# WT-MM/thor-slam

Hardware: AMD Instinct MI355X
Metric: synced stereo frames/sec (detect+match+pose) @640×400, 1/2/4/8 GPU (higher is better)
Workload: dtype u8+f64

## Files before the change

thor-slam_amd/csrc/k_describe.hip:

```cpp
#include "tslam_common.h"

#include "tslam_describe.h"

#define TS_DT_G 1

__device__ __forceinline__ void glds16d(const void* src, void* wave_dst) {
    __builtin_amdgcn_global_load_lds((__attribute__((address_space(1))) void*)src,
                                     (__attribute__((address_space(3))) void*)wave_dst, 16, 0, 0);
}

template <int NCH, int NLD = NCH>
__device__ __forceinline__ void stage_tile(const uint8_t* level, int W, int H, int r0, int cs, int nrows,
                                           uint8_t* lds, bool wide16) {
    const int lane = threadIdx.x & 63, wave = threadIdx.x >> 6;
    if (wide16) {
        const int n = nrows * NCH;
        for (int i0 = wave * 64; i0 < n; i0 += TS_DT_THREADS) {
            const int i = i0 + lane;
            if (i < n) {
                const int r = i / NCH, q = i - r * NCH;
                const int y = r0 + r, x = cs + 16 * q;
                if (q < NLD && y >= 0 && y < H && x >= 0 && x + 16 <= W) glds16d(level + (size_t)y * W + x, lds + 16 * i0);
            }
        }
    } else {
        for (int i = threadIdx.x; i < nrows * 16 * NCH; i += TS_DT_THREADS) {
            const int r = i / (16 * NCH), q = i - r * (16 * NCH);
            const int y = r0 + r, x = cs + q;
            if (y >= 0 && y < H && x >= 0 && x < W) lds[i] = level[(size_t)y * W + x];
        }
    }
}

struct DiscSlot {
    uint32_t wx, mk, wy;
    int32_t rofs;
};
struct DiscTable {
    DiscSlot e[320];
};
constexpr DiscTable make_disc_table() {
    DiscTable t{};
    for (int s = 0; s < 320; ++s) {
        const int r = s / 9, w = s - 9 * r;
        uint32_t a = 0, m = 0, b = 0;
        for (int j = 0; j < 4; ++j) {
            const int dx = 4 * w - 15 + j, dy = r - 15;
            if (r < 31 && dx <= 15 && dx * dx + dy * dy <= 225) {
                a |= (uint32_t)(dx + 15) << (8 * j);
                m |= 1u << (8 * j);
                b |= (uint32_t)(dy + 15) << (8 * j);
            }
        }
        t.e[s] = DiscSlot{a, m, b, (r < 30 ? r : 30) * TS_DT_RAW_P + 4 * w};
    }
    return t;
}
__constant__ DiscTable c_disc = make_disc_table();

__global__ __launch_bounds__(TS_DT_THREADS) void k_describe(BatchCtx c) {
    __shared__ __attribute__((aligned(16))) uint8_t s_raw[(TS_DT_RAW_ROWS + 1) * TS_DT_RAW_P];
    __shared__ __attribute__((aligned(16))) uint8_t s_smo[TS_DT_SMO_ROWS * TS_DT_P];
    __shared__ uint16_t s_list[TS_DT_W * TS_DT_H / 4];
    __shared__ uint32_t s_n;
    const int lane = threadIdx.x & 63, wave = threadIdx.x >> 6;
    int img, local;
    if (!xcd_image_block(blockIdx.x, c.n * c.ncam, c.g.dt_total, &img, &local)) return;
    int l = 0;
    while (l + 1 < c.g.n_levels && local >= c.g.dt_start[l + 1]) ++l;
    local -= c.g.dt_start[l];
    const int nx = c.g.dt_nx[l];
    const int ty = local / nx, tx = local - ty * nx;
    const int W = c.g.W[l], H = c.g.H[l];
    const int x0 = tx * TS_DT_W, y0 = ty * TS_DT_H;
    int cam, f;
    view_image(c, img, &f, &cam);
    const int slot = ring_slot(c, c.g0 + f);
    const size_t ib = (size_t)slot * c.C + cam;
    const uint8_t* raw = c.pyr + ib * c.g.pyr_bytes + c.g.pyr_off[l];
    const uint8_t* smo = c.smo + ((size_t)f * c.C + cam) * c.g.pyr_bytes + c.g.pyr_off[l];
    uint32_t* kps = c.kps + ib * c.g.K * 2;
    uint32_t* desc = c.desc + ib * c.g.K * 8;
    uint32_t* desc_ys = c.desc_ys + ib * c.g.K * 8;
    const uint4* ys = c.ys + ib * c.g.K + c.g.koff[l];
    const uint16_t* rs = c.rowstart + ib * c.g.rs_total + c.g.rs_off[l];
    const int kn = c.kcount[ib * c.g.n_levels + l];

    if (local == 0) {
        const int Kl = c.g.Kq[l];
        for (int i = kn * 8 + threadIdx.x; i < Kl * 8; i += TS_DT_THREADS) {
            desc[(size_t)(c.g.koff[l] + i / 8) * 8 + (i & 7)] = 0u;
            desc_ys[(size_t)(c.g.koff[l] + i / 8) * 8 + (i & 7)] = 0u;
        }
    }
    const int pa = rs[y0], pb = rs[min(y0 + TS_DT_H, H)];
    if (pa >= pb) return;
    if (threadIdx.x == 0) s_n = 0;
    __syncthreads();

    const bool wide16 = ((W & 15) == 0) && ((c.g.pyr_off[l] & 15) == 0) && ((c.g.pyr_bytes & 15) == 0);
    const int c0 = x0 - TS_DT_HX;
    const int cr = x0 - 16;
    stage_tile<TS_DT_RAW_P / 16>(raw, W, H, y0 - 15, cr, TS_DT_RAW_ROWS, s_raw, wide16);
    stage_tile<TS_DT_P / 16, (TS_DT_W + 2 * TS_DT_HX) / 16>(smo, W, H, y0 - 18, c0, TS_DT_SMO_ROWS, s_smo, wide16);

    uint32_t wx[5], mk[5], wy[5];
    int rofs[5];
#pragma unroll
    for (int i = 0; i < 5; ++i) {
        const uint4 d = reinterpret_cast<const uint4*>(&c_disc)[lane + 64 * i];
        wx[i] = d.x;
        mk[i] = d.y;
        wy[i] = d.z;
        rofs[i] = (int)d.w;
    }
    const double wa0 = lane < 30 ? (double)c.wedges[2 * lane] : 0.0, wa1 = lane < 30 ? (double)c.wedges[2 * lane + 1] : 0.0;
    const double wb0 = lane < 30 ? (double)c.wedges[2 * lane + 2] : 0.0, wb1 = lane < 30 ? (double)c.wedges[2 * lane + 3] : 0.0;

    for (int p = pa + threadIdx.x; p < pb; p += TS_DT_THREADS) {
        const int x = ys[p].x & 0xFFFF;
        if (x >= x0 && x < x0 + TS_DT_W) s_list[atomicAdd(&s_n, 1u)] = (uint16_t)p;
    }
    __syncthreads();
    const int n = (int)s_n;
    for (int g0 = wave * TS_DT_G; g0 < n; g0 += (TS_DT_THREADS / 64) * TS_DT_G) {
        int bin[TS_DT_G], pos[TS_DT_G];
        uint4 rec[TS_DT_G];
#pragma unroll
        for (int g = 0; g < TS_DT_G; ++g) {
            pos[g] = g0 + g < n ? (int)s_list[g0 + g] : -1;
            rec[g] = pos[g] >= 0 ? ys[pos[g]] : uint4{0u, 0u, 0u, 0u};
        }
#pragma unroll
        for (int g = 0; g < TS_DT_G; ++g) {
            bin[g] = 0;
            if (pos[g] < 0) continue;
            const int x = rec[g].x & 0xFFFF, y = rec[g].x >> 16;
            const int ob = (y - y0) * TS_DT_RAW_P + (x - 15 - cr);
            const uint32_t sh = (uint32_t)ob & 3u;
            const uint8_t* obase = s_raw + (ob & ~3);
            uint32_t sx = 0, s1 = 0, sy = 0;
#pragma unroll
            for (int i = 0; i < 5; ++i) {
                const uint32_t* wp = reinterpret_cast<const uint32_t*>(obase + rofs[i]);
                const uint32_t v = __builtin_amdgcn_alignbyte(wp[1], wp[0], sh);
                s1 = __builtin_amdgcn_udot4(mk[i], v, s1, false);
                sx = __builtin_amdgcn_udot4(wx[i], v, sx, false);
                sy = __builtin_amdgcn_udot4(wy[i], v, sy, false);
            }
            const int s15 = (int)__umul24(s1, 15u);
            const int m10 = wave_sum_dpp((int)sx - s15);
            const int m01 = wave_sum_dpp((int)sy - s15);
            const double d01 = (double)m01, d10 = (double)m10;
            const bool hit = lane < 30 && (wa0 * d01 - wa1 * d10) >= 0.0 && (wb0 * d01 - wb1 * d10) < 0.0;
            const uint64_t hm = __ballot(hit);
            bin[g] = hm ? (int)__builtin_ctzll(hm) : 0;
        }
        uint32_t t[TS_DT_G][4];
#pragma unroll
        for (int g = 0; g < TS_DT_G; ++g)
#pragma unroll
            for (int j = 0; j < 4; ++j) t[g][j] = pos[g] >= 0 ? c.brief_table[bin[g] * 256 + 64 * j + lane] : 0u;
#pragma unroll
        for (int g = 0; g < TS_DT_G; ++g) {
            if (pos[g] < 0) continue;
            const int x = rec[g].x & 0xFFFF, y = rec[g].x >> 16;
            const uint8_t* pbase = s_smo + (y - y0) * TS_DT_P + (x - 18 - c0);
            uint32_t words[8];
#pragma unroll
            for (int j = 0; j < 4; ++j) {
                const int a = pbase[t[g][j] & 0xFFFFu];
                const int b = pbase[t[g][j] >> 16];
                const uint64_t bm = __ballot(a < b);
                words[2 * j] = (uint32_t)bm;
                words[2 * j + 1] = (uint32_t)(bm >> 32);
            }
            const int kidx = (int)rec[g].z;
            uint32_t w = 0;
#pragma unroll
            for (int j = 0; j < 8; ++j) asm volatile("v_writelane_b32 %0, %1, %2" : "+v"(w) : "s"(words[j]), "i"(j));
            if (lane < 8) {
                desc[(size_t)kidx * 8 + lane] = w;
                desc_ys[(size_t)(c.g.koff[l] + pos[g]) * 8 + lane] = w;
            }
            if (lane == 0) kps[(size_t)kidx * 2 + 1] = (rec[g].y & ~0xFF00u) | ((uint32_t)bin[g] << 8);
        }
    }
}

void launch_describe(const BatchCtx& c, hipStream_t s) {
    hipLaunchKernelGGL(k_describe, dim3(xcd_grid(c.n * c.ncam, c.g.dt_total)), dim3(TS_DT_THREADS), 0, s, c);
}
```

thor-slam_amd/csrc/k_image.hip:

```cpp
#include "tslam_common.h"

__device__ __forceinline__ int remap_px(const uint8_t* src, int W, int H, int2 m) {
    const int sx = m.x >> 5, sy = m.y >> 5;
    const int fx = m.x & 31, fy = m.y & 31;
    const int xa = min(max(sx, 0), W - 1), xb = min(max(sx + 1, 0), W - 1);
    const int ya = min(max(sy, 0), H - 1), yb = min(max(sy + 1, 0), H - 1);
    const int p00 = src[ya * W + xa], p01 = src[ya * W + xb];
    const int p10 = src[yb * W + xa], p11 = src[yb * W + xb];
    const int acc = p00 * (32 - fx) * (32 - fy) + p01 * fx * (32 - fy) + p10 * (32 - fx) * fy + p11 * fx * fy;
    return (acc + 512) >> 10;
}

__device__ __forceinline__ uint32_t box4(uint32_t r0a, uint32_t r0b, uint32_t r1a, uint32_t r1b) {
    auto pairsum = [](uint32_t v) { return (v & 0x00FF00FFu) + ((v >> 8) & 0x00FF00FFu); };
    const uint32_t sa = pairsum(r0a) + pairsum(r1a) + 0x00020002u;
    const uint32_t sb = pairsum(r0b) + pairsum(r1b) + 0x00020002u;
    const uint32_t qa = (sa >> 2) & 0x00FF00FFu, qb = (sb >> 2) & 0x00FF00FFu;
    return __builtin_amdgcn_perm(qb, qa, 0x06040200u);
}

__global__ __launch_bounds__(256) void k_rectify_pyramid(BatchCtx c) {
    extern __shared__ __attribute__((aligned(16))) uint8_t lds[];
    const int img = blockIdx.y;
    int f, cam;
    view_image(c, img, &f, &cam);
    const int W = c.W, H = c.H;
    const int y0 = blockIdx.x * TS_RECT_BAND;
    const int rows0 = min(TS_RECT_BAND, H - y0);
    const uint8_t* src = c.images + view_src(c, img) * W * H;
    uint8_t* pyr = c.pyr + ((size_t)ring_slot(c, c.g0 + f) * c.C + cam) * c.g.pyr_bytes;
    const bool has_map = (c.map_mask >> cam) & 1u;
    const int32_t* map = c.maps + (size_t)cam * W * H * 2;
    bool wide = (W & 63) == 0 && (c.g.pyr_bytes & 15) == 0;
    for (int l = 1; l < c.g.n_levels; ++l) wide = wide && (c.g.pyr_off[l] & 15) == 0 && (c.g.W[l] & 15) == 0;

    uint8_t* l0 = lds;
    if (wide) {
        const int W16 = W >> 4, n16 = rows0 * W16;
        for (int i = threadIdx.x; i < n16; i += blockDim.x) {
            const int r = i / W16, x16 = i - r * W16;
            const size_t off = (size_t)(y0 + r) * W + 16 * x16;
            uint4 v;
            if (has_map) {
                uint32_t w[4];
                const int2* mp = reinterpret_cast<const int2*>(map) + off;
#pragma unroll
                for (int q = 0; q < 4; ++q) {
                    uint32_t acc = 0;
#pragma unroll
                    for (int b = 0; b < 4; ++b) acc |= (uint32_t)remap_px(src, W, H, mp[4 * q + b]) << (8 * b);
                    w[q] = acc;
                }
                v = {w[0], w[1], w[2], w[3]};
            } else {
                v = *reinterpret_cast<const uint4*>(src + off);
            }
            reinterpret_cast<uint4*>(l0)[i] = v;
            *reinterpret_cast<uint4*>(pyr + off) = v;
        }
        __syncthreads();
        const uint8_t* prev = l0;
        int prevW = W;
        uint8_t* cur = l0 + TS_RECT_BAND * W;
        for (int l = 1; l < c.g.n_levels; ++l) {
            const int Wl = c.g.W[l], Hl = c.g.H[l];
            const int ly0 = y0 >> l;
            const int lrows = min(TS_RECT_BAND >> l, Hl - ly0);
            const int W4 = Wl >> 2;
            uint8_t* out = pyr + c.g.pyr_off[l];
            for (int i = threadIdx.x; i < lrows * W4; i += blockDim.x) {
                const int r = i / W4, x4 = i - r * W4;
                const uint2 a = *reinterpret_cast<const uint2*>(prev + (2 * r) * prevW + 8 * x4);
                const uint2 b = *reinterpret_cast<const uint2*>(prev + (2 * r + 1) * prevW + 8 * x4);
                const uint32_t v = box4(a.x, a.y, b.x, b.y);
                reinterpret_cast<uint32_t*>(cur)[i] = v;
                *reinterpret_cast<uint32_t*>(out + (size_t)(ly0 + r) * Wl + 4 * x4) = v;
            }
            __syncthreads();
            prev = cur;
            prevW = Wl;
            cur = cur + (TS_RECT_BAND >> l) * Wl;
        }
        return;
    }

    for (int idx = threadIdx.x; idx < rows0 * W; idx += blockDim.x) {
        const int r = idx / W;
        const int x = idx - r * W;
        const int y = y0 + r;
        const int v = has_map ? remap_px(src, W, H, *reinterpret_cast<const int2*>(map + ((size_t)y * W + x) * 2))
                              : src[y * W + x];
        l0[r * W + x] = (uint8_t)v;
        pyr[(size_t)y * W + x] = (uint8_t)v;
    }
    __syncthreads();
    const uint8_t* prev = l0;
    int prevW = W;
    uint8_t* cur = l0 + TS_RECT_BAND * W;
    for (int l = 1; l < c.g.n_levels; ++l) {
        const int Wl = c.g.W[l], Hl = c.g.H[l];
        const int ly0 = y0 >> l;
        const int lrows = min(TS_RECT_BAND >> l, Hl - ly0);
        uint8_t* out = pyr + c.g.pyr_off[l];
        for (int idx = threadIdx.x; idx < lrows * Wl; idx += blockDim.x) {
            const int r = idx / Wl;
            const int x = idx - r * Wl;
            const int a = prev[(2 * r) * prevW + 2 * x] + prev[(2 * r) * prevW + 2 * x + 1] +
                          prev[(2 * r + 1) * prevW + 2 * x] + prev[(2 * r + 1) * prevW + 2 * x + 1];
            const uint8_t v = (uint8_t)((a + 2) >> 2);
            cur[r * Wl + x] = v;
            out[(size_t)(ly0 + r) * Wl + x] = v;
        }
        __syncthreads();
// ... 268 lines not shown
            kbits |= ((nb >> 15) & 1u) << h;
            kbits |= ((nb >> 31) & 1u) << (h + 2);
        }
#pragma unroll
        for (int j = 0; j < 4; ++j)
            if (x0 + j < M || x0 + j >= W - M) kbits &= ~(1u << j);
    }
    uint64_t bm[4];
    uint32_t tot = 0;
#pragma unroll
    for (int j = 0; j < 4; ++j) {
        bm[j] = __ballot((kbits >> j) & 1u);
        tot += (uint32_t)__popcll(bm[j]);
    }
    if (tot == 0) return;
    uint32_t base = 0;
    if (lane == 0) base = atomicAdd(count, tot);
    base = (uint32_t)__builtin_amdgcn_readfirstlane((int)base);
#pragma unroll
    for (int j = 0; j < 4; ++j) {
        if ((kbits >> j) & 1u) {
            const uint32_t rank = __builtin_amdgcn_mbcnt_hi((uint32_t)(bm[j] >> 32), __builtin_amdgcn_mbcnt_lo((uint32_t)bm[j], 0u));
            const uint32_t pv = (P >> (8 * j)) & 0xFFu;
            cand[base + rank] = ((255u - pv) << 22) | ((uint32_t)y << 11) | (uint32_t)(x0 + j);
            atomicAdd(&hist[255 - pv], 1u);
        }
        base += (uint32_t)__popcll(bm[j]);
    }
}


__device__ __forceinline__ void glds16(const uint4* src, uint4* wave_dst) {
    __builtin_amdgcn_global_load_lds((__attribute__((address_space(1))) void*)src,
                                     (__attribute__((address_space(3))) void*)wave_dst, 16, 0, 0);
}

typedef unsigned short u16x2 __attribute__((ext_vector_type(2)));

struct HsumSel {
    uint32_t d0, d1, d3, d4;
};
__device__ __forceinline__ HsumSel hsum_sel(bool first, bool last) {
    return {first ? 0x05040404u : 0x05040302u, first ? 0x06050404u : 0x06050403u,
            last ? 0x03030201u : 0x04030201u, last ? 0x03030302u : 0x05040302u};
}
__device__ __forceinline__ void hsum4(const uint8_t* p, const HsumSel& s, u16x2* ev, u16x2* od) {
    const uint32_t a = *(const uint32_t*)(p - 4), b = *(const uint32_t*)p, c2 = *(const uint32_t*)(p + 4);
    const uint32_t D0 = __builtin_amdgcn_perm(b, a, s.d0), D1 = __builtin_amdgcn_perm(b, a, s.d1);
    const uint32_t D3 = __builtin_amdgcn_perm(c2, b, s.d3), D4 = __builtin_amdgcn_perm(c2, b, s.d4);
    const uint32_t h0 = __builtin_amdgcn_udot4(D0, 0x04060401u, D1 >> 24, false);
    const uint32_t h1 = __builtin_amdgcn_udot4(D1, 0x04060401u, b >> 24, false);
    const uint32_t h2 = __builtin_amdgcn_udot4(b, 0x04060401u, D3 >> 24, false);
    const uint32_t h3 = __builtin_amdgcn_udot4(D3, 0x04060401u, D4 >> 24, false);
    *ev = __builtin_bit_cast(u16x2, h0 | (h2 << 16));
    *od = __builtin_bit_cast(u16x2, h1 | (h3 << 16));
}

__device__ __forceinline__ uint32_t vsum4(u16x2 e0, u16x2 e1, u16x2 e2, u16x2 e3, u16x2 e4, u16x2 d0, u16x2 d1,
                                          u16x2 d2, u16x2 d3, u16x2 d4) {
    const u16x2 four = {4, 4}, six = {6, 6}, rnd = {128, 128};
    const u16x2 ve = six * e2 + (four * (e1 + e3) + ((e0 + e4) + rnd));
    const u16x2 vo = six * d2 + (four * (d1 + d3) + ((d0 + d4) + rnd));
    return __builtin_amdgcn_perm(__builtin_bit_cast(uint32_t, vo), __builtin_bit_cast(uint32_t, ve), 0x07030501u);
}

template <int MODE, bool CNT>
__device__ __forceinline__ void detect_body(const BatchCtx& c, int bx, int img) {
    extern __shared__ __attribute__((aligned(16))) uint8_t lds[];
    __shared__ uint32_t s_hist[256];
    __shared__ uint32_t s_count;
    __shared__ uint16_t s_q[TS_DET_WAVES][2][TS_DET_Q];
    __shared__ __attribute__((aligned(16))) uint32_t s_tail[2][TS_DET_WAVES];
    int f, cam;
    view_image(c, img, &f, &cam);
    int l = 0;
    while (l + 1 < c.g.n_levels && bx >= c.g.band_start[l + 1]) ++l;
    const int te = MODE == 1 ? c.fast_threshold + 1
                                   : max(c.fast_threshold + 1, (int)c.det_thr[(size_t)cam * c.g.n_levels + l]);
    const int band = bx - c.g.band_start[l];
    const int W = c.g.W[l], H = c.g.H[l];
    const int BR = c.g.band_rows[l];
    const int y0 = band * BR;
    const int lane = threadIdx.x & 63, wave = threadIdx.x >> 6;
    const size_t img_off = ((size_t)ring_slot(c, c.g0 + f) * c.C + cam) * c.g.pyr_bytes + c.g.pyr_off[l];
    const uint8_t* src = c.pyr + img_off;
    uint8_t* smo = c.smo + ((size_t)f * c.C + cam) * c.g.pyr_bytes + c.g.pyr_off[l];
    const int NR = BR + 2 * TS_DET_HALO;
    uint8_t* tile = lds;
    uint8_t* score = lds + NR * W;
    const int thr = c.fast_threshold;
    const bool wide = ((W & 3) == 0) && ((img_off & 3) == 0);
    const int rows_here = min(BR, H - y0);

    for (int i = threadIdx.x; i < 256; i += TS_DET_THREADS) s_hist[i] = 0;
    if (threadIdx.x == 0) s_count = 0;
    if (((W & 15) == 0) && ((img_off & 15) == 0)) {
        const int W16 = W >> 4, n16 = NR * W16;
        const uint4* s16 = (const uint4*)src;
        const int dr = TS_DET_THREADS / W16, dx = TS_DET_THREADS - dr * W16;
        int r = (wave * 64 + lane) / W16, x = wave * 64 + lane - r * W16;
        for (int i0 = wave * 64; i0 < n16; i0 += TS_DET_THREADS) {
            if (i0 + lane < n16)
                glds16(s16 + (size_t)min(max(y0 - TS_DET_HALO + r, 0), H - 1) * W16 + x, (uint4*)tile + i0);
            r += dr;
            x += dx;
            if (x >= W16) {
                x -= W16;
                ++r;
            }
        }
    } else {
        for (int i = threadIdx.x; i < NR * W; i += TS_DET_THREADS) {
            const int r = i / W, x = i - r * W;
            tile[i] = src[(size_t)min(max(y0 - TS_DET_HALO + r, 0), H - 1) * W + x];
        }
    }
    __syncthreads();

    if (wide) {
        const int W4 = W >> 2;
        const int groups = c.g.smooth_groups[l];
        const int SR = (BR + groups - 1) / groups;
        for (int it = threadIdx.x; it < groups * W4; it += TS_DET_THREADS) {
            const int half = it / W4, q = it - half * W4, x0 = 4 * q;
            const int o0 = SR * half, o1 = min(o0 + SR, rows_here);
            if (o0 >= o1) continue;
            const HsumSel hs = hsum_sel(q == 0, q == W4 - 1);
            const uint8_t* rp = tile + (TS_DET_HALO - 2 + o0) * W + x0;
            u16x2 e0, e1, e2, e3, e4, d0, d1, d2, d3, d4;
            hsum4(rp, hs, &e0, &d0);
            hsum4(rp + W, hs, &e1, &d1);
            hsum4(rp + 2 * W, hs, &e2, &d2);
            hsum4(rp + 3 * W, hs, &e3, &d3);
            rp += 4 * W;
            uint32_t off = (uint32_t)((y0 + o0) * W + x0);
            int o = o0;
#define TS_SMOOTH_ROW(A, B, C, D, N, a, b, cc, d, n)                            \
    {                                                                         \
        hsum4(rp, hs, &N, &n);                                                \
        *(uint32_t*)(smo + off) = vsum4(A, B, C, D, N, a, b, cc, d, n);       \
        rp += W;                                                              \
        off += (uint32_t)W;                                                   \
        if (++o == o1) break;                                                 \
    }
            for (;;) {
                TS_SMOOTH_ROW(e0, e1, e2, e3, e4, d0, d1, d2, d3, d4)
                TS_SMOOTH_ROW(e1, e2, e3, e4, e0, d1, d2, d3, d4, d0)
                TS_SMOOTH_ROW(e2, e3, e4, e0, e1, d2, d3, d4, d0, d1)
                TS_SMOOTH_ROW(e3, e4, e0, e1, e2, d3, d4, d0, d1, d2)
                TS_SMOOTH_ROW(e4, e0, e1, e2, e3, d4, d0, d1, d2, d3)
            }
#undef TS_SMOOTH_ROW
        }
    } else {
        for (int x = threadIdx.x; x < W; x += TS_DET_THREADS) {
            const int xm2 = max(x - 2, 0), xm1 = max(x - 1, 0), xp1 = min(x + 1, W - 1), xp2 = min(x + 2, W - 1);
            int h0 = 0, h1 = 0, h2 = 0, h3 = 0;
            for (int r = TS_DET_HALO - 2; r < TS_DET_HALO + rows_here + 2; ++r) {
                const uint8_t* row = tile + r * W;
                const int h4 = row[xm2] + 4 * row[xm1] + 6 * row[x] + 4 * row[xp1] + row[xp2];
                if (r >= TS_DET_HALO + 2) {
                    const int acc = h0 + 4 * h1 + 6 * h2 + 4 * h3 + h4;
                    smo[(size_t)(y0 + r - 2 - TS_DET_HALO) * W + x] = (uint8_t)((acc + 128) >> 8);
                }
                h0 = h1; h1 = h2; h2 = h3; h3 = h4;
            }
        }
// ... 370 lines not shown
    }
    {
        const uint32_t bc = (int)threadIdx.x < nb ? cnt[threadIdx.x] : 0u;
        const uint32_t incl = block_inclusive_scan<NT>(bc, s_part, 1);
        if (threadIdx.x == 0) s_pref[0] = 0u;
        if ((int)threadIdx.x < nb) s_pref[threadIdx.x + 1] = incl;
    }
    __syncthreads();
    const int ncand = (int)s_pref[nb];
    auto sweep_g = [&](auto&& fn) {
        int lo = 0;
        for (int i0 = threadIdx.x; i0 < ncand; i0 += 4 * NT) {
            uint32_t k[4];
#pragma unroll
            for (int u = 0; u < 4; ++u) {
                const int i = i0 + u * NT;
                k[u] = 0u;
                if (i < ncand) {
                    while ((int)s_pref[lo + 1] <= i) ++lo;
                    k[u] = cand[__umul24((uint32_t)lo, (uint32_t)cap) + (uint32_t)(i - (int)s_pref[lo])];
                }
            }
#pragma unroll
            for (int u = 0; u < 4; ++u)
                if (i0 + u * NT < ncand) fn(i0 + u * NT, k[u]);
        }
    };
    bool res = false;
    auto sweep = [&](auto&& fn) {
        if (S::RCAP > 0 && res) {
            for (int i = threadIdx.x; i < ncand; i += NT) fn(i, s_res[i]);
        } else {
            sweep_g(fn);
        }
    };
    const bool fits = S::RCAP > 0 && ncand <= rcap;

    block_find_crossing<NT>(s_h, 256, (uint32_t)Kl, s_part, s_x);
    const uint32_t total = s_x[3];
    for (int i = threadIdx.x; i < 256; i += NT) s_h[i] = 0u;
    uint32_t thresh = 0xFFFFFFFFu;
    if (total > (uint32_t)Kl) {
        const uint32_t sbin = s_x[0];
        const uint32_t need = (uint32_t)Kl - s_x[1];
        const uint32_t eq = s_x[2];
        thresh = (sbin << 22) | 0x3FFFFFu;
        if (need < eq) {
            res = fits;
            sweep_g([&](int i, uint32_t k) {
                if (S::RCAP > 0 && res) s_res[i] = k;
                if ((k >> 22) == sbin) atomicAdd(&s_a[(k >> 11) & 2047u], 1u);
            });
            __syncthreads();
            block_find_crossing<NT>(s_a, BINS, need, s_part, s_x);
            const uint32_t ystar = s_x[0];
            const uint32_t need2 = need - s_x[1];
            const uint32_t eq2 = s_x[2];
            thresh = (sbin << 22) | (ystar << 11) | 2047u;
            for (int i = threadIdx.x; i < BINS; i += NT) s_a[i] = 0u;
            if (need2 < eq2) {
                sweep([&](int, uint32_t k) {
                    if ((k >> 11) == ((sbin << 11) | ystar)) atomicAdd(&s_fill[k & 2047u], 1u);
                });
                __syncthreads();
                block_find_crossing<NT>(s_fill, BINS, need2, s_part, s_x);
                thresh = (sbin << 22) | (ystar << 11) | s_x[0];
                if (!S::BIG || Kl <= S::KCAP)
                    for (int i = threadIdx.x; i < BINS; i += NT) s_fill[i] = 0u;
            }
        }
    }
    if (S::RCAP > 0 && !res && fits && eager) {
        sweep_g([&](int i, uint32_t k) { s_res[i] = k; });
        res = true;
    }
    sweep([&](int, uint32_t k) {
        if (k <= thresh) {
            const uint32_t slot = atomicAdd(&s_nsel, 1u);
            if (slot < (uint32_t)(S::BIG ? SEL_MAX : S::KCAP)) s_keys[slot] = k;
        }
    });
    __syncthreads();
    const int nsel = min((int)s_nsel, Kl);
    const int slot = ring_slot(c, c.g0 + f);
    uint32_t* kp = c.kps + (((size_t)slot * c.C + cam) * c.g.K + c.g.koff[l]) * 2;
    const int Hl = c.g.H[l];
    const bool counting = !S::BIG || nsel <= S::KCAP;
    if (counting) {
        for (int i = threadIdx.x; i < nsel; i += NT) atomicAdd(&s_h[s_keys[i] >> 22], 1u);
        __syncthreads();
        for (int b = threadIdx.x; b < 256; b += NT)
            if (s_h[b] > TS_SEL_BUCKET_MAX) s_flag = 1;
        block_exclusive_scan<NT>(s_h, 256, s_part);
    }
    __syncthreads();
    if (counting && s_flag == 0) {
        uint32_t* fill = s_h + 256;
        for (int i = threadIdx.x; i < nsel; i += NT) {
            const uint32_t k = s_keys[i], b = k >> 22;
            s_tmp[s_h[b] + atomicAdd(&fill[b], 1u)] = k;
        }
        __syncthreads();
        for (int i = threadIdx.x; i < nsel; i += NT) {
            const uint32_t k = s_tmp[i], b = k >> 22;
            const int lo = (int)s_h[b], n = (int)fill[b];
            int r = 0;
            for (int j = lo; j < lo + n; ++j) r += s_tmp[j] < k;
            s_keys[lo + r] = k;
        }
        __syncthreads();
    } else {
        bitonic_sort<NT>(s_keys, nsel);
    }
    for (int i = threadIdx.x; i < Kl; i += NT) {
        uint32_t xy = 0, meta = (uint32_t)l;
        if (i < nsel) {
            const uint32_t k = s_keys[i];
            xy = (k & 2047u) | (((k >> 11) & 2047u) << 16);
            meta = (uint32_t)l | ((255u - (k >> 22)) << 16);
        }
        kp[2 * i] = xy;
        kp[2 * i + 1] = meta;
    }
    if (threadIdx.x == 0) {
        c.kcount[((size_t)slot * c.C + cam) * c.g.n_levels + l] = nsel;
        const int tfull = c.fast_threshold + 1;
        const int te = MODE == 1 ? tfull : max(tfull, (int)c.det_thr[(size_t)cam * c.g.n_levels + l]);
        const bool short_k = (int)total < Kl;
        if (MODE == 0) c.det_fail[fcl] = (short_k && te > tfull) ? 1u : 0u;
        int next = tfull;
        if (!short_k && nsel > 0) {
            const int sk = 255 - (int)(s_keys[nsel - 1] >> 22);
            next = max(tfull, sk - 2);
        }
        atomicMin(&c.det_thr_acc[(size_t)cam * c.g.n_levels + l], (uint32_t)next);
    }

    uint4* ys = c.ys + ((size_t)slot * c.C + cam) * c.g.K + c.g.koff[l];
    uint16_t* rs = c.rowstart + ((size_t)slot * c.C + cam) * c.g.rs_total + c.g.rs_off[l];
    uint16_t* yp = c.ypos + ((size_t)slot * c.C + cam) * c.g.K;
    auto record = [&](int rank) -> uint4 {
        const uint32_t k = s_keys[rank];
        return {(k & 2047u) | (((k >> 11) & 2047u) << 16), (uint32_t)l | ((255u - (k >> 22)) << 16),
                (uint32_t)(c.g.koff[l] + rank), 1u};
    };
    for (int i = nsel + threadIdx.x; i < Kl; i += NT) {
        ys[i] = {0u, (uint32_t)l, (uint32_t)(c.g.koff[l] + i), 0u};
        yp[c.g.koff[l] + i] = (uint16_t)(c.g.koff[l] + i);
    }
    if (counting) {
        for (int i = threadIdx.x; i < nsel; i += NT) atomicAdd(&s_a[(s_keys[i] >> 11) & 2047u], 1u);
        __syncthreads();
        block_exclusive_scan<NT>(s_a, BINS, s_part);
        for (int y = threadIdx.x; y <= Hl; y += NT) rs[y] = (uint16_t)s_a[y];
        for (int i = threadIdx.x; i < nsel; i += NT) {
            const uint32_t y = (s_keys[i] >> 11) & 2047u;
            s_tmp[s_a[y] + atomicAdd(&s_fill[y], 1u)] = (uint32_t)i;
        }
        __syncthreads();
        for (int p = threadIdx.x; p < nsel; p += NT) {
            const uint32_t i = s_tmp[p], y = (s_keys[i] >> 11) & 2047u;
            const int lo = (int)s_a[y], n = (int)s_fill[y];
            int r = 0;
            for (int j = lo; j < lo + n; ++j) r += s_tmp[j] < i;
            ys[lo + r] = record((int)i);
            yp[c.g.koff[l] + i] = (uint16_t)(c.g.koff[l] + lo + r);
        }
// ... 85 lines not shown
```

thor-slam_amd/csrc/k_match.hip:

```cpp
#include "tslam_common.h"

#define TS_MQ 128
#define TS_MRED_PITCH 33
#define TS_MRING 1024
#define TS_MCHUNKS 6
#define TS_MCNT_MERGED 0
#define TS_MCNT_DIRECT 1
#define TS_MCNT_FLUSHED 2
#define TS_MCNT_EMPTY 3
#define TS_MCNT_WALKED 4

typedef int v8i_t __attribute__((ext_vector_type(8)));
typedef float v16f_t __attribute__((ext_vector_type(16)));
typedef unsigned short u16x2_t __attribute__((ext_vector_type(2)));

__device__ __forceinline__ uint32_t med3_u32(uint32_t a, uint32_t b, uint32_t c) {
    uint32_t r;
    asm("v_med3_u32 %0, %1, %2, %3" : "=v"(r) : "v"(a), "v"(b), "v"(c));
    return r;
}

__device__ __forceinline__ bool gate_ok(uint32_t qgate, uint32_t txy, uint32_t span) {
    const u16x2_t d = __builtin_bit_cast(u16x2_t, qgate) - __builtin_bit_cast(u16x2_t, txy);
    const u16x2_t m = __builtin_elementwise_min(d, __builtin_bit_cast(u16x2_t, span));
    return __builtin_bit_cast(uint32_t, m) == __builtin_bit_cast(uint32_t, d);
}

__device__ __forceinline__ uint32_t key_dist(uint32_t key) {
    return (uint32_t)__uint_as_float(key & 0xFFFF8000u);
}

template <bool CNT>
__device__ __forceinline__ void match_body(const BatchCtx& c) {
    TS_BACK_PRIO;
    __shared__ __attribute__((aligned(16))) uint2 s_red[4][32 * TS_MRED_PITCH];
    __shared__ __attribute__((aligned(16))) uint32_t s_key[2][TS_MQ];
    __shared__ __attribute__((aligned(16))) uint32_t s_wk[4][32];
    uint4* const s_qrec = reinterpret_cast<uint4*>(&s_red[0][0]);
    uint4* const s_qdesc = s_qrec + TS_MQ;
    __shared__ uint32_t s_sq[4][32];
    __shared__ uint32_t s_si[4][32];
    __shared__ __attribute__((aligned(16))) uint32_t s_sg[4][2][16];
    __shared__ __attribute__((aligned(16))) float s_spc[4][2][16];
    __shared__ uint32_t s_tb[TS_MTB];
    const int nfp = c.match_modes == 1 ? 0 : c.n * c.npair;
    const int z = blockIdx.y;
    const int mode = z < nfp ? 1 : 0;
    const int fl = z < nfp ? z : z - nfp;
    const int p = c.pair0 + fl % c.npair;
    const int f = fl / c.npair;
    const int64_t g = c.g0 + f;
    int l = 0;
    while (l + 1 < c.g.n_levels && (int)blockIdx.x >= c.g.qtile_start[l + 1]) ++l;
    const int tile = blockIdx.x - c.g.qtile_start[l];
    const int q0 = tile * TS_MQ;
    const size_t mbase = (((size_t)f * c.P + p) * 2 + mode) * c.g.K;
    auto no_match = [&]() {
        if ((int)threadIdx.x < TS_MQ && q0 + (int)threadIdx.x < c.g.Kq[l]) c.qbest[mbase + c.g.koff[l] + q0 + threadIdx.x] = 0xFFFFFFFFu;
        if (CNT && threadIdx.x == 0) atomicAdd(&c.match_cnt[8 * mode + TS_MCNT_EMPTY], 1u);
    };
    if ((mode == 1 && g == 0) ||
        (mode == 0 && c.rgbd)) {
        no_match();
        return;
    }
    const int slot = ring_slot(c, g);
    const int qcam = c.cpp * p;
    const int tslot = mode == 0 ? slot : ring_slot(c, g - 1);
    const int tcam = mode == 0 ? qcam + 1 : qcam;
    const int K = c.g.K;
    const int qn = c.kcount[((size_t)slot * c.C + qcam) * c.g.n_levels + l];
    const int tn = c.kcount[((size_t)tslot * c.C + tcam) * c.g.n_levels + l];
    if (q0 >= qn || tn == 0) {
        no_match();
        return;
    }
    if (CNT && threadIdx.x == 0) atomicAdd(&c.match_cnt[8 * mode + TS_MCNT_WALKED], 1u);
    const int lane = threadIdx.x & 63, wave = threadIdx.x >> 6;
    const int ci = lane & 31, h = lane >> 5;
    const size_t qbase = ((size_t)slot * c.C + qcam) * K;
    const size_t tbase = ((size_t)tslot * c.C + tcam) * K;
    const uint4* qys = c.ys + qbase + c.g.koff[l];
    const uint4* tys = c.ys + tbase + c.g.koff[l];
    uint32_t* const tb = c.tbest + mbase + c.g.koff[l];
    const uint4* qdesc = reinterpret_cast<const uint4*>(c.desc_ys + (qbase + c.g.koff[l]) * 8);
    const uint4* tdesc = reinterpret_cast<const uint4*>(c.desc_ys + (tbase + c.g.koff[l]) * 8);
    const uint16_t* trs = c.rowstart + ((size_t)tslot * c.C + tcam) * c.g.rs_total + c.g.rs_off[l];
    const int Hl = c.g.H[l];
    const int row_tol = c.mp.row_tol, dmax = c.mp.max_disp >> l, win = c.mp.window >> l;
    const int gx_lo = mode == 0 ? 1 : -win, gx_hi = mode == 0 ? dmax : win, gy_tol = mode == 0 ? row_tol : win;
    const uint32_t span = (uint32_t)(2 * gy_tol) << 16 | (uint32_t)(gx_hi - gx_lo);

    const int nq = min(TS_MQ, qn - q0);
    {
        const int t = threadIdx.x & (TS_MQ - 1), half = threadIdx.x >> 7;
        const int pos = q0 + min(t, nq - 1);
        if (half == 0) s_qrec[t] = qys[pos];
        s_qdesc[2 * t + half] = qdesc[2 * pos + half];
    }
    __syncthreads();
    const bool wave_active = 32 * wave < nq;
    const int reach = mode == 0 ? row_tol : win;
    int wt0 = 0, wt1 = 0;
    {
        const int i0 = mode == 1 ? 0 : min(32 * wave, nq - 1), i1 = mode == 1 ? nq - 1 : min(32 * wave + 31, nq - 1);
        const int wy0 = (int)(s_qrec[i0].x >> 16), wy1 = (int)(s_qrec[i1].x >> 16);
        if (wave_active) {
            wt0 = (int)trs[max(0, wy0 - reach)];
            wt1 = (int)trs[min(Hl - 1, wy1 + reach) + 1];
        }
    }
    const uint32_t mcap = (uint32_t)min(c.mp.merge_cap, TS_MTB);
    int bt0 = 0, bt1 = 0;
    if (mcap) {
        const int by0 = (int)(s_qrec[0].x >> 16), by1 = (int)(s_qrec[nq - 1].x >> 16);
        bt0 = __builtin_amdgcn_readfirstlane((int)trs[max(0, by0 - reach)]);
        bt1 = __builtin_amdgcn_readfirstlane((int)trs[min(Hl - 1, by1 + reach) + 1]);
        for (int i = threadIdx.x; i < min((int)mcap, bt1 - bt0); i += 256) s_tb[i] = 0xFFFFFFFFu;
    }
    int bi = 32 * wave + ci;
    if (mode == 1) {
        if (threadIdx.x < TS_MQ) {
            const int t = threadIdx.x;
            s_key[0][t] = t < nq ? (s_qrec[t].x & 0xFFFF) << 8 | (uint32_t)t : 0x1000000u | (uint32_t)t;
        }
        __syncthreads();
        if (threadIdx.x < TS_MQ) {
            const uint32_t key = s_key[0][threadIdx.x];
            int rank = 0;
            const uint4* k4 = reinterpret_cast<const uint4*>(s_key[0]);
#pragma unroll 4
            for (int i = 0; i < TS_MQ / 4; ++i) {
                const uint4 v = k4[i];
                rank += (v.x < key) + (v.y < key) + (v.z < key) + (v.w < key);
            }
            s_key[1][rank] = threadIdx.x;
        }
        __syncthreads();
        bi = (int)s_key[1][32 * wave + ci];
    }
    const bool active = bi < nq;
    int qx = 0, qy = 0;
    uint32_t qi = 0, pc = 0;
    if (active) {
        const uint4 rec = s_qrec[bi];
        const uint4 d = s_qdesc[2 * bi + h];
        qi = rec.z;
        qx = rec.x & 0xFFFF;
        qy = rec.x >> 16;
        pc = __popc(d.x) + __popc(d.y) + __popc(d.z) + __popc(d.w);
    }
// ... 153 lines not shown
                    if (lane == 0 && nd) atomicAdd(&c.match_cnt[8 * mode + TS_MCNT_DIRECT], nd);
                }
            }
        }
        __builtin_amdgcn_fence(__ATOMIC_RELEASE, "wavefront");
        __builtin_amdgcn_wave_barrier();
        __builtin_amdgcn_fence(__ATOMIC_ACQUIRE, "wavefront");
    }

    __builtin_amdgcn_fence(__ATOMIC_RELEASE, "wavefront");
    __builtin_amdgcn_wave_barrier();
    __builtin_amdgcn_fence(__ATOMIC_ACQUIRE, "wavefront");
    uint2* red = s_red[wave];
#pragma unroll
    for (int r = 0; r < 16; ++r) red[(2 * r + h) * TS_MRED_PITCH + ci] = uint2{best[r], second[r]};
    __builtin_amdgcn_fence(__ATOMIC_RELEASE, "wavefront");
    __builtin_amdgcn_wave_barrier();
    __builtin_amdgcn_fence(__ATOMIC_ACQUIRE, "wavefront");
    uint32_t b = 0xFFFFFFFFu, s2 = 0xFFFFFFFFu;
#pragma unroll
    for (int i = 0; i < 16; ++i) {
        const uint2 v = red[ci * TS_MRED_PITCH + 16 * h + i];
        s2 = min(min(s2, v.y), max(b, v.x));
        b = min(b, v.x);
    }
    {
        const uint32_t ob = (uint32_t)__shfl_xor((int)b, 32, 64), os = (uint32_t)__shfl_xor((int)s2, 32, 64);
        s2 = min(min(s2, os), max(b, ob));
        b = min(b, ob);
    }
    const uint32_t qk = s_sq[wave][ci];
    const int qpos = q0 + (int)s_si[wave][ci];
    if (h == 0 && qpos < c.g.Kq[l]) {
        const size_t qp = mbase + c.g.koff[l] + qpos;
        const bool found = qk != 0xFFFFFFFFu && b < 0x7F800000u;
        c.qbest[qp] = found ? key_dist(b) << 16 | (b & 0x7FFFu) : 0xFFFFFFFFu;
        if (qk != 0xFFFFFFFFu) c.qsecond[qp] = s2 < 0x7F800000u ? key_dist(s2) : 256u;
        c.qtpos[qp] = found ? c.ypos[tbase + (b & 0x7FFFu)] : (uint16_t)0;
    }
    if (mcap) {
        __syncthreads();
        const int len = min((int)mcap, bt1 - bt0);
        uint32_t na = 0;
        for (int i = threadIdx.x; i < len; i += 256) {
            const uint32_t v = s_tb[i];
            if (v != 0xFFFFFFFFu) {
                atomicMin(&tb[bt0 + i], v);
                ++na;
            }
        }
        if (CNT && na) atomicAdd(&c.match_cnt[8 * mode + TS_MCNT_FLUSHED], na);
    }
}

__device__ __forceinline__ double parabola(int sm, int s0, int sp) {
    const int den = sm - 2 * s0 + sp;
    return den > 0 ? (double)(sm - sp) / (2.0 * (double)den) : 0.0;
}

__device__ __forceinline__ void row11(const uint8_t* img, int W, int y, int x0, uint32_t* w) {
    const uint8_t* a = img + (size_t)y * W + x0;
    const uint32_t sh = (uint32_t)(reinterpret_cast<uintptr_t>(a) & 3u);
    const uint32_t* p = reinterpret_cast<const uint32_t*>(a - sh);
    const uint32_t d0 = p[0], d1 = p[1], d2 = p[2], d3 = p[3];
    w[0] = __builtin_amdgcn_alignbyte(d1, d0, sh);
    w[1] = __builtin_amdgcn_alignbyte(d2, d1, sh);
    w[2] = __builtin_amdgcn_alignbyte(d3, d2, sh) & 0x00FFFFFFu;
}

__device__ __forceinline__ uint4 stage_row11(const uint8_t* img, int W, int y, int x0) {
    uint32_t w3[3];
    row11(img, W, y, x0, w3);
    return uint4{w3[0], w3[1], w3[2], 0u};
}

__device__ __forceinline__ uint4 align_row15(const uint32_t* d, uint32_t sh) {
    return uint4{__builtin_amdgcn_alignbyte(d[1], d[0], sh), __builtin_amdgcn_alignbyte(d[2], d[1], sh),
                 __builtin_amdgcn_alignbyte(d[3], d[2], sh), __builtin_amdgcn_alignbyte(d[4], d[3], sh) & 0x00FFFFFFu};
}
__device__ __forceinline__ uint4 stage_row15(const uint8_t* img, int W, int y, int x0) {
    const uint8_t* a = img + (size_t)y * W + x0;
    const uint32_t sh = (uint32_t)(reinterpret_cast<uintptr_t>(a) & 3u);
    const uint32_t* q = reinterpret_cast<const uint32_t*>(a - sh);
    const uint32_t d[5] = {q[0], q[1], q[2], q[3], q[4]};
    return align_row15(d, sh);
}

__device__ __forceinline__ void shift_row11(const uint4* row, int kx, uint32_t* w) {
    const uint32_t* wb = reinterpret_cast<const uint32_t*>(row);
    const int kh = kx >> 2;
    const uint32_t sh = (uint32_t)(kx & 3);
    const uint32_t d0 = wb[kh], d1 = wb[kh + 1], d2 = wb[kh + 2], d3 = wb[3 - kh];
    w[0] = __builtin_amdgcn_alignbyte(d1, d0, sh);
    w[1] = __builtin_amdgcn_alignbyte(d2, d1, sh);
    w[2] = __builtin_amdgcn_alignbyte(d3, d2, sh) & 0x00FFFFFFu;
}

__device__ __forceinline__ uint32_t sad_row11(const uint32_t* a, const uint32_t* w, uint32_t s) {
    s = __builtin_amdgcn_sad_u8(a[0], w[0], s);
    s = __builtin_amdgcn_sad_u8(a[1], w[1], s);
    return __builtin_amdgcn_sad_u8(a[2], w[2], s);
}

template <int ASH>
__device__ __forceinline__ uint32_t stereo_sad(const uint4* a, const uint4* b, int kx) {
    uint32_t s = 0;
#pragma unroll
    for (int dy = 0; dy < 11; ++dy) {
        uint32_t la[3], w[3];
        if (ASH < 0) {
            const uint4 ra = a[dy];
            la[0] = ra.x, la[1] = ra.y, la[2] = ra.z;
        } else {
            shift_row11(a + dy, ASH, la);
        }
        shift_row11(b + dy, kx, w);
        s = sad_row11(la, w, s);
    }
    return s;
}

__device__ __forceinline__ void stereo_store(const BatchCtx& c, size_t out, int j, int l, int qx, int xr, int ks,
                                             const int* cost) {
    double d0 = __builtin_nan("");
    if (j >= 0 && ks > 0 && ks < 4) {
        const double delta = parabola(cost[ks - 1], cost[ks], cost[ks + 1]);
        const double sc = (double)(1 << l);
        const double v = ((double)qx - ((double)(xr + (ks - TS_SAD_RANGE)) + delta)) * sc;
        if (v > 0.0) d0 = v;
    }
    c.stereo[out] = j;
    c.disp[out] = d0;
}

#define TS_RT_AROWS 11
#define TS_RT_BROWS 15
__device__ __forceinline__ void temporal_sad(const uint4* a, const uint4* b, int kx, uint32_t* s) {
#pragma unroll
    for (int ky = 0; ky < 5; ++ky) s[ky] = 0u;
#pragma unroll
    for (int r = 0; r < TS_RT_BROWS; ++r) {
        uint32_t w[3];
        shift_row11(b + r, kx, w);
#pragma unroll
        for (int ky = 0; ky < 5; ++ky) {
            const int dy = r - ky;
            if (dy < 0 || dy >= TS_RT_AROWS) continue;
            const uint4 ra = a[dy];
            const uint32_t la[3] = {ra.x, ra.y, ra.z};
            s[ky] = sad_row11(la, w, s[ky]);
        }
    }
}

__device__ __forceinline__ void temporal_store(double* out_uv, int j, int l, int qx, int qy, int a, const int* cq) {
    double u = __builtin_nan(""), v = u;
    if (j >= 0) {
        const int c0 = cq[a];
        const int cl = cq[max(a - 1, 0)], cr = cq[min(a + 1, 24)];
        const int cu = cq[max(a - 5, 0)], cd = cq[min(a + 5, 24)];
        const int ky = a / 5, kx = a % 5;
        if (kx > 0 && kx < 4 && ky > 0 && ky < 4) {
            const double ddx = parabola(cl, c0, cr);
            const double ddy = parabola(cu, c0, cd);
            const double sc = (double)(1 << l);
            u = (((double)(qx + (kx - TS_SAD_RANGE)) + ddx) + 0.5) * sc - 0.5;
            v = (((double)(qy + (ky - TS_SAD_RANGE)) + ddy) + 0.5) * sc - 0.5;
        }
    }
    out_uv[0] = u;
    out_uv[1] = v;
}

struct MatchRef {
    uint32_t qb, sd, tb;
    int j, tp;
};
__device__ __forceinline__ void match_query(const BatchCtx& c, size_t mbase, int pos, MatchRef* m) {
    m->qb = c.qbest[mbase + pos];
    m->sd = c.qsecond[mbase + pos];
    m->tp = c.qtpos[mbase + pos];
    m->j = m->qb == 0xFFFFFFFFu ? 0 : (int)(m->qb & 0xFFFF);
}
__device__ __forceinline__ void match_train(const BatchCtx& c, size_t mbase, size_t tkb, MatchRef* m, uint32_t* tkp) {
    m->tb = c.tbest[mbase + m->tp];
    *tkp = c.kps[(tkb + m->j) * 2];
}
__device__ __forceinline__ int match_accept(const BatchCtx& c, const MatchRef& m, int qi, bool ok) {
    const int bd = (int)(m.qb >> 16);
    return ((int)ok & (int)(m.qb != 0xFFFFFFFFu) & (int)(bd <= c.mp.max_hamming) &
            (int)(bd * 100 < c.mp.ratio_pct * (int)m.sd) & (int)((int)(m.tb & 0xFFFF) == qi)) ? m.j : -1;
}
__device__ __forceinline__ int match_lookup(const BatchCtx& c, size_t mbase, int pos, int qi, bool ok, size_t tkb,
                                            uint32_t* tkp) {
    MatchRef m;
    match_query(c, mbase, pos, &m);
    match_train(c, mbase, tkb, &m, tkp);
    return match_accept(c, m, qi, ok);
}

#define TS_RS_QPB 32
__global__ __launch_bounds__(256) void k_refine_stereo(BatchCtx c) {
    TS_BACK_PRIO;
    __shared__ uint4 s_a[TS_RS_QPB][11];
    __shared__ uint4 s_b[TS_RS_QPB][11];
    __shared__ int s_cost[TS_RS_QPB][5];
    const int lane = threadIdx.x & 63, wave = threadIdx.x >> 6;
    const int K = c.g.K;
    int z, local;
    if (!xcd_image_block(blockIdx.x, c.n * c.npair, (K + TS_RS_QPB - 1) / TS_RS_QPB, &z, &local)) return;
    const int p = c.pair0 + z % c.npair, f = z / c.npair;
    const int64_t g = c.g0 + f;
    const int slot = ring_slot(c, g);
    const int sub = lane & 7;
    const int qslot = wave * 8 + (lane >> 3);
    const int pos = local * TS_RS_QPB + qslot;
    const bool live = pos < K;
    const size_t mbase = (((size_t)f * c.P + p) * 2 + 0) * K;
    const int qcam = c.cpp * p;
    const size_t qkb = ((size_t)slot * c.C + qcam) * K;
    int l = 0, qi = 0, j = -1;
    uint32_t qxy = 0, tkp = 0;
    if (live) {
        const uint4 rec = c.ys[qkb + pos];
        qi = (int)rec.z;
        l = (int)(rec.y & 0xFFu);
        qxy = rec.x;
        j = match_lookup(c, mbase, pos, qi, rec.w != 0, ((size_t)slot * c.C + qcam + 1) * K, &tkp);
    }
    int qx = 0, xr = 0;
    if (j >= 0) {
        const int W = c.g.W[l];
        qx = qxy & 0xFFFF;
        const int qy = qxy >> 16;
        xr = tkp & 0xFFFF;
        const uint8_t* Lp = c.pyr + ((size_t)slot * c.C + qcam) * c.g.pyr_bytes + c.g.pyr_off[l];
        const uint8_t* Rp = c.pyr + ((size_t)slot * c.C + qcam + 1) * c.g.pyr_bytes + c.g.pyr_off[l];
        for (int hl = sub; hl < 22; hl += 8) {
            if (hl < 11)
                s_a[qslot][hl] = stage_row11(Lp, W, qy - TS_SAD_HALF + hl, qx - TS_SAD_HALF);
            else
                s_b[qslot][hl - 11] = stage_row15(Rp, W, qy - TS_SAD_HALF + hl - 11, xr - TS_SAD_HALF - TS_SAD_RANGE);
        }
    }
    __builtin_amdgcn_fence(__ATOMIC_ACQ_REL, "wavefront");
    uint32_t key = 0xFFFFFFFFu;
    if (j >= 0 && sub < 5) {
        const uint32_t s = stereo_sad<-1>(s_a[qslot], s_b[qslot], sub);
        s_cost[qslot][sub] = (int)s;
        key = (s << 5) | (uint32_t)sub;
    }
#pragma unroll
    for (int m = 1; m < 8; m <<= 1) key = min(key, (uint32_t)__shfl_xor((int)key, m, 64));
    __builtin_amdgcn_fence(__ATOMIC_ACQ_REL, "wavefront");
    if (live && sub == 0) stereo_store(c, ((size_t)slot * c.P + p) * K + qi, j, l, qx, xr, (int)(key & 31u), s_cost[qslot]);
}

#define TS_RT_QPB 32
__global__ __launch_bounds__(256) void k_refine_temporal(BatchCtx c) {
    TS_BACK_PRIO;
    __shared__ uint4 s_a[TS_RT_QPB][TS_RT_AROWS];
    __shared__ uint4 s_b[TS_RT_QPB][TS_RT_BROWS];
    __shared__ int s_cost[TS_RT_QPB][25];
    const int lane = threadIdx.x & 63, wave = threadIdx.x >> 6;
    const int K = c.g.K;
    int z, local;
    if (!xcd_image_block(blockIdx.x, c.n * c.npair, (K + TS_RT_QPB - 1) / TS_RT_QPB, &z, &local)) return;
    const int p = c.pair0 + z % c.npair, f = z / c.npair;
    const int64_t g = c.g0 + f;
    const int slot = ring_slot(c, g);
    const int sub = lane & 7;
    const int qslot = wave * 8 + (lane >> 3);
    const int pos = local * TS_RT_QPB + qslot;
    const bool live = pos < K;
    const size_t mbase = (((size_t)f * c.P + p) * 2 + 1) * K;
    const int qcam = c.cpp * p;
    const size_t qkb = ((size_t)slot * c.C + qcam) * K;
    int l = 0, qi = 0, j = -1;
    uint32_t qxy = 0, pxy = 0;
    const int pslot = g > 0 ? ring_slot(c, g - 1) : slot;
    if (live) {
        const uint4 rec = c.ys[qkb + pos];
        qi = (int)rec.z;
        l = (int)(rec.y & 0xFFu);
        qxy = rec.x;
        j = match_lookup(c, mbase, pos, qi, rec.w != 0 && g > 0, ((size_t)pslot * c.C + qcam) * K, &pxy);
    }
    int32_t* out_idx = c.temporal + ((size_t)slot * c.P + p) * K;
    double* out_uv = c.tuv + (((size_t)f * c.P + p) * K + qi) * 2;
    if (live && sub == 0) out_idx[qi] = j;
    int qx = 0, qy = 0;
    if (j >= 0) {
        const int W = c.g.W[l];
        qx = qxy & 0xFFFF;
        qy = qxy >> 16;
        const int px = pxy & 0xFFFF, py = pxy >> 16;
        const uint8_t* A = c.pyr + ((size_t)pslot * c.C + qcam) * c.g.pyr_bytes + c.g.pyr_off[l];
        const uint8_t* B = c.pyr + ((size_t)slot * c.C + qcam) * c.g.pyr_bytes + c.g.pyr_off[l];
        for (int hl = sub; hl < TS_RT_AROWS + TS_RT_BROWS; hl += 8) {
            if (hl < TS_RT_AROWS)
                s_a[qslot][hl] = stage_row11(A, W, py - TS_SAD_HALF + hl, px - TS_SAD_HALF);
            else
                s_b[qslot][hl - TS_RT_AROWS] = stage_row15(B, W, qy - TS_SAD_HALF - TS_SAD_RANGE + hl - TS_RT_AROWS,
                                                           qx - TS_SAD_HALF - TS_SAD_RANGE);
        }
    }
    __builtin_amdgcn_fence(__ATOMIC_ACQ_REL, "wavefront");
    uint32_t key = 0xFFFFFFFFu;
    if (j >= 0 && sub < 5) {
        uint32_t s[5];
        temporal_sad(s_a[qslot], s_b[qslot], sub, s);
#pragma unroll
        for (int ky = 0; ky < 5; ++ky) {
            const int o = ky * 5 + sub;
            s_cost[qslot][o] = (int)s[ky];
            key = min(key, (s[ky] << 5) | (uint32_t)o);
        }
    }
#pragma unroll
    for (int m = 1; m < 8; m <<= 1) key = min(key, (uint32_t)__shfl_xor((int)key, m, 64));
    __builtin_amdgcn_fence(__ATOMIC_ACQ_REL, "wavefront");
    if (live && sub == 0) temporal_store(out_uv, j, l, qx, qy, (int)(key & 31u), s_cost[qslot]);
}

#define TS_RP_QPB 32
#define TS_RP_ROWS (TS_RT_BROWS + TS_RT_AROWS + 11)
#define TS_RP_ROUNDS ((TS_RP_ROWS + 7) / 8)
__global__ __launch_bounds__(256) void k_refine_pair(BatchCtx c) {
    TS_BACK_PRIO;
    __shared__ uint4 s_rows[TS_RP_QPB][TS_RP_ROWS];
    __shared__ int s_ct[TS_RP_QPB][25];
    __shared__ int s_cs[TS_RP_QPB][5];
    const int lane = threadIdx.x & 63, wave = threadIdx.x >> 6;
    const int K = c.g.K;
    int z, local;
    if (!xcd_image_block(blockIdx.x, c.n * c.npair, (K + TS_RP_QPB - 1) / TS_RP_QPB, &z, &local)) return;
    const int p = c.pair0 + z % c.npair, f = z / c.npair;
    const int64_t g = c.g0 + f;
    const int slot = ring_slot(c, g);
    const int pslot = g > 0 ? ring_slot(c, g - 1) : slot;
    const int sub = lane & 7;
    const int qslot = wave * 8 + (lane >> 3);
    const int pos = local * TS_RP_QPB + qslot;
    const bool live = pos < K;
    const size_t mbase = ((size_t)f * c.P + p) * 2 * K;
    const int qcam = c.cpp * p;
    const size_t qkb = ((size_t)slot * c.C + qcam) * K;
    int l = 0, qi = 0, js = -1, jt = -1;
    uint32_t qxy = 0, tkp = 0, pxy = 0;
    if (live) {
        const uint4 rec = c.ys[qkb + pos];
        qi = (int)rec.z;
        l = (int)(rec.y & 0xFFu);
        qxy = rec.x;
        MatchRef ms, mt;
        match_query(c, mbase, pos, &ms);
        match_query(c, mbase + K, pos, &mt);
        match_train(c, mbase, ((size_t)slot * c.C + qcam + 1) * K, &ms, &tkp);
        match_train(c, mbase + K, ((size_t)pslot * c.C + qcam) * K, &mt, &pxy);
        js = match_accept(c, ms, qi, rec.w != 0);
        jt = match_accept(c, mt, qi, rec.w != 0 && g > 0);
    }
    const size_t out = ((size_t)slot * c.P + p) * K + qi;
    if (live && sub == 0) c.temporal[out] = jt;
    const int qx = qxy & 0xFFFF, qy = qxy >> 16, xr = tkp & 0xFFFF;
    {
        int W = c.g.W[0], loff = c.g.pyr_off[0];
#pragma unroll
        for (int i = 1; i < TS_MAX_LEVELS; ++i)
            if (l >= i) W = c.g.W[i], loff = c.g.pyr_off[i];
        const int px = pxy & 0xFFFF, py = pxy >> 16;
        const uint8_t* cur = c.pyr + ((size_t)slot * c.C + qcam) * c.g.pyr_bytes + loff;
        const uint8_t* rgt = cur + c.g.pyr_bytes;
        const uint8_t* prv = c.pyr + ((size_t)pslot * c.C + qcam) * c.g.pyr_bytes + loff;
        const int nw = jt >= 0 ? TS_RT_BROWS : js >= 0 ? 11 : 0, w0 = jt >= 0 ? 0 : TS_SAD_RANGE;
        const int np = jt >= 0 ? TS_RT_AROWS : 0;
        const int total = nw + np + (js >= 0 ? 11 : 0);
        uint32_t d[TS_RP_ROUNDS][5], sh[TS_RP_ROUNDS];
#pragma unroll
        for (int k = 0; k < TS_RP_ROUNDS; ++k) {
            const int hl = sub + 8 * k;
            const bool inw = hl < nw, inp = !inw && hl < nw + np;
            const int r = inw ? hl + w0 : inp ? hl - nw : hl - nw - np;
            const uint8_t* img = inw ? cur : inp ? prv : rgt;
            const int y = inw ? qy - TS_SAD_HALF - TS_SAD_RANGE + r : inp ? py - TS_SAD_HALF + r : qy - TS_SAD_HALF + r;
            const int x0 = inw ? qx - TS_SAD_HALF - TS_SAD_RANGE : inp ? px - TS_SAD_HALF : xr - TS_SAD_HALF - TS_SAD_RANGE;
            const uint8_t* a = hl < total ? img + (size_t)y * W + x0 : cur;
            sh[k] = (uint32_t)(reinterpret_cast<uintptr_t>(a) & 3u);
            const uint32_t* q = reinterpret_cast<const uint32_t*>(a - sh[k]);
#pragma unroll
            for (int i = 0; i < 5; ++i) d[k][i] = q[i];
        }
#pragma unroll
        for (int k = 0; k < TS_RP_ROUNDS; ++k) {
            const int hl = sub + 8 * k;
            const bool inw = hl < nw, inp = !inw && hl < nw + np;
            uint4 v = align_row15(d[k], sh[k]);
            if (inp) v.z &= 0x00FFFFFFu, v.w = 0u;
            const int row = inw ? hl + w0 : inp ? TS_RT_BROWS + hl - nw : TS_RT_BROWS + TS_RT_AROWS + hl - nw - np;
            if (hl < total) s_rows[qslot][row] = v;
        }
    }
    __builtin_amdgcn_fence(__ATOMIC_ACQ_REL, "wavefront");
    const uint4* rows = s_rows[qslot];
    uint32_t kt = 0xFFFFFFFFu, ks = 0xFFFFFFFFu;
    if (jt >= 0 && sub < 5) {
        uint32_t s[5];
        temporal_sad(rows + TS_RT_BROWS, rows, sub, s);
#pragma unroll
        for (int ky = 0; ky < 5; ++ky) {
            const int o = ky * 5 + sub;
            s_ct[qslot][o] = (int)s[ky];
            kt = min(kt, (s[ky] << 5) | (uint32_t)o);
        }
    }
    if (js >= 0 && sub < 5) {
        const uint32_t s = stereo_sad<TS_SAD_RANGE>(rows + TS_SAD_RANGE, rows + TS_RT_BROWS + TS_RT_AROWS, sub);
        s_cs[qslot][sub] = (int)s;
        ks = (s << 5) | (uint32_t)sub;
    }
#pragma unroll
    for (int m = 1; m < 8; m <<= 1) {
        kt = min(kt, (uint32_t)__shfl_xor((int)kt, m, 64));
        ks = min(ks, (uint32_t)__shfl_xor((int)ks, m, 64));
    }
    __builtin_amdgcn_fence(__ATOMIC_ACQ_REL, "wavefront");
    if (live && sub == 0) {
        temporal_store(c.tuv + (((size_t)f * c.P + p) * K + qi) * 2, jt, l, qx, qy, (int)(kt & 31u), s_ct[qslot]);
        stereo_store(c, out, js, l, qx, xr, (int)(ks & 31u), s_cs[qslot]);
    }
}

__global__ __launch_bounds__(256) __attribute__((amdgpu_waves_per_eu(4))) void k_match(BatchCtx c) { match_body<false>(c); }
__global__ __launch_bounds__(256) __attribute__((amdgpu_waves_per_eu(4))) void k_match_counted(BatchCtx c) { match_body<true>(c); }

static void launch_k_match(const BatchCtx& c, dim3 grid, hipStream_t s) {
    if (c.match_cnt)
        hipLaunchKernelGGL(k_match_counted, grid, dim3(256), 0, s, c);
    else
        hipLaunchKernelGGL(k_match, grid, dim3(256), 0, s, c);
}

int match_blocks_per_cu() {
    int n = 0;
    return hipOccupancyMaxActiveBlocksPerMultiprocessor(&n, k_match, 256, 0) == hipSuccess ? n : -1;
}

void launch_match(const BatchCtx& c, hipStream_t s) {
    (void)hipMemsetAsync(c.tbest, 0xFF, sizeof(uint32_t) * (size_t)c.n * c.P * 2 * c.g.K, s);
    dim3 grid(c.g.total_qtiles, c.n * c.npair * (c.match_modes == 1 ? 1 : 2));
    launch_k_match(c, grid, s);
}

void launch_match_stereo(const BatchCtx& c, hipStream_t s) {
    BatchCtx st = c;
    st.match_modes = 1;
    (void)hipMemsetAsync(st.tbest, 0xFF, sizeof(uint32_t) * (size_t)st.n * st.P * 2 * st.g.K, s);
    launch_k_match(st, dim3(st.g.total_qtiles, st.n * st.npair), s);
    hipLaunchKernelGGL(k_refine_stereo, dim3(xcd_grid(st.n * st.npair, (st.g.K + TS_RS_QPB - 1) / TS_RS_QPB)), dim3(256), 0, s, st);
}

void launch_match_refine(const BatchCtx& c, hipStream_t s) {
    const int K = c.g.K;
    if (!c.rgbd && c.match_modes == 3 && c.mp.refine_split == 0) {
        hipLaunchKernelGGL(k_refine_pair, dim3(xcd_grid(c.n * c.npair, (K + TS_RP_QPB - 1) / TS_RP_QPB)), dim3(256), 0, s, c);
        return;
    }
    if (c.rgbd)
        launch_rgbd_depth(c, s);
    else
        hipLaunchKernelGGL(k_refine_stereo, dim3(xcd_grid(c.n * c.npair, (K + TS_RS_QPB - 1) / TS_RS_QPB)), dim3(256), 0, s, c);
    hipLaunchKernelGGL(k_refine_temporal, dim3(xcd_grid(c.n * c.npair, (K + TS_RT_QPB - 1) / TS_RT_QPB)), dim3(256), 0, s, c);
}
```

thor-slam_amd/csrc/k_pose.hip:

```cpp
#include "tslam_common.h"
#include "tslam_mul4.h"

#define P3P_VMAX 1000.0
#define P3P_BISECT 60

struct V3 {
    double x, y, z;
};

__device__ __forceinline__ double dot3(V3 a, V3 b) { return (a.x * b.x + a.y * b.y) + a.z * b.z; }
__device__ __forceinline__ V3 sub3(V3 a, V3 b) { return {a.x - b.x, a.y - b.y, a.z - b.z}; }
__device__ __forceinline__ V3 cross3(V3 a, V3 b) {
    return {a.y * b.z - a.z * b.y, a.z * b.x - a.x * b.z, a.x * b.y - a.y * b.x};
}
__device__ __forceinline__ V3 norm3(V3 a) {
    const double n = sqrt(dot3(a, a));
    return {a.x / n, a.y / n, a.z / n};
}
__device__ __forceinline__ void frame3(V3 p1, V3 p2, V3 p3, V3* e) {
    e[0] = norm3(sub3(p2, p1));
    e[2] = norm3(cross3(e[0], sub3(p3, p1)));
    e[1] = cross3(e[2], e[0]);
}
__device__ __forceinline__ double comp(V3 a, int i) { return i == 0 ? a.x : (i == 1 ? a.y : a.z); }
// ... 119 lines not shown
}

__device__ __forceinline__ uint64_t splitmix64(uint64_t x) {
    x = x + 0x9E3779B97F4A7C15ull;
    x = (x ^ (x >> 30)) * 0xBF58476D1CE4E5B9ull;
    x = (x ^ (x >> 27)) * 0x94D049BB133111EBull;
    return x ^ (x >> 31);
}

__device__ __forceinline__ bool is_inlier(const double* R, const double* t, const double* cr, double fx, double fy, double thr2) {
    const double X = cr[0], Y = cr[1], Z = cr[2], du = cr[3], dv = cr[4];
    const double xc = ((R[0] * X + R[1] * Y) + R[2] * Z) + t[0];
    const double yc = ((R[3] * X + R[4] * Y) + R[5] * Z) + t[1];
    const double zc = ((R[6] * X + R[7] * Y) + R[8] * Z) + t[2];
    const double ex = fx * xc + du * zc;
    const double ey = fy * yc + dv * zc;
    const double e2 = ex * ex + ey * ey;
    const double lim = thr2 * (zc * zc);
    return zc > 0.0 && e2 < lim;
}

typedef float f32x16 __attribute__((ext_vector_type(16)));
__device__ __forceinline__ int inlier_f32(const f32x16& pf, const float* q, float fx, float fy, float thr2) {
    const float X = q[0], Y = q[1], Z = q[2], du = q[3], dv = q[4];
    const float xc = fmaf(pf[0], X, fmaf(pf[1], Y, fmaf(pf[2], Z, pf[9])));
    const float yc = fmaf(pf[3], X, fmaf(pf[4], Y, fmaf(pf[5], Z, pf[10])));
    const float zc = fmaf(pf[6], X, fmaf(pf[7], Y, fmaf(pf[8], Z, pf[11])));
    const float ex = fmaf(fx, xc, du * zc);
    const float ey = fmaf(fy, yc, dv * zc);
    const float e2 = fmaf(ex, ex, ey * ey);
    const float lim = thr2 * (zc * zc);
    const float D = lim - e2;
    const float a = fmaf(pf[12], q[5], pf[13]);
    const float inner = fmaf(fabsf(ex), q[6], fmaf(fabsf(ey), q[7], thr2 * fabsf(zc)));
    const float bsum = fmaf(a, inner, e2 + lim);
    const float E = bsum * (32.0f / 16777216.0f);
    const float Ez = a * (32.0f / 16777216.0f);
    if (zc < -Ez || D < -E) return 0;
    if (zc > Ez && D > E) return 1;
    return -1;
}

__device__ bool solve6(const double* Hm, const double* g, double* x, double* L) {
    double inv[6];
    for (int j = 0; j < 6; ++j) {
        double s = Hm[j * 6 + j];
        for (int k = 0; k < j; ++k) s = s - L[j * 6 + k] * L[j * 6 + k];
        if (!(s > 0.0)) return false;
        const double d = sqrt(s);
        L[j * 6 + j] = d;
        inv[j] = 1.0 / d;
        for (int i = j + 1; i < 6; ++i) {
            double t = Hm[i * 6 + j];
            for (int k = 0; k < j; ++k) t = t - L[i * 6 + k] * L[j * 6 + k];
            L[i * 6 + j] = t * inv[j];
        }
    }
    double y[6];
    for (int i = 0; i < 6; ++i) {
        double s = g[i];
        for (int k = 0; k < i; ++k) s = s - L[i * 6 + k] * y[k];
        y[i] = s * inv[i];
    }
    for (int i = 5; i >= 0; --i) {
        double s = y[i];
        for (int k = i + 1; k < 6; ++k) s = s - L[k * 6 + i] * x[k];
        x[i] = s * inv[i];
    }
    return true;
}

#define POSE_THREADS 256
#define TS_RS_CPT 4
#define TS_MAX_HYP_SPLIT 256
#define N_ACC 29

__device__ __forceinline__ void write_stats(int32_t* so, int status, int n, int n_in, int best_cnt, int best_idx, int64_t g) {
    so[0] = status; so[1] = n; so[2] = n_in; so[3] = best_cnt; so[4] = best_idx; so[5] = (int)g; so[6] = 0; so[7] = 0;
}

__global__ __launch_bounds__(POSE_THREADS) void k_corr(BatchCtx c) {
    TS_BACK_PRIO;
    __shared__ int s_scan[2 * (POSE_THREADS / 64)];
    const int p = c.pair0 + (int)blockIdx.x % c.npair;
    const int f = (int)blockIdx.x / c.npair;
    const int fp = f * c.P + p;
    const int64_t g = c.g0 + f;
    const int tid = threadIdx.x;
    const int K = c.g.K;
    double* pout = c.pose + (size_t)fp * TS_POSE_DOUBLES;
    int32_t* sout = c.stats + (size_t)fp * TS_STATS_INTS;
    for (int i = tid; i < TS_POSE_DOUBLES; i += POSE_THREADS) pout[i] = (i < 16 && (i % 5) == 0) ? 1.0 : 0.0;
    if (g == 0) {
        if (tid == 0) write_stats(sout, 2, 0, 0, 0, -1, g);
        return;
    }
    const PairCalib cal = c.calib[p];
    const double fx = cal.fx, fy = cal.fy, cx = cal.cx, cy = cal.cy;
    const int pslot = ring_slot(c, g - 1);
    const int32_t* tm = c.temporal + ((size_t)ring_slot(c, g) * c.P + p) * K;
    const double* tuv = c.tuv + ((size_t)f * c.P + p) * K * 2;
    const double* dprev = c.disp + ((size_t)pslot * c.P + p) * K;
    const uint32_t* kprev = c.kps + ((size_t)pslot * c.C + c.cpp * p) * K * 2;
    double* corr = c.corr + ((size_t)f * c.P + p) * K * TS_CORR_DOUBLES;
    int n = 0;
    for (int base = 0; base < K; base += POSE_THREADS) {
        const int j = base + tid;
        int flag = 0, i = -1;
        double u = 0.0, v = 0.0, d = 0.0;
        if (j < K) {
            i = tm[j];
            if (i >= 0) {
                d = dprev[i];
                u = tuv[2 * j];
                v = tuv[2 * j + 1];
                flag = __builtin_isfinite(d) && __builtin_isfinite(u) && __builtin_isfinite(v);
            }
        }
        const uint64_t bm = __ballot(flag != 0);
        const int lane = tid & 63, wave = tid >> 6;
        int* wc = s_scan + ((base / POSE_THREADS) & 1) * 4;
        if (lane == 0) wc[wave] = __popcll(bm);
        __syncthreads();
        int before = 0, tot = 0;
#pragma unroll
        for (int w = 0; w < POSE_THREADS / 64; ++w) {
            before += w < wave ? wc[w] : 0;
            tot += wc[w];
        }
        const int pos = n + before + (int)__builtin_amdgcn_mbcnt_hi((uint32_t)(bm >> 32), __builtin_amdgcn_mbcnt_lo((uint32_t)bm, 0u));
        if (flag) {
            const uint32_t xy = kprev[2 * i], meta = kprev[2 * i + 1];
            const double sc = (double)(1 << (meta & 0xFF));
            const double ul = ((double)(xy & 0xFFFF) + 0.5) * sc - 0.5;
            const double vl = ((double)(xy >> 16) + 0.5) * sc - 0.5;
            const double z = cal.fxb / d;
            const double x = (ul - cx) * z / fx;
            const double y = (vl - cy) * z / fy;
            const double bx = (u - cx) / fx;
            const double by = (v - cy) / fy;
            const double nn = sqrt((bx * bx + by * by) + 1.0);
            double* cr = corr + (size_t)pos * TS_CORR_DOUBLES;
            cr[0] = x; cr[1] = y; cr[2] = z; cr[3] = cx - u; cr[4] = cy - v;
            cr[5] = bx / nn; cr[6] = by / nn; cr[7] = 1.0 / nn;
        }
        n += tot;
    }
    if (tid == 0) write_stats(sout, n < max(6, c.pp.min_inliers) ? 1 : 3, n, 0, 0, -1, g);
}

__global__ __launch_bounds__(POSE_THREADS) void k_p3p(BatchCtx c) {
    TS_BACK_PRIO;
    const int H = c.pp.n_hyp;
    const int gid = blockIdx.x * POSE_THREADS + threadIdx.x;
    if (gid >= c.n * c.npair * H) return;
    const int fl = gid / H, h = gid - fl * H;
    const int p = c.pair0 + fl % c.npair;
    const int f = fl / c.npair;
    const int fp = f * c.P + p;
    const int64_t g = c.g0 + f;
    const int32_t* sout = c.stats + (size_t)fp * TS_STATS_INTS;
    if (sout[0] != 3) return;
    const int n = sout[1];
    const double* corr = c.corr + ((size_t)f * c.P + p) * c.g.K * TS_CORR_DOUBLES;
    const uint64_t base_rng = splitmix64(c.pp.seed ^ ((uint64_t)g * 0x9E3779B97F4A7C15ull));
    uint32_t r[3];
#pragma unroll
    for (int k = 0; k < 3; ++k) r[k] = (uint32_t)(splitmix64(base_rng ^ ((uint64_t)h * 4ull + (uint64_t)k)) >> 32);
    const uint32_t un = (uint32_t)n;
    int i0 = (int)(r[0] % un);
    int i1 = (int)(r[1] % (un - 1));
    i1 += (i1 >= i0);
    int i2 = (int)(r[2] % (un - 2));
    const int lo = min(i0, i1), hi = max(i0, i1);
    i2 += (i2 >= lo);
    i2 += (i2 >= hi);
    const int idx[3] = {i0, i1, i2};
    V3 pw[3], fb[3];
#pragma unroll
    for (int k = 0; k < 3; ++k) {
        const double* cr = corr + (size_t)idx[k] * TS_CORR_DOUBLES;
        pw[k] = {cr[0], cr[1], cr[2]};
        fb[k] = {cr[5], cr[6], cr[7]};
// ... 996 lines not shown
```

thor-slam_amd/csrc/k_reloc.hip:

```cpp
#include "tslam_common.h"

#define RL_CHUNK 512

__global__ __launch_bounds__(256) void k_reloc_match(BatchCtx c, RelocQuery qi, const uint32_t* map_desc, int M_arg,
                                                     const int32_t* dM, int32_t* match) {
    __shared__ uint4 s_d[RL_CHUNK][2];
    const int K = c.g.K;
    const int M = dM ? *dM : M_arg;
    const int q = blockIdx.x * blockDim.x + threadIdx.x;
    bool valid = false;
    uint32_t d[8] = {0, 0, 0, 0, 0, 0, 0, 0};
    if (q < K) {
        const uint32_t meta = qi.kps[(size_t)q * 2 + 1];
        const int l = (int)(meta & 0xFF);
        valid = q - c.g.koff[l] < qi.kcount[l];
        const uint4* src = reinterpret_cast<const uint4*>(qi.desc + (size_t)q * 8);
        const uint4 a = src[0], b = src[1];
        d[0] = a.x; d[1] = a.y; d[2] = a.z; d[3] = a.w; d[4] = b.x; d[5] = b.y; d[6] = b.z; d[7] = b.w;
    }
    uint32_t best = 0xFFFFFFFFu, second = 0xFFFFFFFFu;
    for (int m0 = 0; m0 < M; m0 += RL_CHUNK) {
        const int nm = min(RL_CHUNK, M - m0);
        __syncthreads();
        for (int i = threadIdx.x; i < nm * 2; i += blockDim.x)
// ... 21 lines not shown
        const uint32_t bd = best >> 20, sd = second >> 20;
        if ((int)bd <= c.mp.max_hamming && (second == 0xFFFFFFFFu || 100u * bd < (uint32_t)c.mp.ratio_pct * sd))
            out = (int)(best & 0xFFFFFu);
    }
    match[q] = out;
}

__global__ __launch_bounds__(256) void k_reloc_corr(BatchCtx c, RelocQuery qi, int pair, const double* map_xyz,
                                                    const double* xf, const int32_t* match, double* corr, int32_t* stats,
                                                    double* pose, int64_t frame) {
    __shared__ int s_tmp[32];
    const int K = c.g.K;
    for (int i = threadIdx.x; i < TS_POSE_DOUBLES; i += blockDim.x) pose[i] = (i < 16 && (i % 5) == 0) ? 1.0 : 0.0;
    const PairCalib cal = c.calib[pair];
    const double fx = cal.fx, fy = cal.fy, cx = cal.cx, cy = cal.cy;
    int n = 0;
    for (int base = 0; base < K; base += blockDim.x) {
        const int q = base + threadIdx.x;
        const int m = q < K ? match[q] : -1;
        const int flag = m >= 0;
        const int lane = threadIdx.x & 63, wave = threadIdx.x >> 6;
        int x = flag;
        for (int o = 1; o < 64; o <<= 1) {
            const int y = __shfl_up(x, o, 64);
            if (lane >= o) x += y;
        }
        if (lane == 63) s_tmp[wave] = x;
        __syncthreads();
        int off = 0, tot = 0;
        for (int w = 0; w < (int)(blockDim.x >> 6); ++w) {
            if (w < wave) off += s_tmp[w];
            tot += s_tmp[w];
        }
        if (flag) {
            const uint32_t xy = qi.kps[(size_t)q * 2], meta = qi.kps[(size_t)q * 2 + 1];
            const double sc = (double)(1 << (meta & 0xFF));
            const double u = ((double)(xy & 0xFFFF) + 0.5) * sc - 0.5;
            const double v = ((double)(xy >> 16) + 0.5) * sc - 0.5;
            const double bx = (u - cx) / fx;
            const double by = (v - cy) / fy;
            const double nn = sqrt((bx * bx + by * by) + 1.0);
            double* cr = corr + (size_t)(n + off + x - flag) * TS_CORR_DOUBLES;
            const double X = map_xyz[(size_t)m * 3], Y = map_xyz[(size_t)m * 3 + 1], Z = map_xyz[(size_t)m * 3 + 2];
            if (xf) {
                for (int e = 0; e < 3; ++e) cr[e] = ((xf[4 * e] * X + xf[4 * e + 1] * Y) + xf[4 * e + 2] * Z) + xf[4 * e + 3];
            } else {
                cr[0] = X;
                cr[1] = Y;
                cr[2] = Z;
            }
            cr[3] = cx - u;
            cr[4] = cy - v;
            cr[5] = bx / nn;
            cr[6] = by / nn;
            cr[7] = 1.0 / nn;
        }
        n += tot;
        __syncthreads();
    }
    if (threadIdx.x == 0) {
        stats[0] = n < max(6, c.pp.min_inliers) ? 1 : 3;
        stats[1] = n;
        stats[2] = stats[3] = stats[6] = stats[7] = 0;
        stats[4] = -1;
        stats[5] = (int)frame;
    }
}

void launch_reloc(const BatchCtx& c, int pair, int64_t frame, const double* map_xyz, const uint32_t* map_desc, int M,
                  int32_t* match, double* corr, int32_t* stats, double* pose, double* ransac, double* hyp, hipStream_t s) {
    launch_reloc_query(c, pair, frame, reloc_query_ring(c, c.cpp * pair, frame), map_xyz, map_desc, M, nullptr, match, corr,
                       stats, pose, ransac, hyp, s);
}

void launch_reloc_query(const BatchCtx& c, int pair, int64_t frame, RelocQuery q, const double* map_xyz,
                        const uint32_t* map_desc, int M, const int32_t* dM, int32_t* match, double* corr, int32_t* stats,
                        double* pose, double* ransac, double* hyp, hipStream_t s) {
    hipLaunchKernelGGL(k_reloc_match, dim3((c.g.K + 255) / 256), dim3(256), 0, s, c, q, map_desc, M, dM, match);
    hipLaunchKernelGGL(k_reloc_corr, dim3(1), dim3(256), 0, s, c, q, pair, map_xyz, (const double*)nullptr, match,
                       corr, stats, pose, frame);
    BatchCtx r = c;
    r.n = 1;
    r.P = 1;
    r.pair0 = 0;
    r.npair = 1;
    r.g0 = frame;
    r.prior = nullptr;
    r.rig_prior = nullptr;
    r.calib[0] = c.calib[pair];
    r.corr = corr;
    r.stats = stats;
    r.pose = pose;
    r.ransac = ransac;
    r.hyp = hyp;
    launch_pose_solve(r, s);
}

void launch_reloc_rig(const BatchCtx& c, int64_t frame, const double* map_xyz, const uint32_t* map_desc, int M,
                      int32_t* match, double* corr, int32_t* stats, double* pose, double* ransac, double* hyp,
                      double* rig_pose, int32_t* rig_stats, hipStream_t s) {
    const int K = c.g.K;
    for (int p = 0; p < c.P; ++p) {
        int32_t* mp = match + (size_t)p * K;
        const RelocQuery q = reloc_query_ring(c, c.cpp * p, frame);
        hipLaunchKernelGGL(k_reloc_match, dim3((K + 255) / 256), dim3(256), 0, s, c, q, map_desc, M, (const int32_t*)nullptr,
                           mp);
        hipLaunchKernelGGL(k_reloc_corr, dim3(1), dim3(256), 0, s, c, q, p, map_xyz, c.rig_Einv + 16 * p, mp,
                           corr + (size_t)p * K * TS_CORR_DOUBLES, stats + (size_t)p * TS_STATS_INTS,
                           pose + (size_t)p * TS_POSE_DOUBLES, frame);
    }
    BatchCtx r = c;
    r.n = 1;
    r.pair0 = 0;
    r.npair = c.P;
    r.g0 = frame;
    r.corr = corr;
    r.stats = stats;
    r.pose = pose;
    r.ransac = ransac;
    r.hyp = hyp;
    r.prior = nullptr;
    r.rig_prior = nullptr;
    r.rig_pose = rig_pose;
    r.rig_stats = rig_stats;
    r.reloc = 1;
    launch_pose_solve(r, s);
    launch_rig_pose(r, s);
}
```

thor-slam_amd/csrc/k_rgbd.hip:

```cpp
#include "tslam_common.h"

__global__ __launch_bounds__(256) void k_rgbd_gray(BatchCtx c, uint8_t* gray) {
    const int img = blockIdx.y;
    const size_t npx = (size_t)c.W * c.H;
    const uint8_t* src = c.rgbd_in + (size_t)img * npx * 5;
    uint8_t* dst = gray + (size_t)img * npx;
    const size_t i = (size_t)blockIdx.x * blockDim.x + threadIdx.x;
    if ((npx & 3) == 0) {
        if (4 * i >= npx) return;
        const uint32_t* s32 = reinterpret_cast<const uint32_t*>(src) + 3 * i;
        const uint32_t w0 = s32[0], w1 = s32[1], w2 = s32[2];
        const uint8_t px[12] = {(uint8_t)w0, (uint8_t)(w0 >> 8), (uint8_t)(w0 >> 16), (uint8_t)(w0 >> 24),
                                (uint8_t)w1, (uint8_t)(w1 >> 8), (uint8_t)(w1 >> 16), (uint8_t)(w1 >> 24),
                                (uint8_t)w2, (uint8_t)(w2 >> 8), (uint8_t)(w2 >> 16), (uint8_t)(w2 >> 24)};
        uint32_t out = 0;
#pragma unroll
        for (int k = 0; k < 4; ++k) {
            const uint32_t b = px[3 * k], g = px[3 * k + 1], r = px[3 * k + 2];
            out |= ((r * 4899u + g * 9617u + b * 1868u + 8192u) >> 14) << (8 * k);
        }
        reinterpret_cast<uint32_t*>(dst)[i] = out;
    } else {
        for (size_t k = 4 * i; k < 4 * i + 4 && k < npx; ++k) {
            const uint32_t b = src[3 * k], g = src[3 * k + 1], r = src[3 * k + 2];
            dst[k] = (uint8_t)((r * 4899u + g * 9617u + b * 1868u + 8192u) >> 14);
        }
    }
}

__global__ __launch_bounds__(256) void k_rgbd_depth(BatchCtx c) {
    const int K = c.g.K;
    const int fl = blockIdx.y, p = c.pair0 + fl % c.npair, f = fl / c.npair;
    const int k = blockIdx.x * blockDim.x + threadIdx.x;
    if (k >= K) return;
    const int slot = ring_slot(c, c.g0 + f);
    const size_t ib = (size_t)slot * c.C + p;
    const uint32_t* kp = c.kps + (ib * K + k) * 2;
    const int l = (int)(kp[1] & 0xFF);
    const bool valid = k - c.g.koff[l] < c.kcount[ib * c.g.n_levels + l];
    double disp = __builtin_nan("");
    if (valid) {
        const double sc = (double)(1 << l);
        const double u = ((double)(kp[0] & 0xFFFF) + 0.5) * sc - 0.5;
        const double v = ((double)(kp[0] >> 16) + 0.5) * sc - 0.5;
        int ix = min(max((int)floor(u + 0.5), 0), c.W - 1);
        int iy = min(max((int)floor(v + 0.5), 0), c.H - 1);
        if (c.maps && ((c.map_mask >> p) & 1u)) {
            const int32_t* m = c.maps + (((size_t)p * c.H + iy) * c.W + ix) * 2;
            ix = min(max((m[0] + 16) >> 5, 0), c.W - 1);
            iy = min(max((m[1] + 16) >> 5, 0), c.H - 1);
        }
        const size_t npx = (size_t)c.W * c.H;
        const uint16_t* depth = reinterpret_cast<const uint16_t*>(c.rgbd_in + ((size_t)f * c.ncam + (p - c.cam0)) * npx * 5 + npx * 3);
        const uint32_t mm = depth[(size_t)iy * c.W + ix];
        if (mm) disp = c.calib[p].fx / ((double)mm * 0.001);
    }
    const size_t o = ((size_t)slot * c.P + p) * K + k;
    c.disp[o] = disp;
    c.stereo[o] = __builtin_isfinite(disp) ? k : -1;
}

void launch_rgbd_gray(const BatchCtx& c, uint8_t* gray, hipStream_t s) {
    const size_t groups = ((size_t)c.W * c.H + 3) / 4;
    hipLaunchKernelGGL(k_rgbd_gray, dim3((unsigned)((groups + 255) / 256), c.n * c.ncam), dim3(256), 0, s, c, gray);
}

void launch_rgbd_depth(const BatchCtx& c, hipStream_t s) {
    hipLaunchKernelGGL(k_rgbd_depth, dim3((c.g.K + 255) / 256, c.n * c.npair), dim3(256), 0, s, c);
}
```

thor-slam_amd/csrc/tslam_api.cpp:

```cpp
#include <algorithm>
#include <cmath>
#include <cstring>

#include "tslam_describe.h"
#include "tslam_handle.h"
#include "tslam_tables.h"

static thread_local std::string g_err;

int fail(int code, const std::string& msg) {
    g_err = msg;
    return code;
}

int tslam_internal_fail(int code, const char* msg) { return fail(code, msg); }

int dev_alloc(tslam_handle* h, void** p, size_t bytes) {
    if (bytes == 0) bytes = 16;
    hipError_t e = hipMalloc(p, bytes);
    if (e != hipSuccess) return fail(TSLAM_ENOMEM, std::string("hipMalloc failed: ") + hipGetErrorString(e));
    h->allocs.push_back(*p);
    HIPCHK(hipMemset(*p, 0, bytes));
    HIPCHK(hipDeviceSynchronize());
    return TSLAM_OK;
// ... 27 lines not shown
    h->host_allocs.push_back(*p);
    *cap = bytes;
    return TSLAM_OK;
}

static void free_all(tslam_handle* h) {
    if (h->drv && h->drv_owned) tslam_internal_driver_destroy(h->drv);
    h->drv = nullptr;
    for (void* p : h->allocs) (void)hipFree(p);
    h->allocs.clear();
    for (void* p : h->host_allocs) (void)hipHostFree(p);
    h->host_allocs.clear();
}

static void build_geometry(tslam_handle* h) {
    LevelGeom& g = h->g;
    const tslam_params& p = h->prm;
    g.n_levels = p.n_levels;
    g.K = p.n_features;
    int w = h->W, hh = h->H, off = 0;
    double tot = 0.0;
    for (int l = 0; l < p.n_levels; ++l) tot += std::pow(0.25, l);
    int sumq = 0;
    for (int l = 0; l < p.n_levels; ++l) {
        g.W[l] = w;
        g.H[l] = hh;
        g.pyr_off[l] = off;
        off += w * hh;
        w >>= 1;
        hh >>= 1;
        g.Kq[l] = (int)((double)p.n_features * std::pow(0.25, l) / tot);
        if (l > 0) sumq += g.Kq[l];
    }
    g.Kq[0] = p.n_features - sumq;
    g.pyr_bytes = (off + 15) & ~15;
    int ko = 0, bs = 0, co = 0, qs = 0;
    const int br0 = (2 * TS_BAND_ROWS_MAX + 10) * g.W[0] <= 48 * 1024 ? TS_BAND_ROWS_MAX
                  : (2 * 24 + 10) * g.W[0] <= 78 * 1024 ? 24 : 16;
    const int det_budget = (2 * br0 + 10) * g.W[0];
    g.det_lds = 0;
    for (int l = 0; l < p.n_levels; ++l) {
        const int maxr = l == 0 ? br0 : std::max(br0, std::min(124, (det_budget / g.W[l] - 10) / 2));
        const int nb = (g.H[l] + maxr - 1) / maxr;
        g.band_rows[l] = l == 0 ? br0 : ((g.H[l] + nb - 1) / nb + 1) & ~1;
        g.smooth_groups[l] = std::max(2, g.band_rows[l] / 16);
        g.det_lds = std::max(g.det_lds, (2 * g.band_rows[l] + 10) * g.W[l]);
    }
    g.dt_total = 0;
    for (int l = 0; l < p.n_levels; ++l) {
        g.koff[l] = ko;
        ko += g.Kq[l];
        g.nbands[l] = (g.H[l] + g.band_rows[l] - 1) / g.band_rows[l];
        g.band_start[l] = bs;
        bs += g.nbands[l];
        g.cand_cap[l] = ((g.band_rows[l] + 1) / 2) * (g.W[l] / 2 + 1);
        g.cand_off[l] = co;
        co += g.nbands[l] * g.cand_cap[l];
        g.dt_nx[l] = (g.W[l] - p.edge_margin + TS_DT_W - 1) / TS_DT_W;
        g.dt_start[l] = g.dt_total;
        g.dt_total += g.dt_nx[l] * ((g.H[l] - p.edge_margin + TS_DT_H - 1) / TS_DT_H);
        g.qtiles[l] = (g.Kq[l] + 127) / 128;
        g.qtile_start[l] = qs;
        qs += g.qtiles[l];
    }
    g.total_bands = bs;
    g.cand_total = co;
    g.total_qtiles = qs;
    int ro = 0;
    for (int l = 0; l < p.n_levels; ++l) {
        g.rs_off[l] = ro;
        ro += g.H[l] + 1;
    }
    g.rs_total = (ro + 7) & ~7;
}

BatchCtx make_ctx(tslam_handle* h) {
    BatchCtx c{};
    c.g = h->g;
    c.C = h->C;
    c.P = h->P;
    c.B = h->B;
    c.R = h->R;
    c.n = h->cur_n;
    c.g0 = h->cur_g0;
    c.W = h->W;
    c.H = h->H;
    c.cpp = h->prm.rgbd ? 1 : 2;
    c.rgbd = h->prm.rgbd;
    c.images = h->prm.rgbd ? h->d_gray : h->cur_images;
    c.rgbd_in = h->prm.rgbd ? h->cur_images : nullptr;
    c.maps = h->d_maps;
    c.map_mask = h->map_mask;
    c.pyr = (uint8_t*)h->buf[TSLAM_BUF_PYRAMID].ptr;
    c.smo = (uint8_t*)h->buf[TSLAM_BUF_SMOOTH].ptr;
    c.cand = h->d_cand;
    c.ccount = h->d_ccount;
    c.hist = h->d_hist;
    c.kps = (uint32_t*)h->buf[TSLAM_BUF_KEYPOINTS].ptr;
    c.kcount = (int32_t*)h->buf[TSLAM_BUF_KCOUNT].ptr;
    c.desc = (uint32_t*)h->buf[TSLAM_BUF_DESC].ptr;
    c.ys = (uint4*)h->buf[TSLAM_BUF_YSORTED].ptr;
    c.desc_ys = (uint32_t*)h->buf[TSLAM_BUF_DESC_YS].ptr;
    c.rowstart = (uint16_t*)h->buf[TSLAM_BUF_ROWSTART].ptr;
    c.qbest = (uint32_t*)h->buf[TSLAM_BUF_QBEST].ptr;
    c.qsecond = (uint32_t*)h->buf[TSLAM_BUF_QSECOND].ptr;
    c.tbest = (uint32_t*)h->buf[TSLAM_BUF_TBEST].ptr;
    c.ypos = (uint16_t*)h->buf[TSLAM_BUF_YPOS].ptr;
    c.qtpos = (uint16_t*)h->buf[TSLAM_BUF_QTPOS].ptr;
    c.stereo = (int32_t*)h->buf[TSLAM_BUF_STEREO].ptr;
    c.disp = (double*)h->buf[TSLAM_BUF_DISP].ptr;
    c.temporal = (int32_t*)h->buf[TSLAM_BUF_TEMPORAL].ptr;
    c.tuv = (double*)h->buf[TSLAM_BUF_TEMPORAL_UV].ptr;
    c.corr = (double*)h->buf[TSLAM_BUF_CORR].ptr;
    c.pose = (double*)h->buf[TSLAM_BUF_POSE].ptr;
    c.stats = (int32_t*)h->buf[TSLAM_BUF_STATS].ptr;
    c.state = h->d_state;
    c.prior = h->prior_armed ? h->d_prior + (size_t)(h->batch_idx & 1) * TS_PRIOR_DOUBLES * h->P * h->B : nullptr;
    c.rig_E = h->d_rig_E;
    c.rig_Einv = h->d_rig_E ? h->d_rig_E + 16 * h->rig_q : nullptr;
    c.rig_pose = h->d_rig_pose;
    c.rig_stats = h->d_rig_stats;
    c.rig_state = h->d_rig_state;
    c.rig_prior = (h->prior_armed && h->d_rig_prior) ? h->d_rig_prior + (size_t)(h->batch_idx & 1) * TS_PRIOR_DOUBLES * h->B
                                                     : nullptr;
    c.ransac = h->d_ransac;
    c.hyp = h->d_hyp;
    c.det_thr = (const uint32_t*)h->buf[TSLAM_BUF_DET_THR].ptr;
    c.det_thr_acc = h->d_det_thr_acc;
    c.det_fail = (uint32_t*)h->buf[TSLAM_BUF_DET_FAIL].ptr;
    c.brief_table = h->d_brief;
    c.wedges = h->d_wedges;
    for (int p = 0; p < h->P; ++p) c.calib[p] = h->calib[p];
    c.mp.max_hamming = h->prm.max_hamming;
    c.mp.ratio_pct = h->prm.ratio_pct;
    c.mp.row_tol = h->prm.stereo_row_tol;
    c.mp.max_disp = h->prm.max_disparity;
    c.mp.window = h->prm.temporal_window;
    c.mp.refine_split = h->prm.match_refine;
    c.mp.merge_cap = h->match_mode == 1 ? 0 : h->match_cap > 0 ? std::min(h->match_cap, TS_MTB) : TS_MTB;
    c.match_cnt = h->d_match_cnt;
    c.det_cnt = h->d_det_cnt;
    c.pp.n_hyp = h->prm.ransac_hypotheses;
    c.pp.iters = h->prm.refine_iters;
    c.pp.min_inliers = h->prm.min_inliers;
    c.pp.splits = h->prm.ransac_splits;
    c.pp.mode = h->prm.ransac_mode;
    c.pp.refine_block = h->prm.refine_block;
    c.pp.thr2 = h->prm.ransac_thr_px * h->prm.ransac_thr_px;
    c.pp.seed = h->prm.ransac_seed;
    c.fast_threshold = h->prm.fast_threshold;
    c.margin = h->prm.edge_margin;
    c.cam0 = h->sh_cam_lo;
    c.ncam = h->sh_cam_hi - h->sh_cam_lo;
    c.pair0 = 0;
    c.npair = h->P;
    c.match_modes = 3;
    c.reloc = 0;
    c.peer_S = c.peer_me = c.peer_nbuf = c.peer_skip = 0;
    return c;
}

int run_front_stage(tslam_handle* h, const BatchCtx& c, int stage, hipStream_t s) {
    switch (stage) {
        case TSLAM_STAGE_RECTIFY:
        case TSLAM_KERNEL_RECTIFY_PYRAMID:
            if (h->prm.rgbd) launch_rgbd_gray(c, h->d_gray, s);
            launch_rectify_pyramid(c, s);
            return 1;
        case TSLAM_STAGE_DETECT: launch_detect(c, s); launch_select(c, s, h->sel_mode, h->sel_rcap); return 1;
        case TSLAM_KERNEL_DETECT: launch_detect(c, s); return 1;
        case TSLAM_KERNEL_SELECT: launch_select(c, s, h->sel_mode, h->sel_rcap); return 1;
        case TSLAM_STAGE_DESCRIBE:
        case TSLAM_KERNEL_DESCRIBE: launch_describe(c, s); return 1;
        default: return 0;
    }
}

int run_back_stage(tslam_handle* h, const BatchCtx& c, const BackView& v, int stage, hipStream_t s) {
    switch (stage) {
        case TSLAM_STAGE_MATCH:
            if (v.pre) launch_match_stereo(*v.pre, s);
            if (v.b) {
                launch_match(*v.b, s);
                launch_match_refine(*v.b, s);
            }
            return 1;
        case TSLAM_KERNEL_MATCH:
            if (v.pre) launch_match_stereo(*v.pre, s);
            if (v.b) launch_match(*v.b, s);
            return 1;
        case TSLAM_KERNEL_MATCH_REFINE:
            if (v.b) launch_match_refine(*v.b, s);
            return 1;
        case TSLAM_STAGE_POSE:
            if (v.b) launch_pose(*v.b, s);
            if (v.pose_rig && h->rig && v.rig) launch_rig_pose(*v.rig, s);
            if (v.pose_chain) {
                launch_chains(c, h->rig, s);
                loop_auto_store(h, c, s);
            }
            return 1;
        case TSLAM_KERNEL_POSE:
            if (v.b) launch_pose(*v.b, s);
            return 1;
        case TSLAM_KERNEL_RIG:
            if (!h->rig) return fail(TSLAM_ESTATE, "no rig set (tslam_set_rig)");
            if (v.rig) launch_rig_pose(*v.rig, s);
            return 1;
        case TSLAM_KERNEL_CHAIN: launch_chains(c, h->rig, s); return 1;
        default: return 0;
    }
}

extern "C" {

const char* tslam_last_error(void) { return g_err.c_str(); }

int tslam_abi_version(void) { return TSLAM_ABI_VERSION; }

int tslam_create(const tslam_stereo_desc* pairs, const tslam_params* params, int device, tslam_handle** out) {
    if (!pairs || !params || !out) return fail(TSLAM_EINVAL, "null argument");
    const tslam_params& p = *params;
    if (p.n_pairs < 1 || p.n_pairs > 8) return fail(TSLAM_EINVAL, "n_pairs must be in [1, 8]");
    if (p.n_levels < 1 || p.n_levels > TS_MAX_LEVELS) return fail(TSLAM_EINVAL, "n_levels must be in [1, 6]");
    if (p.n_features < 1 || p.n_features > 8192) return fail(TSLAM_EINVAL, "n_features must be in [1, 8192]");
    if (p.ransac_hypotheses < 1 || p.ransac_hypotheses > 256) return fail(TSLAM_EINVAL, "ransac_hypotheses must be in [1, 256]");
    if (p.edge_margin < 19) return fail(TSLAM_EINVAL, "edge_margin must be >= 19");
    if (p.fast_threshold < 0 || p.fast_threshold > 254) return fail(TSLAM_EINVAL, "fast_threshold must be in [0, 254]");
    if (p.max_batch < 1) return fail(TSLAM_EINVAL, "max_batch must be >= 1");
    if (p.max_hamming < 0 || p.max_hamming > 253) return fail(TSLAM_EINVAL, "max_hamming must be in [0, 253]");
    if (p.stereo_row_tol < 0 || p.stereo_row_tol > 2047 || p.max_disparity < 0 || p.max_disparity > 2047 ||
        p.temporal_window < 0 || p.temporal_window > 2047)
        return fail(TSLAM_EINVAL, "stereo_row_tol, max_disparity, temporal_window must be in [0, 2047]");
    if (!(p.ba_window == 0 || (p.ba_window >= 2 && p.ba_window <= TS_BA_MAXW)))
        return fail(TSLAM_EINVAL, "ba_window must be 0 (off) or in [2, 10]");
    if (p.ba_window && (p.ba_kf_interval < 1 || p.ba_iters < 1 || !(p.ba_lambda >= 0.0) || !(p.ba_outlier_px > 0.0)))
        return fail(TSLAM_EINVAL, "ba_kf_interval, ba_iters >= 1, ba_lambda >= 0, ba_outlier_px > 0");
    if (p.refine_iters < 1) return fail(TSLAM_EINVAL, "refine_iters must be >= 1");
// ... 3 lines not shown
        return fail(TSLAM_EINVAL, "refine_block must be 0, 128 or 256");
    if (p.match_refine != 0 && p.match_refine != 1) return fail(TSLAM_EINVAL, "match_refine must be 0 or 1");
    const int W = pairs[0].width, H = pairs[0].height;
    if (W < 64 || H < 64 || W > 2047 || H > 2047) return fail(TSLAM_EINVAL, "image size must be within [64, 2047]");
    for (int i = 1; i < p.n_pairs; ++i)
        if (pairs[i].width != W || pairs[i].height != H) return fail(TSLAM_EINVAL, "all pairs must share the image size");
    if ((H >> (p.n_levels - 1)) < 2 * p.edge_margin + 3 || (W >> (p.n_levels - 1)) < 2 * p.edge_margin + 3)
        return fail(TSLAM_EINVAL, "coarsest pyramid level smaller than 2*edge_margin+3");
    for (int i = 0; i < p.n_pairs; ++i)
        if (!(p.rgbd || pairs[i].baseline > 0.0) || !(pairs[i].fx > 0.0) || !(pairs[i].fy > 0.0))
            return fail(TSLAM_EINVAL, "pair calibration needs fx, fy, baseline > 0");
    if (p.rgbd != 0 && p.rgbd != 1) return fail(TSLAM_EINVAL, "rgbd must be 0 or 1");
    if (p.rgbd && ((W * H) & 1)) return fail(TSLAM_EINVAL, "RGB-D needs an even pixel count (u16 depth alignment)");

    hipError_t e = hipSetDevice(device);
    if (e != hipSuccess) return fail(TSLAM_EHIP, std::string("hipSetDevice: ") + hipGetErrorString(e));

    tslam_handle* h = new tslam_handle();
    h->device = device;
    h->prm = p;
    h->W = W;
    h->H = H;
    h->P = p.n_pairs;
    h->C = (p.rgbd ? 1 : 2) * p.n_pairs;
    h->B = p.max_batch;
    h->sh_cam_hi = h->C;
    h->R = 2 * p.max_batch + 1;
    if (p.ba_window) h->R = 2 * p.max_batch + p.ba_kf_interval + 1;
    build_geometry(h);
    for (int i = 0; i < h->P; ++i) {
        h->calib[i].fx = pairs[i].fx;
        h->calib[i].fy = pairs[i].fy;
        h->calib[i].cx = pairs[i].cx;
        h->calib[i].cy = pairs[i].cy;
        h->calib[i].fxb = pairs[i].fx * (p.rgbd ? 1.0 : pairs[i].baseline);
    }

    const int64_t K = p.n_features, C = h->C, P = h->P, B = h->B, R = h->R, L = p.n_levels;
    struct Spec {
        int which;
        int64_t frames;
        int64_t per_frame;
    } specs[] = {
        {TSLAM_BUF_PYRAMID, R, C * h->g.pyr_bytes},
        {TSLAM_BUF_SMOOTH, B, C * h->g.pyr_bytes},
        {TSLAM_BUF_KEYPOINTS, R, C * K * 2 * 4},
        {TSLAM_BUF_KCOUNT, R, C * L * 4},
        {TSLAM_BUF_DESC, R, C * K * 8 * 4},
        {TSLAM_BUF_STEREO, R, P * K * 4},
        {TSLAM_BUF_DISP, R, P * K * 8},
        {TSLAM_BUF_TEMPORAL, R, P * K * 4},
        {TSLAM_BUF_TEMPORAL_UV, B, P * K * 2 * 8},
        {TSLAM_BUF_CORR, B, P * K * TS_CORR_DOUBLES * 8},
        {TSLAM_BUF_POSE, B, P * TS_POSE_DOUBLES * 8},
        {TSLAM_BUF_STATS, B, P * TS_STATS_INTS * 4},
        {TSLAM_BUF_QBEST, B, P * 2 * K * 4},
        {TSLAM_BUF_QSECOND, B, P * 2 * K * 4},
        {TSLAM_BUF_TBEST, B, P * 2 * K * 4},
        {TSLAM_BUF_YSORTED, R, C * K * 16},
        {TSLAM_BUF_DESC_YS, R, C * K * 8 * 4},
        {TSLAM_BUF_ROWSTART, R, C * (int64_t)h->g.rs_total * 2},
        {TSLAM_BUF_DET_THR, 1, C * L * 4},
        {TSLAM_BUF_DET_FAIL, B, C * L * 4},
        {TSLAM_BUF_YPOS, R, C * K * 2},
        {TSLAM_BUF_QTPOS, B, P * 2 * K * 2},
        {TSLAM_BUF_HYP, B, P * 4 * (int64_t)p.ransac_hypotheses * TS_HYP_DOUBLES * 8},
    };
    int rc = TSLAM_OK;
    for (const Spec& s : specs) {
        Buffer& b = h->buf[s.which];
        b.per_frame = s.per_frame;
        b.bytes = s.per_frame * s.frames;
        if ((rc = dev_alloc(h, &b.ptr, (size_t)b.bytes)) != TSLAM_OK) break;
    }
    if (rc == TSLAM_OK) rc = dev_alloc(h, (void**)&h->d_cand, sizeof(uint32_t) * (size_t)B * C * h->g.cand_total);
    if (rc == TSLAM_OK) rc = dev_alloc(h, (void**)&h->d_ccount, sizeof(uint32_t) * (size_t)B * C * h->g.total_bands);
    if (rc == TSLAM_OK) rc = dev_alloc(h, (void**)&h->d_hist, sizeof(uint32_t) * (size_t)B * C * L * 256);
    if (rc == TSLAM_OK) rc = dev_alloc(h, (void**)&h->d_det_thr_acc, sizeof(uint32_t) * (size_t)C * L);
    if (rc == TSLAM_OK) rc = dev_alloc(h, (void**)&h->d_state, sizeof(double) * 32 * (size_t)P);
    if (rc == TSLAM_OK) rc = dev_alloc(h, (void**)&h->d_ransac, sizeof(uint32_t) * TS_RANSAC_WORDS * TS_MAX_SPLITS * (size_t)B * P);
    if (rc == TSLAM_OK) h->d_hyp = (double*)h->buf[TSLAM_BUF_HYP].ptr;
    if (rc == TSLAM_OK) rc = dev_alloc(h, (void**)&h->d_brief, sizeof(TSLAM_BRIEF_TABLE));
    if (rc == TSLAM_OK) rc = dev_alloc(h, (void**)&h->d_wedges, sizeof(TSLAM_WEDGES));
    if (rc == TSLAM_OK) rc = dev_alloc(h, (void**)&h->d_maps, sizeof(int32_t) * (size_t)C * W * H * 2);
    if (rc == TSLAM_OK && p.ba_window) rc = alloc_ba(h);
    if (rc == TSLAM_OK && p.rgbd) rc = dev_alloc(h, (void**)&h->d_gray, (size_t)B * P * W * H);
    if (rc != TSLAM_OK) {
        free_all(h);
        delete h;
        return rc;
    }
    std::vector<uint32_t> brief_off(30 * 256);
    for (int i = 0; i < 30 * 256; ++i) {
        const uint32_t t = TSLAM_BRIEF_TABLE[i];
        const int px = (int8_t)(t & 0xFF), py = (int8_t)((t >> 8) & 0xFF);
        const int qx = (int8_t)((t >> 16) & 0xFF), qy = (int8_t)(t >> 24);
        brief_off[i] = (uint32_t)((py + 18) * TS_DT_P + px + 18) | ((uint32_t)((qy + 18) * TS_DT_P + qx + 18) << 16);
    }
    bool ok = hipMemcpy(h->d_brief, brief_off.data(), sizeof(uint32_t) * brief_off.size(), hipMemcpyHostToDevice) == hipSuccess &&
              hipMemcpy(h->d_wedges, TSLAM_WEDGES, sizeof(TSLAM_WEDGES), hipMemcpyHostToDevice) == hipSuccess;
    for (int i = 0; i < h->P && ok; ++i) {
        const int32_t* m[2] = {pairs[i].map_left, pairs[i].map_right};
        const int cpp = p.rgbd ? 1 : 2;
        for (int s = 0; s < cpp; ++s) {
            if (!m[s]) continue;
            h->map_mask |= 1u << (cpp * i + s);
            ok = ok && hipMemcpy(h->d_maps + (size_t)(cpp * i + s) * W * H * 2, m[s], sizeof(int32_t) * (size_t)W * H * 2,
                                 hipMemcpyHostToDevice) == hipSuccess;
        }
    }
    if (!ok) {
        free_all(h);
        delete h;
        return fail(TSLAM_EHIP, "uploading tables / maps failed");
    }
    if (tslam_reset(h) != TSLAM_OK) {
        free_all(h);
        delete h;
        return TSLAM_EHIP;
    }
    *out = h;
    return TSLAM_OK;
}

int tslam_destroy(tslam_handle* h) {
    if (!h) return TSLAM_OK;
    (void)ba_flush(h);
    loop_worker_stop(h);
    (void)hipSetDevice(h->device);
    (void)hipDeviceSynchronize();
    loop_destroy(h);
    for (hipEvent_t e : {h->ev_front, h->ev_back[0], h->ev_back[1], h->ev_prior[0], h->ev_prior[1], h->as_staged[0],
                         h->as_staged[1], h->as_res[0].ev, h->as_res[1].ev})
        if (e) (void)hipEventDestroy(e);
    for (hipStream_t st : {h->as_front, h->as_back, h->as_ba})
        if (st) (void)hipStreamDestroy(st);
    ba_destroy(h);
    register_destroy(h);
    free_all(h);
    delete h;
    return TSLAM_OK;
}

int tslam_reset(tslam_handle* h) {
    if (!h) return fail(TSLAM_EINVAL, "null handle");
    BA_FLUSH(h);
    loop_worker_drain(h);
    HIPCHK(hipSetDevice(h->device));
    HIPCHK(hipDeviceSynchronize());
    std::vector<double> eye(32 * (size_t)h->P, 0.0);
    for (int q = 0; q < 2 * h->P; ++q)
        for (int k = 0; k < 4; ++k) eye[(size_t)q * 16 + 5 * k] = 1.0;
    HIPCHK(hipMemcpy(h->d_state, eye.data(), sizeof(double) * eye.size(), hipMemcpyHostToDevice));
    if (h->d_rig_state) HIPCHK(hipMemcpy(h->d_rig_state, eye.data(), sizeof(double) * 32, hipMemcpyHostToDevice));
    h->frames_done = 0;
    HIPCHK(hipMemset(h->buf[TSLAM_BUF_DET_THR].ptr, 0, sizeof(uint32_t) * (size_t)h->C * h->g.n_levels));
    HIPCHK(hipMemset(h->d_det_thr_acc, 0xFF, sizeof(uint32_t) * (size_t)h->C * h->g.n_levels));
    int rc = ba_reset(h);
    if (rc == TSLAM_OK) rc = dense_reset(h);
    if (rc == TSLAM_OK) rc = loop_reset(h);
    if (rc != TSLAM_OK) return rc;
    h->back_pending[0] = h->back_pending[1] = false;
    h->in_batch = false;
    h->cur_n = 0;
    for (auto& r : h->as_res) r.pending = false;
    h->as_last_pose_batch = h->as_batches - 1;
    HIPCHK(hipDeviceSynchronize());
    return TSLAM_OK;
}

static int64_t host_frame_bytes(const tslam_handle* h) {
    return h->prm.rgbd ? (int64_t)h->P * 5 * h->W * h->H : (int64_t)h->C * h->W * h->H;
}

static int ensure_result_slots(tslam_handle* h) {
    if (h->as_res[0].ev) return TSLAM_OK;
    const size_t B = h->B, P = h->P;
    for (int k = 0; k < 2; ++k) {
        auto& r = h->as_res[k];
        const size_t bytes[4] = {8 * B * P * TS_POSE_DOUBLES, 4 * B * P * TS_STATS_INTS, 8 * B * TS_POSE_DOUBLES,
                                 4 * B * TS_STATS_INTS};
        void** dst[4] = {(void**)&r.pose, (void**)&r.stats, (void**)&r.rig_pose, (void**)&r.rig_stats};
        for (int i = 0; i < 4; ++i) {
// ... 534 lines not shown
```

thor-slam_amd/csrc/tslam_api_exchange.cpp:

```cpp
#include "tslam_handle.h"

static BatchCtx range_ctx(const BatchCtx& c, int lo, int hi) {
    BatchCtx r = c;
    const size_t P = c.P, K = c.g.K, f = lo;
    r.g0 = c.g0 + lo;
    r.n = hi - lo;
    r.qbest += f * P * 2 * K;
    r.qsecond += f * P * 2 * K;
    r.tbest += f * P * 2 * K;
    r.qtpos += f * P * 2 * K;
    r.tuv += f * P * K * 2;
    r.corr += f * P * K * TS_CORR_DOUBLES;
    r.pose += f * P * TS_POSE_DOUBLES;
    r.stats += f * P * TS_STATS_INTS;
    r.ransac += f * P * TS_MAX_SPLITS * TS_RANSAC_WORDS / 2;
    r.hyp += f * P * 4 * (size_t)c.pp.n_hyp * TS_HYP_DOUBLES;
    if (r.prior) r.prior += f * P * TS_PRIOR_DOUBLES;
    if (r.rig_prior) r.rig_prior += f * TS_PRIOR_DOUBLES;
    if (r.rig_pose) r.rig_pose += f * TS_POSE_DOUBLES;
    if (r.rig_stats) r.rig_stats += f * TS_STATS_INTS;
    return r;
}

static void shard_range(const tslam_handle* h, int n, int* lo, int* hi) {
    peer_range(rig_slot(h->sh_rank, h->sh_world, h->sh_pairs), n, h->sh_world, lo, hi);
}
static void pair_half(const tslam_handle* h, int n, int* lo, int* hi) { peer_range(h->sh_cam_lo & 1, n, 2, lo, hi); }

static int run_sharded_rgbd_stage(tslam_handle* h, const BatchCtx& c, int stage, hipStream_t s) {
    int lo, hi;
    shard_range(h, c.n, &lo, &hi);
    BatchCtx own = c;
    own.pair0 = h->sh_cam_lo;
    own.npair = h->sh_cam_hi - h->sh_cam_lo;
    const BatchCtx cr = range_ctx(c, lo, hi);
    const BackView v{&own, nullptr, hi > lo ? &cr : nullptr, false, false};
    int rc = run_front_stage(h, c, stage, s);
    if (rc == 0) rc = run_back_stage(h, c, v, stage, s);
    if (rc < 0) return rc;
    if (rc == 0)
        return fail(TSLAM_ESTATE, "a camera-sharded RGB-D handle runs its stages one by one: RECTIFY..DESCRIBE, "
                                  "MATCH, POSE, pack/exchange/unpack pairs, KERNEL_RIG, pose records, CHAIN");
    HIPCHK(hipGetLastError());
    return TSLAM_OK;
}

int run_sharded_stage(tslam_handle* h, const BatchCtx& c, int stage, hipStream_t s) {
    if (h->prm.rgbd) return run_sharded_rgbd_stage(h, c, stage, s);
    int lo, hi;
    if (h->sh_pairs) pair_half(h, c.n, &lo, &hi);
    else shard_range(h, c.n, &lo, &hi);
    BatchCtx cb = range_ctx(c, lo, hi);
    const bool empty = hi <= lo;
    const bool pre = !empty && c.g0 + lo - 1 >= 0;
    BatchCtx cp = c;
    cp.g0 = c.g0 + lo - 1;
    cp.n = 1;
    BatchCtx cr = c;
    BackView v{empty ? nullptr : &cb, pre ? &cp : nullptr, empty ? nullptr : &cb, true, false};
    if (h->sh_pairs) {
        cb.pair0 = cp.pair0 = h->sh_cam_lo / 2;
        cb.npair = cp.npair = 1;
        int rl, rh;
        shard_range(h, c.n, &rl, &rh);
        cr = range_ctx(c, rl, rh);
        v.rig = rh > rl ? &cr : nullptr;
        v.pose_rig = false;
    }
    int rc = run_front_stage(h, c, stage, s);
    if (rc == 0) rc = run_back_stage(h, c, v, stage, s);
    if (rc < 0) return rc;
    if (rc == 0) {
        if (stage == TSLAM_STAGE_BA) return ba_stage(h, c, s);
        return fail(TSLAM_ESTATE, "a sharded handle runs its stages one by one around the exchange "
                                  "(RECTIFY..DESCRIBE, pack/exchange/unpack, MATCH, POSE, exchange, CHAIN)");
    }
    HIPCHK(hipGetLastError());
    return TSLAM_OK;
}

extern "C" {

int tslam_set_shard(tslam_handle* h, int cam_lo, int cam_hi, int rank, int world) {
    if (!h) return fail(TSLAM_EINVAL, "null handle");
    BA_FLUSH(h);
    if (h->in_batch) return fail(TSLAM_ESTATE, "tslam_set_shard inside a batch");
    if (cam_lo < 0 || cam_hi > h->C || cam_lo >= cam_hi) return fail(TSLAM_EINVAL, "camera range outside [0, cameras)");
    if (world < 1 || rank < 0 || rank >= world || world > h->B) return fail(TSLAM_EINVAL, "need 0 <= rank < world <= max_batch");
    if (world > 1 && h->prm.ba_window && h->prm.rgbd)
        return fail(TSLAM_EINVAL, "a camera-sharded RGB-D rig runs without local BA");
    h->sh_cam_lo = cam_lo;
    h->sh_cam_hi = cam_hi;
    h->sh_rank = rank;
    h->sh_world = world;
    h->sh_pairs = false;
    return TSLAM_OK;
}

int tslam_exchange_sizes(tslam_handle* h, int64_t* stream_block, int64_t* pose_record) {
    if (!h) return fail(TSLAM_EINVAL, "null handle");
    if (stream_block) *stream_block = stream_block_bytes(h->g);
    if (pose_record) *pose_record = pose_record_bytes(h->P);
    return TSLAM_OK;
}

static int check_frames_cams(tslam_handle* h, int64_t first_frame, int n_frames, int cam_lo, int cam_hi) {
    if (n_frames < 1 || n_frames > h->R) return fail(TSLAM_EINVAL, "n_frames must be in [1, ring]");
    if (cam_lo < 0 || cam_hi > h->C || cam_lo >= cam_hi) return fail(TSLAM_EINVAL, "camera range outside [0, cameras)");
    if (first_frame + n_frames < 0) return fail(TSLAM_EINVAL, "frame range before the sequence start");
    return TSLAM_OK;
}

int tslam_pack_streams(tslam_handle* h, int64_t first_frame, int n_frames, int cam_lo, int cam_hi, void* dst, void* stream) {
    if (!h || !dst) return fail(TSLAM_EINVAL, "bad argument");
    int rc = check_frames_cams(h, first_frame, n_frames, cam_lo, cam_hi);
    if (rc != TSLAM_OK) return rc;
    HIPCHK(hipSetDevice(h->device));
    launch_stream_blocks(make_ctx(h), true, first_frame, n_frames, cam_lo, cam_hi - cam_lo, (uint8_t*)dst, (hipStream_t)stream);
    HIPCHK(hipGetLastError());
    return TSLAM_OK;
}

int tslam_unpack_streams(tslam_handle* h, int64_t first_frame, int n_frames, int cam_lo, int cam_hi, const void* src,
                         void* stream) {
    if (!h || !src) return fail(TSLAM_EINVAL, "bad argument");
    int rc = check_frames_cams(h, first_frame, n_frames, cam_lo, cam_hi);
    if (rc != TSLAM_OK) return rc;
    HIPCHK(hipSetDevice(h->device));
    launch_stream_blocks(make_ctx(h), false, first_frame, n_frames, cam_lo, cam_hi - cam_lo, (uint8_t*)src, (hipStream_t)stream);
    HIPCHK(hipGetLastError());
    return TSLAM_OK;
}

int tslam_import_raw(tslam_handle* h, const uint8_t* images, int64_t first_frame, int n_frames, int cam_lo, int cam_hi,
                     void* stream) {
    if (!h || !images) return fail(TSLAM_EINVAL, "bad argument");
    int rc = check_frames_cams(h, first_frame, n_frames, cam_lo, cam_hi);
    if (rc != TSLAM_OK) return rc;
    if (h->prm.rgbd) return fail(TSLAM_EINVAL, "tslam_import_raw takes gray stereo images");
    HIPCHK(hipSetDevice(h->device));
    BatchCtx c = make_ctx(h);
    const int ncam = cam_hi - cam_lo;
    const int64_t skip = first_frame < 0 ? -first_frame : 0;
    c.images = images + (size_t)skip * ncam * h->W * h->H;
    c.g0 = first_frame + skip;
    c.n = (int)(n_frames - skip);
    c.cam0 = cam_lo;
    c.ncam = ncam;
    launch_rectify_pyramid(c, (hipStream_t)stream);
    HIPCHK(hipGetLastError());
    return TSLAM_OK;
}

int tslam_pair_block_bytes(tslam_handle* h, int64_t* bytes) {
    if (!h || !bytes) return fail(TSLAM_EINVAL, "bad argument");
    *bytes = pair_block_bytes(h->g);
    return TSLAM_OK;
}

static int pair_blocks(tslam_handle* h, bool pack, int f0, int n_frames, int pair_lo, int pair_hi, uint8_t* buf, void* stream) {
    if (!h || !buf) return fail(TSLAM_EINVAL, "bad argument");
    if (!h->in_batch) return fail(TSLAM_ESTATE, "pair blocks are packed / unpacked inside a batch");
    if (f0 < 0 || n_frames < 1 || f0 + n_frames > h->cur_n) return fail(TSLAM_EINVAL, "frame range outside the batch");
    if (pair_lo < 0 || pair_hi > h->P || pair_lo >= pair_hi) return fail(TSLAM_EINVAL, "pair range outside [0, pairs)");
    HIPCHK(hipSetDevice(h->device));
    launch_pair_blocks(make_ctx(h), pack, f0, n_frames, pair_lo, pair_hi - pair_lo, buf, (hipStream_t)stream);
    HIPCHK(hipGetLastError());
    return TSLAM_OK;
}

int tslam_pack_pairs(tslam_handle* h, int f0, int n_frames, int pair_lo, int pair_hi, void* dst, void* stream) {
    return pair_blocks(h, true, f0, n_frames, pair_lo, pair_hi, (uint8_t*)dst, stream);
}

int tslam_unpack_pairs(tslam_handle* h, int f0, int n_frames, int pair_lo, int pair_hi, const void* src, void* stream) {
    return pair_blocks(h, false, f0, n_frames, pair_lo, pair_hi, (uint8_t*)src, stream);
}

int tslam_internal_info(tslam_handle* h, tslam_handle_info* o) {
    if (!h || !o) return fail(TSLAM_EINVAL, "bad argument");
    o->device = h->device;
    o->W = h->W;
    o->H = h->H;
    o->P = h->P;
    o->C = h->C;
    o->B = h->B;
    o->rgbd = h->prm.rgbd;
    o->rig = h->rig ? 1 : 0;
    o->ba = h->prm.ba_window;
    o->frames_done = h->frames_done;
    o->stream_block = stream_block_bytes(h->g);
    o->pose_record = pose_record_bytes(h->P);
    o->pair_block = pair_block_bytes(h->g);
    o->state_range = state_range_block_bytes(h->g);
    o->state_camera = state_camera_block_bytes(h->g);
    o->cam_lo = h->sh_cam_lo;
    o->cam_hi = h->sh_cam_hi;
    o->rank = h->sh_rank;
    o->world = h->sh_world;
    return TSLAM_OK;
}

int tslam_internal_attach_driver(tslam_handle* h, tslam_shard_driver* d, bool owned) {
    if (!h) return fail(TSLAM_EINVAL, "null handle");
    if (h->drv && h->drv_owned && h->drv != d) tslam_internal_driver_destroy(h->drv);
    h->drv = d;
    h->drv_owned = d && owned;
    h->sh_comm = d != nullptr;
    return TSLAM_OK;
}

tslam_shard_driver* tslam_internal_driver(tslam_handle* h) { return h ? h->drv : nullptr; }

int tslam_internal_state_blocks(tslam_handle* h, int pack, int rank, int cam_lo, int cam_hi, void* buf, void* stream) {
    if (!h || !buf) return fail(TSLAM_EINVAL, "bad argument");
    if (!h->in_batch) return fail(TSLAM_ESTATE, "state blocks are packed / unpacked inside a batch");
    if (h->prm.rgbd) return fail(TSLAM_ESTATE, "state blocks describe a stereo rig");
    HIPCHK(hipSetDevice(h->device));
    launch_state_blocks(make_ctx(h), pack != 0, h->cur_n, h->sh_world, rank, cam_lo, cam_hi, (uint8_t*)buf,
                        (hipStream_t)stream);
    HIPCHK(hipGetLastError());
    return TSLAM_OK;
}

int tslam_perturb_temporal(tslam_handle* h, int percent, uint64_t seed, void* stream) {
    if (!h) return fail(TSLAM_EINVAL, "null handle");
    BA_FLUSH(h);
    if (!h->in_batch) return fail(TSLAM_ESTATE, "tslam_perturb_temporal inside a batch (after MATCH_REFINE)");
    if (percent < 0 || percent > 100) return fail(TSLAM_EINVAL, "percent must be in [0, 100]");
    if (h->sh_world > 1 || h->sh_comm) return fail(TSLAM_ESTATE, "tslam_perturb_temporal takes an unsharded handle");
    HIPCHK(hipSetDevice(h->device));
    if (percent > 0) launch_perturb_uv(make_ctx(h), percent, seed, (hipStream_t)stream);
    HIPCHK(hipGetLastError());
    return TSLAM_OK;
}

static int check_peers(tslam_handle* h) {
    if (!h) return fail(TSLAM_EINVAL, "null handle");
    if (!h->in_batch) return fail(TSLAM_ESTATE, "peer exchange blocks are packed / imported inside a batch");
    if (h->sh_world < 2 || h->prm.rgbd) return fail(TSLAM_ESTATE, "a stereo handle sharded over world > 1");
    if ((h->sh_cam_hi - h->sh_cam_lo) * h->sh_world != h->C || h->sh_cam_lo != h->sh_rank * (h->sh_cam_hi - h->sh_cam_lo))
        return fail(TSLAM_EINVAL, "peer layout needs cameras [rank*S, (rank+1)*S)");
    return TSLAM_OK;
}
static XGeom peers_geom(tslam_handle* h) {
    tslam_handle_info in{};
    (void)tslam_internal_info(h, &in);
    return tslam_xgeom(in, h->sh_world, h->cur_n, false, false);
}

int tslam_pack_streams_peers(tslam_handle* h, void* dst, void* stream) {
    int rc = check_peers(h);
    if (rc != TSLAM_OK) return rc;
    if (!dst) return fail(TSLAM_EINVAL, "null buffer");
    HIPCHK(hipSetDevice(h->device));
    const XGeom g = peers_geom(h);
    launch_stream_blocks_peers(make_ctx(h), true, h->cur_g0, g.n, g.world, xp_slot_frames(g), h->sh_rank, g.S, (uint8_t*)dst,
                               (hipStream_t)stream);
    HIPCHK(hipGetLastError());
    return TSLAM_OK;
}

int tslam_stage_raw_peers(tslam_handle* h, const uint8_t* prev_raw, void* dst, void* stream) {
    int rc = check_peers(h);
    if (rc != TSLAM_OK) return rc;
    if (!prev_raw || !dst) return fail(TSLAM_EINVAL, "null buffer");
    HIPCHK(hipSetDevice(h->device));
    const XGeom g = peers_geom(h);
    launch_stage_raw_peers(h->cur_images, prev_raw, (uint8_t*)dst, g.n, g.world, xp_slot_frames(g), h->sh_rank, g.S,
                           (int64_t)g.img, (hipStream_t)stream);
    HIPCHK(hipGetLastError());
    return TSLAM_OK;
}

int tslam_import_peers(tslam_handle* h, const uint8_t* raw, const void* streams, void* stream) {
    int rc = check_peers(h);
    if (rc != TSLAM_OK) return rc;
    if (!raw || !streams) return fail(TSLAM_EINVAL, "null buffer");
    HIPCHK(hipSetDevice(h->device));
    const XGeom g = peers_geom(h);
    int lo;
    const int nr = xp_back_frames(g, h->sh_rank, &lo);
    if (nr == 0) return TSLAM_OK;
    const int64_t first = h->cur_g0 + lo - 1;
    const int skip = first < 0 ? 1 : 0;
    BatchCtx c = make_ctx(h);
    c.images = raw;
    c.g0 = first + skip;
    c.n = nr - skip;
    c.peer_S = g.S;
    c.peer_me = h->sh_rank;
    c.peer_nbuf = xp_slot_frames(g);
    c.peer_skip = skip;
    if (c.n > 0) launch_rectify_pyramid(c, (hipStream_t)stream);
    launch_stream_blocks_peers(make_ctx(h), false, h->cur_g0, g.n, g.world, xp_slot_frames(g), h->sh_rank, g.S,
                               (uint8_t*)streams, (hipStream_t)stream);
    HIPCHK(hipGetLastError());
    return TSLAM_OK;
}

int tslam_internal_set_pairs(tslam_handle* h, int on) {
    if (!h) return fail(TSLAM_EINVAL, "null handle");
    if (h->in_batch) return fail(TSLAM_ESTATE, "the pair split is set outside a batch");
    if (on) {
        if (h->prm.rgbd) return fail(TSLAM_EINVAL, "the pair split shards a stereo rig");
        if (h->sh_world < 2 || h->sh_world != h->C || h->sh_cam_hi - h->sh_cam_lo != 1 || h->sh_cam_lo != h->sh_rank)
            return fail(TSLAM_EINVAL, "the pair split needs one camera per rank (world = cameras)");
        if (h->prm.ba_window) return fail(TSLAM_EINVAL, "the pair split runs without local BA (no state gather)");
    }
    h->sh_pairs = on != 0;
    return TSLAM_OK;
}

static int check_partner(tslam_handle* h) {
    if (!h) return fail(TSLAM_EINVAL, "null handle");
    if (!h->in_batch) return fail(TSLAM_ESTATE, "partner blocks are packed / imported inside a batch");
    if (!h->sh_pairs) return fail(TSLAM_ESTATE, "the handle is not pair-split (TSLAM_SHARD_PAIRS)");
    return TSLAM_OK;
}

int tslam_internal_pack_partner(tslam_handle* h, void* dst, void* stream) {
    int rc = check_partner(h);
    if (rc != TSLAM_OK) return rc;
    if (!dst) return fail(TSLAM_EINVAL, "null buffer");
    HIPCHK(hipSetDevice(h->device));
    int lo, hi;
    peer_range((h->sh_cam_lo & 1) ^ 1, h->cur_n, 2, &lo, &hi);
    if (hi > lo)
        launch_stream_blocks(make_ctx(h), true, h->cur_g0 + lo - 1, hi - lo + 1, h->sh_cam_lo, 1, (uint8_t*)dst,
                             (hipStream_t)stream);
    HIPCHK(hipGetLastError());
    return TSLAM_OK;
}

int tslam_internal_import_partner(tslam_handle* h, const uint8_t* raw, const void* streams, void* stream) {
    int rc = check_partner(h);
    if (rc != TSLAM_OK) return rc;
    if (!raw || !streams) return fail(TSLAM_EINVAL, "null buffer");
    HIPCHK(hipSetDevice(h->device));
    int lo, hi;
    pair_half(h, h->cur_n, &lo, &hi);
    if (hi <= lo) return TSLAM_OK;
    const int partner = h->sh_cam_lo ^ 1, nf = hi - lo + 1;
    const int64_t first = h->cur_g0 + lo - 1;
    const int skip = first < 0 ? 1 : 0;
    BatchCtx c = make_ctx(h);
    c.images = raw + (size_t)skip * h->W * h->H;
    c.g0 = first + skip;
    c.n = nf - skip;
    c.cam0 = partner;
    c.ncam = 1;
    if (c.n > 0) launch_rectify_pyramid(c, (hipStream_t)stream);
    launch_stream_blocks(make_ctx(h), false, first, nf, partner, 1, (uint8_t*)streams, (hipStream_t)stream);
    HIPCHK(hipGetLastError());
    return TSLAM_OK;
}

int tslam_pack_poses(tslam_handle* h, void* dst, void* stream) {
    if (!h || !dst) return fail(TSLAM_EINVAL, "bad argument");
    if (!h->in_batch) return fail(TSLAM_ESTATE, "tslam_pack_poses inside a batch (after its POSE stage)");
    HIPCHK(hipSetDevice(h->device));
    int lo, hi;
    shard_range(h, h->cur_n, &lo, &hi);
    launch_pose_records(make_ctx(h), true, lo, hi - lo, (uint8_t*)dst, (hipStream_t)stream);
    HIPCHK(hipGetLastError());
    return TSLAM_OK;
}

int tslam_unpack_poses(tslam_handle* h, const void* src, void* stream) {
    if (!h || !src) return fail(TSLAM_EINVAL, "bad argument");
    if (!h->in_batch) return fail(TSLAM_ESTATE, "tslam_unpack_poses inside a batch (before its CHAIN stage)");
    HIPCHK(hipSetDevice(h->device));
    launch_pose_records_gathered(make_ctx(h), h->sh_world, h->sh_pairs, (const uint8_t*)src, (hipStream_t)stream);
    HIPCHK(hipGetLastError());
    return TSLAM_OK;
}

}
```

thor-slam_amd/csrc/tslam_common.h:

```cpp
#pragma once

#include <hip/hip_runtime.h>
#include <stdint.h>

#define TS_MAX_LEVELS 6
#define TS_DCNT 12
#define TS_DCNT_BLOCKS 9
#define TS_BAND_ROWS_MAX 32
#define TS_DET_HALO 4
#define TS_RECT_BAND 32
#define TS_MATCH_CHUNK 512
#define TS_MTB 896
#define TS_SAD_HALF 5
#define TS_SAD_RANGE 2
#define TS_POSE_DOUBLES 68
#define TS_STATS_INTS 8
#define TS_CORR_DOUBLES 8
#define TS_MAX_HYP 1024
#define TS_HYP_DOUBLES 20
#define TS_MAX_SPLITS 32
#define TS_RANSAC_WORDS 26
#define TS_PRIOR_DOUBLES 16
#define TS_BA_CU_RESERVE 96
#define TS_BACK_PRIO __builtin_amdgcn_s_setprio(2)
#define TS_BA_MAXW 10

struct LevelGeom {
    int n_levels;
    int W[TS_MAX_LEVELS], H[TS_MAX_LEVELS];
    int pyr_off[TS_MAX_LEVELS];
    int pyr_bytes;
    int K;
    int Kq[TS_MAX_LEVELS], koff[TS_MAX_LEVELS];
    int band_rows[TS_MAX_LEVELS];
    int smooth_groups[TS_MAX_LEVELS];
    int det_lds;
    int nbands[TS_MAX_LEVELS], band_start[TS_MAX_LEVELS];
    int total_bands;
    int cand_cap[TS_MAX_LEVELS];
    int cand_off[TS_MAX_LEVELS];
    int cand_total;
    int qtiles[TS_MAX_LEVELS], qtile_start[TS_MAX_LEVELS];
    int total_qtiles;
    int rs_off[TS_MAX_LEVELS];
    int rs_total;
    int dt_nx[TS_MAX_LEVELS], dt_start[TS_MAX_LEVELS];
    int dt_total;
};

struct PairCalib {
    double fx, fy, cx, cy, fxb;
};

struct MatchParams {
    int max_hamming, ratio_pct, row_tol, max_disp, window;
    int refine_split;
    int merge_cap;
};

struct PoseParams {
    int n_hyp, iters, min_inliers, splits;
    int mode;
    int refine_block;
    double thr2;
    uint64_t seed;
};

struct BatchCtx {
    LevelGeom g;
    int C, P, B, R;
    int cpp;
    int rgbd;
    int n;
    int cam0, ncam;
    int pair0, npair;
    int match_modes;
    int reloc;
    int peer_S, peer_me, peer_nbuf, peer_skip;
    int64_t g0;
    int W, H;
    const uint8_t* images;
    const uint8_t* rgbd_in;
    const int32_t* maps;
    uint32_t map_mask;
    uint8_t* pyr;
    uint8_t* smo;
    uint32_t* cand;
    uint32_t* ccount;
    uint32_t* hist;
    uint32_t* kps;
    int32_t* kcount;
    uint32_t* desc;
    uint4* ys;
    uint32_t* desc_ys;
    uint16_t* rowstart;
    uint32_t* qbest;
    uint32_t* qsecond;
    uint32_t* tbest;
    uint16_t* ypos;
    uint16_t* qtpos;
    int32_t* stereo;
    double* disp;
    int32_t* temporal;
    double* tuv;
    double* corr;
    double* pose;
    double* ransac;
    double* hyp;
    int32_t* stats;
    double* state;
    const double* prior;
    const double* rig_E;
    const double* rig_Einv;
    double* rig_pose;
    int32_t* rig_stats;
    double* rig_state;
    double* rig_prior;
    const uint32_t* det_thr;
    uint32_t* det_thr_acc;
    uint32_t* det_fail;
    uint32_t* match_cnt;
    uint32_t* det_cnt;

    const uint32_t* brief_table;
    const int64_t* wedges;
    PairCalib calib[8];
    MatchParams mp;
    PoseParams pp;
    int fast_threshold, margin;
};

static inline __host__ __device__ int ring_slot(const BatchCtx& c, int64_t g) { return (int)(g % c.R); }

#include "tslam_ranges.h"
__device__ __forceinline__ void view_image(const BatchCtx& c, int img, int* f, int* cam) {
    if (c.peer_S) {
        const int per = c.n * c.peer_S, qq = img / per, q = qq < c.peer_me ? qq : qq + 1;
        const int r = img - qq * per;
        *f = r / c.peer_S;
        *cam = q * c.peer_S + (r - *f * c.peer_S);
        return;
    }
    *f = img / c.ncam;
    *cam = c.cam0 + (img - *f * c.ncam);
}
__device__ __forceinline__ size_t view_src(const BatchCtx& c, int img) {
    if (c.peer_S) {
        const int per = c.n * c.peer_S, qq = img / per, q = qq < c.peer_me ? qq : qq + 1;
        const int r = img - qq * per, f = r / c.peer_S;
        return ((size_t)q * c.peer_nbuf + c.peer_skip + f) * c.peer_S + (r - f * c.peer_S);
    }
    return (size_t)img;
}

void launch_rectify_pyramid(const BatchCtx& c, hipStream_t s);
void launch_detect(const BatchCtx& c, hipStream_t s);
void launch_select(const BatchCtx& c, hipStream_t s, int mode, int rcap);
void launch_describe(const BatchCtx& c, hipStream_t s);
void launch_match(const BatchCtx& c, hipStream_t s);
int match_blocks_per_cu();
void launch_match_refine(const BatchCtx& c, hipStream_t s);
void launch_match_stereo(const BatchCtx& c, hipStream_t s);
void launch_pose(const BatchCtx& c, hipStream_t s);
void launch_chains(const BatchCtx& c, bool rig, hipStream_t s);
void launch_rig_pose(const BatchCtx& c, hipStream_t s);
int64_t stream_block_bytes(const LevelGeom& g);
int64_t pose_record_bytes(int P);
void launch_stream_blocks(const BatchCtx& c, bool pack, int64_t first, int n_frames, int cam_lo, int ncam, uint8_t* blk,
                          hipStream_t s);
void launch_stream_blocks_peers(const BatchCtx& c, bool pack, int64_t g0, int n, int world, int cap, int me, int S,
                                uint8_t* blk, hipStream_t s);
void launch_stage_raw_peers(const uint8_t* images, const uint8_t* prev, uint8_t* dst, int n, int world, int cap, int me,
                            int S, int64_t img_bytes, hipStream_t s);
void launch_pose_records(const BatchCtx& c, bool pack, int f0, int n, uint8_t* rec, hipStream_t s);
void launch_pose_records_gathered(const BatchCtx& c, int world, bool pairs, const uint8_t* rec, hipStream_t s);
int64_t state_range_block_bytes(const LevelGeom& g);
int64_t state_camera_block_bytes(const LevelGeom& g);
void launch_state_blocks(const BatchCtx& c, bool pack, int n, int world, int rank, int cam_lo, int cam_hi, uint8_t* blk,
                         hipStream_t s);
int64_t pair_block_bytes(const LevelGeom& g);
void launch_pair_blocks(const BatchCtx& c, bool pack, int f0, int n_frames, int p0, int np, uint8_t* blk, hipStream_t s);
void launch_pose_solve(const BatchCtx& c, hipStream_t s);
void launch_perturb_uv(const BatchCtx& c, int percent, uint64_t seed, hipStream_t s);
void launch_reloc(const BatchCtx& c, int pair, int64_t frame, const double* map_xyz, const uint32_t* map_desc, int M,
                  int32_t* match, double* corr, int32_t* stats, double* pose, double* ransac, double* hyp, hipStream_t s);
void launch_reloc_rig(const BatchCtx& c, int64_t frame, const double* map_xyz, const uint32_t* map_desc, int M,
                      int32_t* match, double* corr, int32_t* stats, double* pose, double* ransac, double* hyp,
                      double* rig_pose, int32_t* rig_stats, hipStream_t s);
struct RelocQuery {
    const uint32_t* kps;
    const int32_t* kcount;
    const uint32_t* desc;
};
static inline RelocQuery reloc_query_ring(const BatchCtx& c, int cam, int64_t frame) {
    const size_t ib = (size_t)ring_slot(c, frame) * c.C + cam;
    return {c.kps + ib * c.g.K * 2, c.kcount + ib * c.g.n_levels, c.desc + ib * c.g.K * 8};
}
void launch_reloc_query(const BatchCtx& c, int pair, int64_t frame, RelocQuery q, const double* map_xyz,
                        const uint32_t* map_desc, int M, const int32_t* dM, int32_t* match, double* corr, int32_t* stats,
                        double* pose, double* ransac, double* hyp, hipStream_t s);
struct LoopDb {
    double* xyz;
    uint32_t* desc;
    int32_t* n;
    uint32_t* snap_kps;
    int32_t* snap_kcount;
    uint32_t* snap_desc;
};
void launch_loop_store(const BatchCtx& c, int pair, int64_t frame, double* xyz, uint32_t* desc, int32_t* n_out,
                       hipStream_t s);
void launch_loop_store_auto(const BatchCtx& c, int interval, const LoopDb& db, int capk, bool rig, int64_t* count,
                            hipStream_t s);
void launch_loop_vote(const uint32_t* db_desc, const int32_t* db_n, int K, int S, int q_slot, int64_t k0, int capk, int P,
                      int n_cand, int max_hamming, int ratio_pct, int32_t* votes, hipStream_t s);
void launch_pose_graph_iteration(double* T, const int32_t* edges, const double* Z, const double* info, int N, int E,
                                 const int32_t* adj_off, const int32_t* adj, const int32_t* ftile, double* terms,
                                 double* H, double* g, double* delta, double* Ld, hipStream_t s);
void pose_graph_test_delay(int spins);
void launch_pose_graph_cost(const double* T, const int32_t* edges, const double* Z, const double* info, int E,
                            double* terms, double* cost, hipStream_t s);
#define TSDF_MAX_FRAMES 256
#define TSDF_POSE 13
struct TsdfArgs {
    float* tsdf;
    float* weight;
    int nx, ny, nz;
// ... 200 lines not shown
    return v;
}

__device__ __forceinline__ uint32_t wave_min_dpp(uint32_t v) {
    v = min(v, (uint32_t)__builtin_amdgcn_mov_dpp((int)v, 0xB1, 0xF, 0xF, false));
    v = min(v, (uint32_t)__builtin_amdgcn_mov_dpp((int)v, 0x4E, 0xF, 0xF, false));
    v = min(v, (uint32_t)__builtin_amdgcn_mov_dpp((int)v, 0x141, 0xF, 0xF, false));
    v = min(v, (uint32_t)__builtin_amdgcn_mov_dpp((int)v, 0x140, 0xF, 0xF, false));
    const uint32_t a = (uint32_t)__builtin_amdgcn_readlane((int)v, 0), b = (uint32_t)__builtin_amdgcn_readlane((int)v, 16);
    const uint32_t c = (uint32_t)__builtin_amdgcn_readlane((int)v, 32), d = (uint32_t)__builtin_amdgcn_readlane((int)v, 48);
    return min(min(a, b), min(c, d));
}

__device__ __forceinline__ int wave_sum_dpp(int v) {
    v += __builtin_amdgcn_update_dpp(0, v, 0xB1, 0xF, 0xF, true);
    v += __builtin_amdgcn_update_dpp(0, v, 0x4E, 0xF, 0xF, true);
    v += __builtin_amdgcn_update_dpp(0, v, 0x141, 0xF, 0xF, true);
    v += __builtin_amdgcn_update_dpp(0, v, 0x140, 0xF, 0xF, true);
    v += __builtin_amdgcn_update_dpp(0, v, 0x142, 0xA, 0xF, false);
    v += __builtin_amdgcn_update_dpp(0, v, 0x143, 0xC, 0xF, false);
    return __builtin_amdgcn_readlane(v, 63);
}

__device__ __forceinline__ double dpp_f64(double v, int ctrl_sel) {
    const uint64_t b = __builtin_bit_cast(uint64_t, v);
    int lo = (int)(uint32_t)b, hi = (int)(uint32_t)(b >> 32);
    switch (ctrl_sel) {
        case 0: lo = __builtin_amdgcn_mov_dpp(lo, 0xB1, 0xF, 0xF, false); hi = __builtin_amdgcn_mov_dpp(hi, 0xB1, 0xF, 0xF, false); break;
        case 1: lo = __builtin_amdgcn_mov_dpp(lo, 0x4E, 0xF, 0xF, false); hi = __builtin_amdgcn_mov_dpp(hi, 0x4E, 0xF, 0xF, false); break;
        case 2: lo = __builtin_amdgcn_mov_dpp(lo, 0x141, 0xF, 0xF, false); hi = __builtin_amdgcn_mov_dpp(hi, 0x141, 0xF, 0xF, false); break;
        default: lo = __builtin_amdgcn_mov_dpp(lo, 0x140, 0xF, 0xF, false); hi = __builtin_amdgcn_mov_dpp(hi, 0x140, 0xF, 0xF, false); break;
    }
    return __builtin_bit_cast(double, ((uint64_t)(uint32_t)hi << 32) | (uint32_t)lo);
}
template <int CTRL>
__device__ __forceinline__ double dpp_f64c(double v) {
    const uint64_t b = __builtin_bit_cast(uint64_t, v);
    const int lo = __builtin_amdgcn_mov_dpp((int)(uint32_t)b, CTRL, 0xF, 0xF, false);
    const int hi = __builtin_amdgcn_mov_dpp((int)(uint32_t)(b >> 32), CTRL, 0xF, 0xF, false);
    return __builtin_bit_cast(double, ((uint64_t)(uint32_t)hi << 32) | (uint32_t)lo);
}
__device__ __forceinline__ double readlane_f64(double v, int lane) {
    const uint64_t b = __builtin_bit_cast(uint64_t, v);
    const uint32_t lo = (uint32_t)__builtin_amdgcn_readlane((int)(uint32_t)b, lane);
    const uint32_t hi = (uint32_t)__builtin_amdgcn_readlane((int)(uint32_t)(b >> 32), lane);
    return __builtin_bit_cast(double, ((uint64_t)hi << 32) | lo);
}
__device__ __forceinline__ double wave_sum_f64(double v) {
    v = v + dpp_f64(v, 0);
    v = v + dpp_f64(v, 1);
    v = v + dpp_f64(v, 2);
    v = v + dpp_f64(v, 3);
    return (readlane_f64(v, 0) + readlane_f64(v, 16)) + (readlane_f64(v, 32) + readlane_f64(v, 48));
}

template <int N>
__device__ __forceinline__ double wave_multi_sum(const double (&in)[N]) {
    static_assert(N <= 32, "at most 32 values");
    double v[32];
#pragma unroll
    for (int k = 0; k < 32; ++k) v[k] = k < N ? in[k] : 0.0;
    const int lane = threadIdx.x & 63;
#pragma unroll
    for (int h = 16; h >= 1; h >>= 1) {
        const int d = 2 * h;
        const bool upper = (lane & d) != 0;
#pragma unroll
        for (int j = 0; j < h; ++j) {
            const double keep = upper ? v[h + j] : v[j];
            const double send = upper ? v[j] : v[h + j];
            v[j] = keep + __shfl_xor(send, d, 64);
        }
    }
    return v[0] + __shfl_xor(v[0], 1, 64);
}

static inline __host__ int xcd_grid(int n_img, int bpi) { return ((n_img + 7) / 8) * 8 * bpi; }
__device__ __forceinline__ bool xcd_image_block(int b, int n_img, int bpi, int* img, int* local) {
    const int k = b >> 3;
    *img = (k / bpi) * 8 + (b & 7);
    *local = k % bpi;
    return *img < n_img;
}

__device__ __forceinline__ double pose_used(const BatchCtx& c, int st, int f0, int i) {
    return (st == 0 || (st == 2 && c.g0 + f0 + i == 0)) ? 1.0 : 0.0;
}

__device__ __forceinline__ const double* call_pose(const BatchCtx& c, int pair, int f0, const double* host_wTc, int i,
                                                   double* use) {
    if (host_wTc) {
        const double* T = host_wTc + 16 * (size_t)i;
        *use = __builtin_isfinite(T[0]) ? 1.0 : 0.0;
        return T;
    }
    const size_t o = (size_t)(f0 + i) * c.P + pair;
    const double* T = c.pose + o * TS_POSE_DOUBLES + 16;
    const int st = c.stats[o * TS_STATS_INTS];
    *use = pose_used(c, st, f0, i);
    return T;
}

__device__ __forceinline__ void store_cam_T_world(const double* T, double* q) {
    for (int r = 0; r < 3; ++r) {
        for (int k = 0; k < 3; ++k) q[3 * r + k] = T[4 * k + r];
        q[9 + r] = -((T[r] * T[3] + T[4 + r] * T[7]) + T[8 + r] * T[11]);
    }
}

__device__ __forceinline__ int pos_level(const LevelGeom& g, int pos) {
    int l = 0;
    while (l + 1 < g.n_levels && pos >= g.koff[l + 1]) ++l;
    return l;
}
```

thor-slam_amd/csrc/tslam_handle.h:

```cpp
#pragma once

#include <hip/hip_runtime.h>

#include <array>
#include <condition_variable>
#include <deque>
#include <functional>
#include <map>
#include <mutex>
#include <string>
#include <thread>
#include <vector>

#include "../../include/tslam.h"
#include "tslam_ba.h"
#include "tslam_common.h"
#include "tslam_internal.h"

struct Buffer {
    void* ptr = nullptr;
    int64_t bytes = 0;
    int64_t per_frame = 0;
};

struct tslam_handle {
    int device = 0;
    tslam_params prm{};
    int W = 0, H = 0, P = 0, C = 0, B = 0, R = 0;
    LevelGeom g{};
    PairCalib calib[8]{};
    uint32_t map_mask = 0;
    int32_t* d_maps = nullptr;
    uint32_t* d_brief = nullptr;
    int64_t* d_wedges = nullptr;
    uint8_t* d_gray = nullptr;
    Buffer buf[TSLAM_BUF_COUNT];
    uint32_t* d_cand = nullptr;
    uint32_t* d_ccount = nullptr;
    uint32_t* d_det_thr_acc = nullptr;
    uint32_t* d_hist = nullptr;
    double* d_state = nullptr;
    double* d_ransac = nullptr;
    double* d_hyp = nullptr;
    int64_t frames_done = 0;
    const uint8_t* cur_images = nullptr;
    int cur_n = 0;
    int64_t cur_g0 = 0;
    bool in_batch = false;
    int64_t batch_idx = 0;
    bool batch_started = false;
    hipStream_t last_stream = nullptr;
    std::vector<void*> allocs;
    std::vector<void*> host_allocs;
    hipStream_t front_stream = nullptr, back_stream = nullptr;
    bool front_started = false, back_started = false;
    hipEvent_t ev_front = nullptr, ev_back[2] = {nullptr, nullptr};
    bool back_pending[2] = {false, false};
    bool rig = false;
    int rig_q = 0, rig_cap = 0;
    double* d_rig_E = nullptr;
    double* d_rig_pose = nullptr;
    int32_t* d_rig_stats = nullptr;
    double* d_rig_state = nullptr;
    double* d_prior = nullptr;
    double* d_rig_prior = nullptr;
    hipEvent_t ev_prior[2] = {nullptr, nullptr};
    bool prior_read_armed[2] = {false, false};
    bool prior_armed = false;
    double* h_prior_pin[2] = {nullptr, nullptr};
    bool prior_copy_pending = false;
    hipStream_t as_front = nullptr, as_back = nullptr;
    hipStream_t as_ba = nullptr;
    uint8_t* as_stage[2] = {nullptr, nullptr};
    uint8_t* as_input[2] = {nullptr, nullptr};
    hipEvent_t as_staged[2] = {nullptr, nullptr};
    bool as_staged_armed[2] = {false, false};
    struct ResultSlot {
        double* pose = nullptr;
        int32_t* stats = nullptr;
        double* rig_pose = nullptr;
        int32_t* rig_stats = nullptr;
        std::vector<double> ts;
        hipEvent_t ev = nullptr;
        int64_t batch = -1, g0 = 0;
        int n = 0;
        bool pending = false;
    } as_res[2];
    int64_t as_batches = 0;
    int64_t as_last_pose_batch = -1;
    BaStore ba{};
    int64_t ba_frame[TS_BA_MAXW]{};
    int64_t ba_nkf = 0;
    int64_t ba_last = -1;
    BaTiming ba_timing{};
    bool ba_split = false;
    bool ba_defer = false;
    int sel_mode = 0, sel_rcap = 0;
    int match_mode = 0, match_cap = 0;
    uint32_t* d_match_cnt = nullptr;
    uint32_t* d_det_cnt = nullptr;
    struct {
        bool pending = false;
        BatchCtx c{};
        hipStream_t s = nullptr;
        double* snap = nullptr;
        double* snap_body = nullptr;
        int32_t* assoc = nullptr;
        int par = 0;
    } ba_job;
    std::map<std::pair<int, int64_t>, std::array<double, 10>> ba_imu;
    std::map<std::pair<int, int64_t>, std::array<double, TS_BA_INE + 3>> ba_ine;
    std::vector<std::array<double, 12>> ba_icfg;
    std::vector<std::array<uint8_t, TS_BA_MAXW>> ba_ine_slot;
    std::vector<BaArgs> ba_solved;
    struct BaGraphInst {
        hipGraph_t graph = nullptr;
        hipGraphExec_t exec = nullptr;
// ... 225 lines not shown
```

thor-slam_amd/csrc/tslam_tables.h:

```cpp
#pragma once
#include <stdint.h>

static const uint32_t TSLAM_BRIEF_TABLE[30 * 256] = {
    0xfcfafdfbu, 0xf9080604u, 0xf4020301u, 0xff010206u, 0x0003fff8u, 0xfe02f400u, 0xfc00ff04u, 0x02f501f8u,
    0x09fefbf9u, 0x00f8fdfau, 0xfe06010du, 0x0608f901u, 0xfe00fefeu, 0xfa03fefeu, 0xfbfb0d03u, 0x0a000206u,
    0xfcfffcfeu, 0x0dff03fdu, 0xfa05fd02u, 0x0201faf9u, 0x020d02feu, 0xfd01fffcu, 0xf3060b01u, 0xfe00f7feu,
    0xf80d0601u, 0xf3010300u, 0x01f503fbu, 0x0105fd05u, 0xfdfa060du, 0x0304fb08u, 0x0307f902u, 0xf5fb04f9u,
    0xfbfc05fbu, 0xfafcfbfau, 0x00050602u, 0xfcf6f900u, 0x02fc0b00u, 0x0405060bu, 0xfdfeff04u, 0x05060a08u,
    0x08fa0201u, 0xfa010108u, 0xfb0900f5u, 0x0409fdfau, 0xfa000d05u, 0x03f9fbfau, 0xff05fa02u, 0x000206fdu,
    0xf900f805u, 0x020c0302u, 0x06080702u, 0x06fcf906u, 0xfb0105feu, 0x07fafcfbu, 0xfffcff00u, 0x0104f705u,
    0x08f9fd04u, 0xf7fdfefau, 0x01030503u, 0xff050303u, 0xfd000608u, 0x05ff0202u, 0xfa0709fcu, 0xf7020103u,
    0x02fc0c01u, 0xf9fa0106u, 0xfdfe0901u, 0x06fffe0du, 0x07fefd0au, 0x0a03f804u, 0x030b03fbu, 0x03fe0df6u,
    0xfe000306u, 0x000104feu, 0x00fb04fdu, 0x00fdf8f8u, 0xfcfa020cu, 0xfb020b03u, 0xf80b0407u, 0x03fd0407u,
    0x0d04fdf8u, 0xf7030806u, 0xf30402f4u, 0x06ff0100u, 0x0b05fcfbu, 0x0102f9ffu, 0x03fffffbu, 0x0600fff8u,
    0x0df30209u, 0xf9090108u, 0xfb0001ffu, 0xf9fcfefbu, 0x0c02fdffu, 0xfc00f9ffu, 0xfafa0503u, 0x0003f906u,
    0xf9060206u, 0xf802fdfdu, 0x03fefb04u, 0xfcfcf404u, 0x00ff0003u, 0xfcfcfa05u, 0x0604f4fcu, 0xfc030200u,
    0x02f9fefbu, 0xf8fb01f8u, 0x0901fd04u, 0xfc0003f3u, 0x060105fbu, 0xf4fc0500u, 0x05fe0504u, 0x03f4f901u,
    0x070c0404u, 0xf306f7feu, 0xfe080902u, 0x0104fd0du, 0x00fcfdfcu, 0x08fd0805u, 0xfb0909feu, 0x02f903fcu,
    0x0d00faf7u, 0xf9020105u, 0xf7000007u, 0xf70801f3u, 0xf304f303u, 0x0201fffau, 0x03060afdu, 0x0105fd05u,
    0x01fefff9u, 0xfc05f406u, 0x0700f7fdu, 0x0b02fff5u, 0xfe0200fbu, 0xf9f800fcu, 0x0800f903u, 0x0501fffbu,
    0xfe0104f8u, 0x060207f9u, 0xfe0cf3ffu, 0xfc030704u, 0xf6fd01ffu, 0xfefa0206u, 0xfa000209u, 0xfe06fcf3u,
    0xfa090904u, 0x00f90d07u, 0x06030a04u, 0xfb09fe01u, 0x04fcf806u, 0x06fbfa06u, 0xfe0cfffeu, 0xfd000307u,
    0x000304fbu, 0x09fbf3fbu, 0xfbfb00fdu, 0x04f9f700u, 0xfc09fcffu, 0xfefbf7f9u, 0x01080604u, 0xfe0102fcu,
    0xfef600f8u, 0x0001fa01u, 0xf802f300u, 0xfff8f904u, 0x06020309u, 0x090300fdu, 0x090df900u, 0xfd0b0a00u,
// ... 858 lines not shown
    0x0b0800f5u, 0xf9fefe05u, 0xf9fbfc06u, 0xf40108f6u, 0xf3fcf4fbu, 0x010203fbu, 0xff070a03u, 0xfe05fb02u,
    0x02ff03fau, 0xfa02f3feu, 0x0604faf8u, 0x080806f7u, 0xfd0003fcu, 0xfff502fdu, 0x0605f9feu, 0x030402fbu,
    0xfe0008fcu, 0x04050afeu, 0xf709f6f8u, 0xfb000307u, 0xfaf80100u, 0x02fafe06u, 0xfbfcfc08u, 0xfb0404f3u,
    0xf6040509u, 0x04fa060du, 0x03060609u, 0xf704fe00u, 0x06fff600u, 0x08fff801u, 0xf70900feu, 0xfefefe07u,
    0xfe0206feu, 0x0a01f8f4u, 0xfff902feu, 0x07fdf9fbu, 0xf705fdfdu, 0x01fbfdf5u, 0xfc070307u, 0xfe0004feu,
    0x04f705fau, 0xff01fbfdu, 0xf8fdf5f8u, 0x04f9f8ffu, 0x0405fd09u, 0x060802feu, 0x0010fafcu, 0xf7070806u,
    0x08fd0700u, 0xfe04f600u, 0x040002fau, 0x01000d04u, 0xff010409u, 0xfe0404fdu, 0xfe04ee03u, 0x00fe0c04u,
    0x06fe03fdu, 0xf3ff0efbu, 0xfa00fa04u, 0x020bfbf7u, 0xf8030807u, 0xf7000503u, 0xfefcfe06u, 0x04fb0607u,
    0xfdfe0702u, 0x0e030a01u, 0x0007fb04u, 0x00ffff08u, 0xff01fffbu, 0x02fdf607u, 0xfb010500u, 0xff09f5f9u,
    0x0702f808u, 0xfdfd04fcu, 0x0005010du, 0x00f50501u, 0x0206fe07u, 0xf7fcfeffu, 0x010702fau, 0x08ff0404u,
    0x000204fdu, 0x01fafef3u, 0x03fffc00u, 0xff050101u, 0x02f9f9feu, 0xff090407u, 0xfafffb0cu, 0xf9040503u,
    0x03fa04fdu, 0x09010200u, 0xf8fcef01u, 0xf3fefe04u, 0xfe03fcfeu, 0x0a03010du, 0xff020bf8u, 0xf503fa06u,
    0xfb020305u, 0xfa0104f3u, 0xfffdf8fcu, 0xfcff0600u, 0xf408f709u, 0x03fbfcfau, 0xfff8fc04u, 0x0c010307u,
    0x0300ff00u, 0x02f9f904u, 0xfd04faf2u, 0xfdf90dfeu, 0x02fff6fbu, 0xfd05f607u, 0xfe01fafdu, 0xfefb05fcu,
    0xf9040601u, 0x08f80507u, 0x04fdff00u, 0xfb050204u, 0x0205fb07u, 0xfefef801u, 0x0303fc0du, 0xfdfef600u,
    0xfd0504f9u, 0x000bfdfdu, 0x090a0dfeu, 0xfcfbf500u, 0xfe0203fdu, 0xfb090f00u, 0xfe07fcf9u, 0x0afe04f8u,
    0xf1020203u, 0x070cfffdu, 0xfc07f4fau, 0x0809fdfcu, 0x04fc0af7u, 0x0502fe00u, 0xfefef9feu, 0x05f506feu,
    0xfff9fffau, 0xf6040406u, 0xf4fd0202u, 0xff01ff06u, 0xff0302f8u, 0xfd01f5fbu, 0xfcfefd03u, 0x06f704f9u,
    0x0902fef8u, 0x03f900f9u, 0xfc05fc0cu, 0x020af9feu, 0xfefffffdu, 0xf900fffdu, 0xfdf90b08u, 0x0904ff06u,
    0xfdfdfdfdu, 0x0c0404feu, 0xf802fc01u, 0x0102fdf7u, 0xfd0d03ffu, 0xfd0001fcu, 0xf2000a05u, 0xfefff9fbu,
    0xf3090503u, 0xf4fc0301u, 0x05f605fdu, 0xff05fb03u, 0x00f9000eu, 0x0105f805u, 0x0008f9ffu, 0xf8f707fbu,
    0xfdfa07fdu, 0xfcfafef8u, 0xfe050504u, 0x00f5fafdu, 0x03fd0a04u, 0x0206010cu, 0xfefdfd03u, 0x0208060bu,
    0x0afe0102u, 0xfafefe08u, 0xf80604f6u, 0x000a00f9u, 0xfbfe0a0au, 0x06fbfef8u, 0xfd04faffu, 0xff020700u,
    0xfafdf701u, 0xfd0c0203u, 0x020a0605u, 0x07fff703u, 0xfbff0500u, 0x09fdfefau, 0x01fcff00u, 0xff04f601u,
    0x0afdfc02u, 0xf9fa01fau, 0x00030305u, 0xfd040204u, 0xfdff020au, 0x05010103u, 0xf8040a00u, 0xf7fe0003u,
    0x03fd0b06u, 0xfcf8fe06u, 0xfefd0805u, 0x0602f90bu, 0x0701f908u, 0x0807f700u, 0xfe0b05fdu, 0x04ff10fcu,
    0xfeff0007u, 0x00010400u, 0x02fb05ffu, 0x01fdfcf5u, 0xfff9fd0cu, 0xfb000907u, 0xf4070108u, 0x04fe0108u,
    0x0a0901f7u, 0xf7ff0509u, 0xf2fe07f6u, 0x06020100u, 0x0809fefau, 0x0002fafcu, 0x030001fbu, 0x050202f8u,
    0x11f9fe09u, 0xf605fe08u, 0xfbfe01ffu, 0xfbf900fbu, 0x0a07fefeu, 0xfcfefafcu, 0xfdf80305u, 0xff03f703u,
    0xf703ff06u, 0xf8fffefcu, 0x04fffa02u, 0xfefbf3ffu, 0x00ffff03u, 0xfefbf802u, 0x0406f7f7u, 0xfb010201u,
    0x05fa00fbu, 0xfbf804f9u, 0x0805fc02u, 0xfcfe08f5u, 0x050307fdu, 0xf7f70502u, 0x05000306u, 0x08f6f9feu,
    0x020e0205u, 0xf200f9fbu, 0xfb060705u, 0xff04f80bu, 0x02fcfffbu, 0x09010508u, 0xf8060902u, 0x05fa04feu,
    0x0c05fef5u, 0xf9ffff05u, 0xf8fcfd06u, 0xf50406f5u, 0xf2fef3fdu, 0x010202fau, 0x00070a01u, 0xff05fb03u,
    0x02ff02f9u, 0xfa03f301u, 0x0603f9fau, 0x090604f6u, 0xfd0102fbu, 0xfdf602fcu, 0x0703f800u, 0x040301fbu,
    0xfe0007fau, 0x050409fcu, 0xf90af5fau, 0xfb010507u, 0xf8f901ffu, 0x01faff06u, 0xfbfefe09u, 0xfc0502f2u,
    0xf7060707u, 0x03fa090cu, 0x04050808u, 0xf806fe00u, 0x05fef602u, 0x08fef803u, 0xf90a00feu, 0xfdff0008u,
    0xff0306fdu, 0x0afff6f6u, 0xfdf901fdu, 0x07fbf8fcu, 0xf907fdfdu, 0x00fbfbf6u, 0xfe080406u, 0xfe0003fdu,
    0x02f603f9u, 0x0001fafeu, 0xf8fff4fbu, 0x02f8f801u, 0x0504ff09u, 0x070601fdu, 0x0310fafdu, 0xf9090904u,
    0x07fc07ffu, 0xff04f602u, 0x04ff01fau, 0x01ff0e02u, 0x00010508u, 0xff0403fcu, 0xff04ef07u, 0x00fe0d01u,
    0x06fd03fdu, 0xf3020cf8u, 0xfa02fb06u, 0x040bf9f9u, 0xf9040a05u, 0xf8020602u, 0xfdfdff06u, 0x02fb0705u,
    0xfcfe0800u, 0x0e000affu, 0x0107fc05u, 0xffff0108u, 0x0001fefcu, 0x02fcf808u, 0xfc0205ffu, 0x0009f4fcu,
    0x0800fa09u, 0xfdfd03fbu, 0x0105040du, 0xfef50500u, 0x0306ff07u, 0xf6fefeffu, 0x030701fau, 0x08fe0503u,
    0x000203fcu, 0xfffafbf4u, 0x03fefc01u, 0x00050100u, 0x00f8f800u, 0x01090506u, 0xfa01fd0du, 0xfa050602u,
    0x02f903fcu, 0x09000200u, 0xf7fdf005u, 0xf301ff04u, 0xfe04fcffu, 0x0a01040du, 0xff0209f6u, 0xf605fc07u,
    0xfb030404u, 0xfb0201f2u, 0xfefdf7feu, 0xfc0006feu, 0xf60af90bu, 0x02fafafbu, 0xfdf8fd05u, 0x0cff0507u,
    0x03ffff01u, 0x00f8fa05u, 0xfe05f7f3u, 0xfcfa0cfbu, 0x02fff5fdu, 0xfe06f808u, 0xfe01f9feu, 0xfdfb04fbu,
    0xfa0506ffu, 0x06f70606u, 0x03fcff01u, 0xfc060303u, 0x0305fc08u, 0xfdfff802u, 0x0303ff0eu, 0xfcfef602u,
    0xfe0602f8u, 0x020bfdfdu, 0x0b080cfbu, 0xfbfcf502u, 0xff0303fdu, 0xfd0a0ffdu, 0x0008fbfau, 0x0afc02f7u,
    0xf2050202u, 0x090bfefdu, 0xfe08f3fdu, 0x0a08fcfdu, 0x03fb08f5u, 0x0501fe00u, 0xfdfff9ffu, 0x02f406fdu,
    0xfdf9fefau, 0xf7060505u, 0xf4ff0302u, 0xff010106u, 0xff0301f8u, 0xfe02f4feu, 0xfcfffe04u, 0x04f603f8u,
    0x0900fdf8u, 0x02f8fefau, 0xfd05fe0du, 0x0409f900u, 0xfe00fefeu, 0xfa02fefeu, 0xfcfa0c06u, 0x0a020106u,
    0xfcfefdfdu, 0x0d0204feu, 0xf904fd01u, 0x0201fcf8u, 0xff0d02feu, 0xfd0000fcu, 0xf2030b03u, 0xfe00f8fcu,
    0xf50b0602u, 0xf3fe0301u, 0x03f504fcu, 0x0005fc04u, 0xfefa030eu, 0x0205f907u, 0x0107f901u, 0xf6f905fau,
    0xfcfb06fcu, 0xfbfbfcf9u, 0xff050503u, 0xfef5f9ffu, 0x03fd0b02u, 0x0306040cu, 0xfdfdfe04u, 0x0407080au,
    0x09fc0201u, 0xfa00ff08u, 0xf90802f5u, 0x020afefau, 0xfaff0c08u, 0x04fafcf9u, 0xfe05fa01u, 0x000206feu,
    0xf9fff703u, 0xff0c0303u, 0x04090603u, 0x07fdf804u, 0xfb0005ffu, 0x08fcfdfau, 0x00fcff00u, 0x0004f603u,
    0x09fbfc03u, 0xf8fbfffau, 0x00030404u, 0xfe050204u, 0xfdff0409u, 0x05000202u, 0xf9060afeu, 0xf7000003u,
    0x03fd0c03u, 0xfaf90006u, 0xfdfd0903u, 0x0600fb0cu, 0x07fffb09u, 0x0905f702u, 0x010b04fcu, 0x03ff0ff9u,
    0xfe000206u, 0x000104ffu, 0x01fb05feu, 0x01fdfaf7u, 0xfdf9ff0cu, 0xfb010a05u, 0xf6090208u, 0x04fe0208u,
    0x0c07fff8u, 0xf7010708u, 0xf20104f5u, 0x06000100u, 0x0a07fdfau, 0x0102f9feu, 0x030000fbu, 0x060101f8u,
    0x0ff60009u, 0xf707ff08u, 0xfbff01ffu, 0xfafbfffbu, 0x0b04fdfeu, 0xfcfff9feu, 0xfbf90404u, 0xff03f804u,
    0xf8040106u, 0xf800fefcu, 0x03fffa03u, 0xfdfbf301u, 0x00ffff03u, 0xfdfbf904u, 0x0505f5fau, 0xfb020200u,
    0x03fafffbu, 0xf9f903f8u, 0x0903fc03u, 0xfcff06f4u, 0x060206fcu, 0xf5fa0501u, 0x05ff0405u, 0x05f5f900u,
    0x040d0305u, 0xf203f8fcu, 0xfc070804u, 0x0004fa0cu, 0x01fcfefbu, 0x08ff0707u, 0xf9080900u, 0x03fa04fdu,
    0x0d03fcf6u, 0xf9010005u, 0xf7feff07u, 0xf60604f3u, 0xf201f300u, 0x020100fau, 0x02060affu, 0x0005fc04u,
    0x01fe00f9u, 0xfb04f303u, 0x0701f8fbu, 0x0a0401f5u, 0xfe0201fbu, 0xfbf701fcu, 0x0802f901u, 0x050200fbu,
    0xfe0106f9u, 0x050308fbu, 0xfc0bf3fcu, 0xfb020605u, 0xf7fb01ffu, 0xfffa0106u, 0xfaff0009u, 0xfd05fff2u,
    0xf8080806u, 0x01f90b0au, 0x05040906u, 0xf908fe01u, 0x05fdf704u, 0x07fcf905u, 0xfc0bfffeu, 0xfdff0107u,
    0xff0305fcu, 0x0afdf4f8u, 0xfcfa01fdu, 0x05faf7feu, 0xfa08fcfeu, 0xfffbf9f7u, 0xff080505u, 0xfe0103fdu,
    0x00f602f8u, 0x0001fa00u, 0xf800f3fdu, 0x01f8f802u, 0x05030109u, 0x080501fdu, 0x060ff9ffu, 0xfb0a0a02u,
    0x06fa07fdu, 0x0004f704u, 0x03fffffau, 0x01ff0effu, 0x00010707u, 0x000402fbu, 0x0004f10au, 0xfffe0dffu,
    0x05fc02fcu, 0xf4050af6u, 0xfa03fd06u, 0x0609f8fau, 0xfa060b03u, 0xf8030600u, 0xfdfd0106u, 0x01fa0804u,
    0xfcff07ffu, 0x0efd0afdu, 0x0307fd05u, 0xffff0208u, 0x0001fdfcu, 0x01fcfa0au, 0xfc0305feu, 0x0209f3feu,
    0x07fffc0au, 0xfcfe02fau, 0x0205070cu, 0xfcf605ffu, 0x04050107u, 0xf600fe00u, 0x0406fffau, 0x07fc0602u,
    0x010202fbu, 0xfefaf9f5u, 0x03fdfd01u, 0x01050100u, 0xfff9f901u, 0x03090604u, 0xfa02000du, 0xfc060600u,
    0x00f902fbu, 0x09fe02ffu, 0xf7fff108u, 0xf3030004u, 0xff04fc00u, 0x0aff070cu, 0x000207f4u, 0xf707fd08u,
    0xfc040403u, 0xfb03fef2u, 0xfdfdf700u, 0xfc0106fdu, 0xf80cfb0cu, 0x00fafafdu, 0xfbf9fe06u, 0x0bfc0605u,
    0x02feff01u, 0xfff9fc06u, 0xff05f5f5u, 0xfbfb0bf9u, 0x01fef500u, 0x0006fa0au, 0xff02f900u, 0xfcfc03fbu,
    0xfc0606feu, 0x04f60705u, 0x02fbff01u, 0xfe070303u, 0x0404fe09u, 0xfdfff904u, 0x0402020eu, 0xfcfff704u,
    0x000601f8u, 0x040afcfeu, 0x0c060bf9u, 0xfbfdf604u, 0xff0302fcu, 0xff0a0efau, 0x0107fafcu, 0x09fa00f7u,
    0xf3070302u, 0x0b09fdfdu, 0xff08f3ffu, 0x0b05fbfeu, 0x02fa06f4u, 0x0500fe01u, 0xfdfff901u, 0x00f405fcu,
};

static const int64_t TSLAM_WEDGES[31 * 2] = {
    16685309ll, -1753697ll,
    16685309ll, 1753697ll,
    15956081ll, 5184445ll,
    14529495ll, 8388608ll,
    12467901ll, 11226149ll,
    9861400ll, 13573053ll,
    6823909ll, 15326749ll,
    3488179ll, 16410594ll,
    0ll, 16777216ll,
    -3488179ll, 16410594ll,
    -6823909ll, 15326749ll,
    -9861400ll, 13573053ll,
    -12467901ll, 11226149ll,
    -14529495ll, 8388608ll,
    -15956081ll, 5184445ll,
    -16685309ll, 1753697ll,
    -16685309ll, -1753697ll,
    -15956081ll, -5184445ll,
    -14529495ll, -8388608ll,
    -12467901ll, -11226149ll,
    -9861400ll, -13573053ll,
    -6823909ll, -15326749ll,
    -3488179ll, -16410594ll,
    0ll, -16777216ll,
    3488179ll, -16410594ll,
    6823909ll, -15326749ll,
    9861400ll, -13573053ll,
    12467901ll, -11226149ll,
    14529495ll, -8388608ll,
    15956081ll, -5184445ll,
    16685309ll, -1753697ll,
};
```

Baseline: 270,200.

## Precompute tile/slot indexing and replace integer divisions with reciprocal multiplies

Replaces per-block level search and divisions in the describe kernel with a host-built tile lookup table, and uses a 3D grid so image and tile indices come straight from block coordinates. Ring-slot modulo on 64-bit frame indices is replaced by a precomputed slot0 plus a wrap-around, and small divisions by npair/ncam become umulhi reciprocal multiplies. Wedge constants move to a constexpr constant table, desc_ys zero-fill is deferred until after tile staging is issued, and some unaligned tail loads are skipped when not needed. This adds context setters that must be called everywhere g0 or the view ranges change, so any missed call site would leave slot0 or the reciprocals stale.

Result: faster. 281,500 (median of 6 runs) (+4.2%).

```diff
diff --git a/thor-slam_amd/csrc/k_describe.hip b/thor-slam_amd/csrc/k_describe.hip
--- a/thor-slam_amd/csrc/k_describe.hip
+++ b/thor-slam_amd/csrc/k_describe.hip
@@ -58,6 +58,18 @@
 }
 __constant__ DiscTable c_disc = make_disc_table();
 
+#include "tslam_tables.h"
+struct WedgeTable {
+    double e[64][4];
+};
+constexpr WedgeTable make_wedge_table() {
+    WedgeTable t{};
+    for (int b = 0; b < 30; ++b)
+        for (int j = 0; j < 4; ++j) t.e[b][j] = (double)TSLAM_WEDGES[2 * b + j];
+    return t;
+}
+__constant__ WedgeTable c_wedge = make_wedge_table();
+
 __global__ __launch_bounds__(TS_DT_THREADS) void k_describe(BatchCtx c) {
     __shared__ __attribute__((aligned(16))) uint8_t s_raw[(TS_DT_RAW_ROWS + 1) * TS_DT_RAW_P];
     __shared__ __attribute__((aligned(16))) uint8_t s_smo[TS_DT_SMO_ROWS * TS_DT_P];
@@ -65,36 +77,27 @@
     __shared__ uint32_t s_n;
     const int lane = threadIdx.x & 63, wave = threadIdx.x >> 6;
     int img, local;
-    if (!xcd_image_block(blockIdx.x, c.n * c.ncam, c.g.dt_total, &img, &local)) return;
-    int l = 0;
-    while (l + 1 < c.g.n_levels && local >= c.g.dt_start[l + 1]) ++l;
-    local -= c.g.dt_start[l];
-    const int nx = c.g.dt_nx[l];
-    const int ty = local / nx, tx = local - ty * nx;
+    if (!xcd_image_block3(c.n * c.ncam, c.g.dt_total, &img, &local)) return;
+    const uint32_t tile = c.dt_tile[local];
+    const int l = (int)(tile & 0xFFu), tx = (int)((tile >> 8) & 0xFFu), ty = (int)(tile >> 16);
+    const bool first = local == c.g.dt_start[l];
     const int W = c.g.W[l], H = c.g.H[l];
     const int x0 = tx * TS_DT_W, y0 = ty * TS_DT_H;
     int cam, f;
     view_image(c, img, &f, &cam);
-    const int slot = ring_slot(c, c.g0 + f);
+    const int slot = batch_slot(c, f);
     const size_t ib = (size_t)slot * c.C + cam;
+    const int koff = c.g.koff[l];
     const uint8_t* raw = c.pyr + ib * c.g.pyr_bytes + c.g.pyr_off[l];
     const uint8_t* smo = c.smo + ((size_t)f * c.C + cam) * c.g.pyr_bytes + c.g.pyr_off[l];
     uint32_t* kps = c.kps + ib * c.g.K * 2;
     uint32_t* desc = c.desc + ib * c.g.K * 8;
-    uint32_t* desc_ys = c.desc_ys + ib * c.g.K * 8;
-    const uint4* ys = c.ys + ib * c.g.K + c.g.koff[l];
-    const uint16_t* rs = c.rowstart + ib * c.g.rs_total + c.g.rs_off[l];
-    const int kn = c.kcount[ib * c.g.n_levels + l];
-
-    if (local == 0) {
-        const int Kl = c.g.Kq[l];
-        for (int i = kn * 8 + threadIdx.x; i < Kl * 8; i += TS_DT_THREADS) {
-            desc[(size_t)(c.g.koff[l] + i / 8) * 8 + (i & 7)] = 0u;
-            desc_ys[(size_t)(c.g.koff[l] + i / 8) * 8 + (i & 7)] = 0u;
-        }
-    }
-    const int pa = rs[y0], pb = rs[min(y0 + TS_DT_H, H)];
-    if (pa >= pb) return;
+    uint32_t* desc_ys = c.desc_ys + (ib * c.g.K + koff) * 8;
+    const uint4* ys = c.ys + ib * c.g.K + koff;
+    const size_t ra = ib * c.g.rs_total + c.g.rs_off[l] + y0, rb = ra + (min(y0 + TS_DT_H, H) - y0);
+    const uint32_t* rs32 = reinterpret_cast<const uint32_t*>(c.rowstart);
+    const uint32_t wa = rs32[ra >> 1], wb = rs32[rb >> 1];
+    const int kn = first ? c.kcount[ib * c.g.n_levels + l] : 0;
     if (threadIdx.x == 0) s_n = 0;
     __syncthreads();
 
@@ -103,6 +106,19 @@
     const int cr = x0 - 16;
     stage_tile<TS_DT_RAW_P / 16>(raw, W, H, y0 - 15, cr, TS_DT_RAW_ROWS, s_raw, wide16);
     stage_tile<TS_DT_P / 16, (TS_DT_W + 2 * TS_DT_HX) / 16>(smo, W, H, y0 - 18, c0, TS_DT_SMO_ROWS, s_smo, wide16);
+
+    if (first) {
+        const int Kl = c.g.Kq[l];
+        for (int i = kn * 8 + threadIdx.x; i < Kl * 8; i += TS_DT_THREADS) {
+            desc[(size_t)(koff + i / 8) * 8 + (i & 7)] = 0u;
+            desc_ys[i] = 0u;
+        }
+    }
+    const int pa = (int)((wa >> (16 * (ra & 1))) & 0xFFFFu), pb = (int)((wb >> (16 * (rb & 1))) & 0xFFFFu);
+    if (pa >= pb) {
+        asm volatile("s_waitcnt vmcnt(0)" ::: "memory");
+        return;
+    }
 
     uint32_t wx[5], mk[5], wy[5];
     int rofs[5];
@@ -114,8 +130,7 @@
         wy[i] = d.z;
         rofs[i] = (int)d.w;
     }
-    const double wa0 = lane < 30 ? (double)c.wedges[2 * lane] : 0.0, wa1 = lane < 30 ? (double)c.wedges[2 * lane + 1] : 0.0;
-    const double wb0 = lane < 30 ? (double)c.wedges[2 * lane + 2] : 0.0, wb1 = lane < 30 ? (double)c.wedges[2 * lane + 3] : 0.0;
+    const double wa0 = c_wedge.e[lane][0], wa1 = c_wedge.e[lane][1], wb0 = c_wedge.e[lane][2], wb1 = c_wedge.e[lane][3];
 
     for (int p = pa + threadIdx.x; p < pb; p += TS_DT_THREADS) {
         const int x = ys[p].x & 0xFFFF;
@@ -136,7 +151,7 @@
             bin[g] = 0;
             if (pos[g] < 0) continue;
             const int x = rec[g].x & 0xFFFF, y = rec[g].x >> 16;
-            const int ob = (y - y0) * TS_DT_RAW_P + (x - 15 - cr);
+            const int ob = (int)__umul24((uint32_t)(y - y0), TS_DT_RAW_P) + (x - 15 - cr);
             const uint32_t sh = (uint32_t)ob & 3u;
             const uint8_t* obase = s_raw + (ob & ~3);
             uint32_t sx = 0, s1 = 0, sy = 0;
@@ -165,7 +180,7 @@
         for (int g = 0; g < TS_DT_G; ++g) {
             if (pos[g] < 0) continue;
             const int x = rec[g].x & 0xFFFF, y = rec[g].x >> 16;
-            const uint8_t* pbase = s_smo + (y - y0) * TS_DT_P + (x - 18 - c0);
+            const uint8_t* pbase = s_smo + ((int)__umul24((uint32_t)(y - y0), TS_DT_P) + (x - 18 - c0));
             uint32_t words[8];
 #pragma unroll
             for (int j = 0; j < 4; ++j) {
@@ -181,7 +196,7 @@
             for (int j = 0; j < 8; ++j) asm volatile("v_writelane_b32 %0, %1, %2" : "+v"(w) : "s"(words[j]), "i"(j));
             if (lane < 8) {
                 desc[(size_t)kidx * 8 + lane] = w;
-                desc_ys[(size_t)(c.g.koff[l] + pos[g]) * 8 + lane] = w;
+                desc_ys[(size_t)pos[g] * 8 + lane] = w;
             }
             if (lane == 0) kps[(size_t)kidx * 2 + 1] = (rec[g].y & ~0xFF00u) | ((uint32_t)bin[g] << 8);
         }
@@ -189,5 +204,5 @@
 }
 
 void launch_describe(const BatchCtx& c, hipStream_t s) {
-    hipLaunchKernelGGL(k_describe, dim3(xcd_grid(c.n * c.ncam, c.g.dt_total)), dim3(TS_DT_THREADS), 0, s, c);
-}
+    hipLaunchKernelGGL(k_describe, xcd_grid3(c.n * c.ncam, c.g.dt_total), dim3(TS_DT_THREADS), 0, s, c);
+}
diff --git a/thor-slam_amd/csrc/k_image.hip b/thor-slam_amd/csrc/k_image.hip
--- a/thor-slam_amd/csrc/k_image.hip
+++ b/thor-slam_amd/csrc/k_image.hip
@@ -28,7 +28,7 @@
     const int y0 = blockIdx.x * TS_RECT_BAND;
     const int rows0 = min(TS_RECT_BAND, H - y0);
     const uint8_t* src = c.images + view_src(c, img) * W * H;
-    uint8_t* pyr = c.pyr + ((size_t)ring_slot(c, c.g0 + f) * c.C + cam) * c.g.pyr_bytes;
+    uint8_t* pyr = c.pyr + ((size_t)batch_slot(c, f) * c.C + cam) * c.g.pyr_bytes;
     const bool has_map = (c.map_mask >> cam) & 1u;
     const int32_t* map = c.maps + (size_t)cam * W * H * 2;
     bool wide = (W & 63) == 0 && (c.g.pyr_bytes & 15) == 0;
@@ -463,7 +463,7 @@
     const int BR = c.g.band_rows[l];
     const int y0 = band * BR;
     const int lane = threadIdx.x & 63, wave = threadIdx.x >> 6;
-    const size_t img_off = ((size_t)ring_slot(c, c.g0 + f) * c.C + cam) * c.g.pyr_bytes + c.g.pyr_off[l];
+    const size_t img_off = ((size_t)batch_slot(c, f) * c.C + cam) * c.g.pyr_bytes + c.g.pyr_off[l];
     const uint8_t* src = c.pyr + img_off;
     uint8_t* smo = c.smo + ((size_t)f * c.C + cam) * c.g.pyr_bytes + c.g.pyr_off[l];
     const int NR = BR + 2 * TS_DET_HALO;
@@ -1000,7 +1000,7 @@
     });
     __syncthreads();
     const int nsel = min((int)s_nsel, Kl);
-    const int slot = ring_slot(c, c.g0 + f);
+    const int slot = batch_slot(c, f);
     uint32_t* kp = c.kps + (((size_t)slot * c.C + cam) * c.g.K + c.g.koff[l]) * 2;
     const int Hl = c.g.H[l];
     const bool counting = !S::BIG || nsel <= S::KCAP;
diff --git a/thor-slam_amd/csrc/k_match.hip b/thor-slam_amd/csrc/k_match.hip
--- a/thor-slam_amd/csrc/k_match.hip
+++ b/thor-slam_amd/csrc/k_match.hip
@@ -47,8 +47,8 @@
     const int z = blockIdx.y;
     const int mode = z < nfp ? 1 : 0;
     const int fl = z < nfp ? z : z - nfp;
-    const int p = c.pair0 + fl % c.npair;
-    const int f = fl / c.npair;
+    const int f = div_small(fl, c.npair_rcp);
+    const int p = c.pair0 + (fl - f * c.npair);
     const int64_t g = c.g0 + f;
     int l = 0;
     while (l + 1 < c.g.n_levels && (int)blockIdx.x >= c.g.qtile_start[l + 1]) ++l;
@@ -64,9 +64,9 @@
         no_match();
         return;
     }
-    const int slot = ring_slot(c, g);
+    const int slot = batch_slot(c, f);
     const int qcam = c.cpp * p;
-    const int tslot = mode == 0 ? slot : ring_slot(c, g - 1);
+    const int tslot = mode == 0 ? slot : prev_slot(c, slot);
     const int tcam = mode == 0 ? qcam + 1 : qcam;
     const int K = c.g.K;
     const int qn = c.kcount[((size_t)slot * c.C + qcam) * c.g.n_levels + l];
@@ -386,7 +386,7 @@
     const uint8_t* a = img + (size_t)y * W + x0;
     const uint32_t sh = (uint32_t)(reinterpret_cast<uintptr_t>(a) & 3u);
     const uint32_t* q = reinterpret_cast<const uint32_t*>(a - sh);
-    const uint32_t d[5] = {q[0], q[1], q[2], q[3], q[4]};
+    const uint32_t d[5] = {q[0], q[1], q[2], q[3], sh >= 2u ? q[4] : 0u};
     return align_row15(d, sh);
 }
 
@@ -512,10 +512,9 @@
     const int lane = threadIdx.x & 63, wave = threadIdx.x >> 6;
     const int K = c.g.K;
     int z, local;
-    if (!xcd_image_block(blockIdx.x, c.n * c.npair, (K + TS_RS_QPB - 1) / TS_RS_QPB, &z, &local)) return;
-    const int p = c.pair0 + z % c.npair, f = z / c.npair;
-    const int64_t g = c.g0 + f;
-    const int slot = ring_slot(c, g);
+    if (!xcd_image_block3(c.n * c.npair, (K + TS_RS_QPB - 1) / TS_RS_QPB, &z, &local)) return;
+    const int f = div_small(z, c.npair_rcp), p = c.pair0 + (z - f * c.npair);
+    const int slot = batch_slot(c, f);
     const int sub = lane & 7;
     const int qslot = wave * 8 + (lane >> 3);
     const int pos = local * TS_RS_QPB + qslot;
@@ -569,10 +568,10 @@
     const int lane = threadIdx.x & 63, wave = threadIdx.x >> 6;
     const int K = c.g.K;
     int z, local;
-    if (!xcd_image_block(blockIdx.x, c.n * c.npair, (K + TS_RT_QPB - 1) / TS_RT_QPB, &z, &local)) return;
-    const int p = c.pair0 + z % c.npair, f = z / c.npair;
-    const int64_t g = c.g0 + f;
-    const int slot = ring_slot(c, g);
+    if (!xcd_image_block3(c.n * c.npair, (K + TS_RT_QPB - 1) / TS_RT_QPB, &z, &local)) return;
+    const int f = div_small(z, c.npair_rcp), p = c.pair0 + (z - f * c.npair);
+    const bool has_prev = c.g0 + f > 0;
+    const int slot = batch_slot(c, f);
     const int sub = lane & 7;
     const int qslot = wave * 8 + (lane >> 3);
     const int pos = local * TS_RT_QPB + qslot;
@@ -582,13 +581,13 @@
     const size_t qkb = ((size_t)slot * c.C + qcam) * K;
     int l = 0, qi = 0, j = -1;
     uint32_t qxy = 0, pxy = 0;
-    const int pslot = g > 0 ? ring_slot(c, g - 1) : slot;
+    const int pslot = has_prev ? prev_slot(c, slot) : slot;
     if (live) {
         const uint4 rec = c.ys[qkb + pos];
         qi = (int)rec.z;
         l = (int)(rec.y & 0xFFu);
         qxy = rec.x;
-        j = match_lookup(c, mbase, pos, qi, rec.w != 0 && g > 0, ((size_t)pslot * c.C + qcam) * K, &pxy);
+        j = match_lookup(c, mbase, pos, qi, rec.w != 0 && has_prev, ((size_t)pslot * c.C + qcam) * K, &pxy);
     }
     int32_t* out_idx = c.temporal + ((size_t)slot * c.P + p) * K;
     double* out_uv = c.tuv + (((size_t)f * c.P + p) * K + qi) * 2;
@@ -638,11 +637,11 @@
     const int lane = threadIdx.x & 63, wave = threadIdx.x >> 6;
     const int K = c.g.K;
     int z, local;
-    if (!xcd_image_block(blockIdx.x, c.n * c.npair, (K + TS_RP_QPB - 1) / TS_RP_QPB, &z, &local)) return;
-    const int p = c.pair0 + z % c.npair, f = z / c.npair;
-    const int64_t g = c.g0 + f;
-    const int slot = ring_slot(c, g);
-    const int pslot = g > 0 ? ring_slot(c, g - 1) : slot;
+    if (!xcd_image_block3(c.n * c.npair, (K + TS_RP_QPB - 1) / TS_RP_QPB, &z, &local)) return;
+    const int f = div_small(z, c.npair_rcp), p = c.pair0 + (z - f * c.npair);
+    const bool has_prev = c.g0 + f > 0;
+    const int slot = batch_slot(c, f);
+    const int pslot = has_prev ? prev_slot(c, slot) : slot;
     const int sub = lane & 7;
     const int qslot = wave * 8 + (lane >> 3);
     const int pos = local * TS_RP_QPB + qslot;
@@ -663,7 +662,7 @@
         match_train(c, mbase, ((size_t)slot * c.C + qcam + 1) * K, &ms, &tkp);
         match_train(c, mbase + K, ((size_t)pslot * c.C + qcam) * K, &mt, &pxy);
         js = match_accept(c, ms, qi, rec.w != 0);
-        jt = match_accept(c, mt, qi, rec.w != 0 && g > 0);
+        jt = match_accept(c, mt, qi, rec.w != 0 && has_prev);
     }
     const size_t out = ((size_t)slot * c.P + p) * K + qi;
     if (live && sub == 0) c.temporal[out] = jt;
@@ -693,7 +692,8 @@
             sh[k] = (uint32_t)(reinterpret_cast<uintptr_t>(a) & 3u);
             const uint32_t* q = reinterpret_cast<const uint32_t*>(a - sh[k]);
 #pragma unroll
-            for (int i = 0; i < 5; ++i) d[k][i] = q[i];
+            for (int i = 0; i < 4; ++i) d[k][i] = q[i];
+            d[k][4] = (!inp && sh[k] >= 2u) ? q[4] : 0u;
         }
 #pragma unroll
         for (int k = 0; k < TS_RP_ROUNDS; ++k) {
@@ -761,18 +761,18 @@
     st.match_modes = 1;
     (void)hipMemsetAsync(st.tbest, 0xFF, sizeof(uint32_t) * (size_t)st.n * st.P * 2 * st.g.K, s);
     launch_k_match(st, dim3(st.g.total_qtiles, st.n * st.npair), s);
-    hipLaunchKernelGGL(k_refine_stereo, dim3(xcd_grid(st.n * st.npair, (st.g.K + TS_RS_QPB - 1) / TS_RS_QPB)), dim3(256), 0, s, st);
+    hipLaunchKernelGGL(k_refine_stereo, xcd_grid3(st.n * st.npair, (st.g.K + TS_RS_QPB - 1) / TS_RS_QPB), dim3(256), 0, s, st);
 }
 
 void launch_match_refine(const BatchCtx& c, hipStream_t s) {
     const int K = c.g.K;
     if (!c.rgbd && c.match_modes == 3 && c.mp.refine_split == 0) {
-        hipLaunchKernelGGL(k_refine_pair, dim3(xcd_grid(c.n * c.npair, (K + TS_RP_QPB - 1) / TS_RP_QPB)), dim3(256), 0, s, c);
+        hipLaunchKernelGGL(k_refine_pair, xcd_grid3(c.n * c.npair, (K + TS_RP_QPB - 1) / TS_RP_QPB), dim3(256), 0, s, c);
         return;
     }
     if (c.rgbd)
         launch_rgbd_depth(c, s);
     else
-        hipLaunchKernelGGL(k_refine_stereo, dim3(xcd_grid(c.n * c.npair, (K + TS_RS_QPB - 1) / TS_RS_QPB)), dim3(256), 0, s, c);
-    hipLaunchKernelGGL(k_refine_temporal, dim3(xcd_grid(c.n * c.npair, (K + TS_RT_QPB - 1) / TS_RT_QPB)), dim3(256), 0, s, c);
-}
+        hipLaunchKernelGGL(k_refine_stereo, xcd_grid3(c.n * c.npair, (K + TS_RS_QPB - 1) / TS_RS_QPB), dim3(256), 0, s, c);
+    hipLaunchKernelGGL(k_refine_temporal, xcd_grid3(c.n * c.npair, (K + TS_RT_QPB - 1) / TS_RT_QPB), dim3(256), 0, s, c);
+}
diff --git a/thor-slam_amd/csrc/k_pose.hip b/thor-slam_amd/csrc/k_pose.hip
--- a/thor-slam_amd/csrc/k_pose.hip
+++ b/thor-slam_amd/csrc/k_pose.hip
@@ -225,8 +225,8 @@
 __global__ __launch_bounds__(POSE_THREADS) void k_corr(BatchCtx c) {
     TS_BACK_PRIO;
     __shared__ int s_scan[2 * (POSE_THREADS / 64)];
-    const int p = c.pair0 + (int)blockIdx.x % c.npair;
-    const int f = (int)blockIdx.x / c.npair;
+    const int f = div_small((int)blockIdx.x, c.npair_rcp);
+    const int p = c.pair0 + ((int)blockIdx.x - f * c.npair);
     const int fp = f * c.P + p;
     const int64_t g = c.g0 + f;
     const int tid = threadIdx.x;
@@ -240,8 +240,8 @@
     }
     const PairCalib cal = c.calib[p];
     const double fx = cal.fx, fy = cal.fy, cx = cal.cx, cy = cal.cy;
-    const int pslot = ring_slot(c, g - 1);
-    const int32_t* tm = c.temporal + ((size_t)ring_slot(c, g) * c.P + p) * K;
+    const int slot = batch_slot(c, f), pslot = prev_slot(c, slot);
+    const int32_t* tm = c.temporal + ((size_t)slot * c.P + p) * K;
     const double* tuv = c.tuv + ((size_t)f * c.P + p) * K * 2;
     const double* dprev = c.disp + ((size_t)pslot * c.P + p) * K;
     const uint32_t* kprev = c.kps + ((size_t)pslot * c.C + c.cpp * p) * K * 2;
diff --git a/thor-slam_amd/csrc/k_reloc.hip b/thor-slam_amd/csrc/k_reloc.hip
--- a/thor-slam_amd/csrc/k_reloc.hip
+++ b/thor-slam_amd/csrc/k_reloc.hip
@@ -127,9 +127,8 @@
     BatchCtx r = c;
     r.n = 1;
     r.P = 1;
-    r.pair0 = 0;
-    r.npair = 1;
-    r.g0 = frame;
+    ctx_set_views(r, r.cam0, r.ncam, 0, 1);
+    ctx_set_first_frame(r, frame);
     r.prior = nullptr;
     r.rig_prior = nullptr;
     r.calib[0] = c.calib[pair];
@@ -156,9 +155,8 @@
     }
     BatchCtx r = c;
     r.n = 1;
-    r.pair0 = 0;
-    r.npair = c.P;
-    r.g0 = frame;
+    ctx_set_views(r, r.cam0, r.ncam, 0, c.P);
+    ctx_set_first_frame(r, frame);
     r.corr = corr;
     r.stats = stats;
     r.pose = pose;
diff --git a/thor-slam_amd/csrc/k_rgbd.hip b/thor-slam_amd/csrc/k_rgbd.hip
--- a/thor-slam_amd/csrc/k_rgbd.hip
+++ b/thor-slam_amd/csrc/k_rgbd.hip
@@ -33,7 +33,7 @@
     const int fl = blockIdx.y, p = c.pair0 + fl % c.npair, f = fl / c.npair;
     const int k = blockIdx.x * blockDim.x + threadIdx.x;
     if (k >= K) return;
-    const int slot = ring_slot(c, c.g0 + f);
+    const int slot = batch_slot(c, f);
     const size_t ib = (size_t)slot * c.C + p;
     const uint32_t* kp = c.kps + (ib * K + k) * 2;
     const int l = (int)(kp[1] & 0xFF);
diff --git a/thor-slam_amd/csrc/tslam_api.cpp b/thor-slam_amd/csrc/tslam_api.cpp
--- a/thor-slam_amd/csrc/tslam_api.cpp
+++ b/thor-slam_amd/csrc/tslam_api.cpp
@@ -133,7 +133,7 @@
     c.B = h->B;
     c.R = h->R;
     c.n = h->cur_n;
-    c.g0 = h->cur_g0;
+    ctx_set_first_frame(c, h->cur_g0);
     c.W = h->W;
     c.H = h->H;
     c.cpp = h->prm.rgbd ? 1 : 2;
@@ -181,6 +181,7 @@
     c.det_fail = (uint32_t*)h->buf[TSLAM_BUF_DET_FAIL].ptr;
     c.brief_table = h->d_brief;
     c.wedges = h->d_wedges;
+    c.dt_tile = h->d_dt_tile;
     for (int p = 0; p < h->P; ++p) c.calib[p] = h->calib[p];
     c.mp.max_hamming = h->prm.max_hamming;
     c.mp.ratio_pct = h->prm.ratio_pct;
@@ -201,10 +202,7 @@
     c.pp.seed = h->prm.ransac_seed;
     c.fast_threshold = h->prm.fast_threshold;
     c.margin = h->prm.edge_margin;
-    c.cam0 = h->sh_cam_lo;
-    c.ncam = h->sh_cam_hi - h->sh_cam_lo;
-    c.pair0 = 0;
-    c.npair = h->P;
+    ctx_set_views(c, h->sh_cam_lo, h->sh_cam_hi - h->sh_cam_lo, 0, h->P);
     c.match_modes = 3;
     c.reloc = 0;
     c.peer_S = c.peer_me = c.peer_nbuf = c.peer_skip = 0;
@@ -374,6 +372,7 @@
     if (rc == TSLAM_OK) h->d_hyp = (double*)h->buf[TSLAM_BUF_HYP].ptr;
     if (rc == TSLAM_OK) rc = dev_alloc(h, (void**)&h->d_brief, sizeof(TSLAM_BRIEF_TABLE));
     if (rc == TSLAM_OK) rc = dev_alloc(h, (void**)&h->d_wedges, sizeof(TSLAM_WEDGES));
+    if (rc == TSLAM_OK) rc = dev_alloc(h, (void**)&h->d_dt_tile, sizeof(uint32_t) * (size_t)h->g.dt_total);
     if (rc == TSLAM_OK) rc = dev_alloc(h, (void**)&h->d_maps, sizeof(int32_t) * (size_t)C * W * H * 2);
     if (rc == TSLAM_OK && p.ba_window) rc = alloc_ba(h);
     if (rc == TSLAM_OK && p.rgbd) rc = dev_alloc(h, (void**)&h->d_gray, (size_t)B * P * W * H);
@@ -391,6 +390,9 @@
     }
     bool ok = hipMemcpy(h->d_brief, brief_off.data(), sizeof(uint32_t) * brief_off.size(), hipMemcpyHostToDevice) == hipSuccess &&
               hipMemcpy(h->d_wedges, TSLAM_WEDGES, sizeof(TSLAM_WEDGES), hipMemcpyHostToDevice) == hipSuccess;
+    std::vector<uint32_t> dt_tile(h->g.dt_total);
+    describe_tile_table(h->g, dt_tile.data());
+    ok = ok && hipMemcpy(h->d_dt_tile, dt_tile.data(), sizeof(uint32_t) * dt_tile.size(), hipMemcpyHostToDevice) == hipSuccess;
     for (int i = 0; i < h->P && ok; ++i) {
         const int32_t* m[2] = {pairs[i].map_left, pairs[i].map_right};
         const int cpp = p.rgbd ? 1 : 2;
diff --git a/thor-slam_amd/csrc/tslam_api_exchange.cpp b/thor-slam_amd/csrc/tslam_api_exchange.cpp
--- a/thor-slam_amd/csrc/tslam_api_exchange.cpp
+++ b/thor-slam_amd/csrc/tslam_api_exchange.cpp
@@ -3,7 +3,7 @@
 static BatchCtx range_ctx(const BatchCtx& c, int lo, int hi) {
     BatchCtx r = c;
     const size_t P = c.P, K = c.g.K, f = lo;
-    r.g0 = c.g0 + lo;
+    ctx_set_first_frame(r, c.g0 + lo);
     r.n = hi - lo;
     r.qbest += f * P * 2 * K;
     r.qsecond += f * P * 2 * K;
@@ -31,8 +31,7 @@
     int lo, hi;
     shard_range(h, c.n, &lo, &hi);
     BatchCtx own = c;
-    own.pair0 = h->sh_cam_lo;
-    own.npair = h->sh_cam_hi - h->sh_cam_lo;
+    ctx_set_views(own, own.cam0, own.ncam, h->sh_cam_lo, h->sh_cam_hi - h->sh_cam_lo);
     const BatchCtx cr = range_ctx(c, lo, hi);
     const BackView v{&own, nullptr, hi > lo ? &cr : nullptr, false, false};
     int rc = run_front_stage(h, c, stage, s);
@@ -54,13 +53,13 @@
     const bool empty = hi <= lo;
     const bool pre = !empty && c.g0 + lo - 1 >= 0;
     BatchCtx cp = c;
-    cp.g0 = c.g0 + lo - 1;
+    ctx_set_first_frame(cp, c.g0 + lo - 1);
     cp.n = 1;
     BatchCtx cr = c;
     BackView v{empty ? nullptr : &cb, pre ? &cp : nullptr, empty ? nullptr : &cb, true, false};
     if (h->sh_pairs) {
-        cb.pair0 = cp.pair0 = h->sh_cam_lo / 2;
-        cb.npair = cp.npair = 1;
+        ctx_set_views(cb, cb.cam0, cb.ncam, h->sh_cam_lo / 2, 1);
+        ctx_set_views(cp, cp.cam0, cp.ncam, h->sh_cam_lo / 2, 1);
         int rl, rh;
         shard_range(h, c.n, &rl, &rh);
         cr = range_ctx(c, rl, rh);
@@ -143,10 +142,9 @@
     const int ncam = cam_hi - cam_lo;
     const int64_t skip = first_frame < 0 ? -first_frame : 0;
     c.images = images + (size_t)skip * ncam * h->W * h->H;
-    c.g0 = first_frame + skip;
+    ctx_set_first_frame(c, first_frame + skip);
     c.n = (int)(n_frames - skip);
-    c.cam0 = cam_lo;
-    c.ncam = ncam;
+    ctx_set_views(c, cam_lo, ncam, c.pair0, c.npair);
     launch_rectify_pyramid(c, (hipStream_t)stream);
     HIPCHK(hipGetLastError());
     return TSLAM_OK;
@@ -286,7 +284,7 @@
     const int skip = first < 0 ? 1 : 0;
     BatchCtx c = make_ctx(h);
     c.images = raw;
-    c.g0 = first + skip;
+    ctx_set_first_frame(c, first + skip);
     c.n = nr - skip;
     c.peer_S = g.S;
     c.peer_me = h->sh_rank;
@@ -346,10 +344,9 @@
     const int skip = first < 0 ? 1 : 0;
     BatchCtx c = make_ctx(h);
     c.images = raw + (size_t)skip * h->W * h->H;
-    c.g0 = first + skip;
+    ctx_set_first_frame(c, first + skip);
     c.n = nf - skip;
-    c.cam0 = partner;
-    c.ncam = 1;
+    ctx_set_views(c, partner, 1, c.pair0, c.npair);
     if (c.n > 0) launch_rectify_pyramid(c, (hipStream_t)stream);
     launch_stream_blocks(make_ctx(h), false, first, nf, partner, 1, (uint8_t*)streams, (hipStream_t)stream);
     HIPCHK(hipGetLastError());
diff --git a/thor-slam_amd/csrc/tslam_common.h b/thor-slam_amd/csrc/tslam_common.h
--- a/thor-slam_amd/csrc/tslam_common.h
+++ b/thor-slam_amd/csrc/tslam_common.h
@@ -48,6 +48,16 @@
     int dt_total;
 };
 
+static inline void describe_tile_table(const LevelGeom& g, uint32_t* out) {
+    for (int l = 0; l < g.n_levels; ++l) {
+        const int end = l + 1 < g.n_levels ? g.dt_start[l + 1] : g.dt_total;
+        for (int i = g.dt_start[l]; i < end; ++i) {
+            const int local = i - g.dt_start[l], ty = local / g.dt_nx[l], tx = local - ty * g.dt_nx[l];
+            out[i] = (uint32_t)l | ((uint32_t)tx << 8) | ((uint32_t)ty << 16);
+        }
+    }
+}
+
 struct PairCalib {
     double fx, fy, cx, cy, fxb;
 };
@@ -78,6 +88,9 @@
     int reloc;
     int peer_S, peer_me, peer_nbuf, peer_skip;
     int64_t g0;
+    int slot0;
+    uint32_t ncam_rcp, npair_rcp;
+    const uint32_t* dt_tile;
     int W, H;
     const uint8_t* images;
     const uint8_t* rgbd_in;
@@ -131,6 +144,23 @@
 };
 
 static inline __host__ __device__ int ring_slot(const BatchCtx& c, int64_t g) { return (int)(g % c.R); }
+static inline uint32_t small_rcp(int d) { return d > 1 ? (uint32_t)((1ull << 32) / (uint32_t)d) + 1u : 0u; }
+static inline void ctx_set_first_frame(BatchCtx& c, int64_t g0) {
+    c.g0 = g0;
+    c.slot0 = ring_slot(c, g0);
+}
+static inline void ctx_set_views(BatchCtx& c, int cam0, int ncam, int pair0, int npair) {
+    c.cam0 = cam0, c.ncam = ncam, c.pair0 = pair0, c.npair = npair;
+    c.ncam_rcp = small_rcp(ncam), c.npair_rcp = small_rcp(npair);
+}
+#ifdef __HIPCC__
+__device__ __forceinline__ int batch_slot(const BatchCtx& c, int f) {
+    const int s = c.slot0 + f;
+    return s >= c.R ? s - c.R : s;
+}
+__device__ __forceinline__ int prev_slot(const BatchCtx& c, int slot) { return slot > 0 ? slot - 1 : c.R - 1; }
+__device__ __forceinline__ int div_small(int a, uint32_t rcp) { return rcp ? (int)__umulhi((uint32_t)a, rcp) : a; }
+#endif
 
 #include "tslam_ranges.h"
 __device__ __forceinline__ void view_image(const BatchCtx& c, int img, int* f, int* cam) {
@@ -141,7 +171,7 @@
         *cam = q * c.peer_S + (r - *f * c.peer_S);
         return;
     }
-    *f = img / c.ncam;
+    *f = div_small(img, c.ncam_rcp);
     *cam = c.cam0 + (img - *f * c.ncam);
 }
 __device__ __forceinline__ size_t view_src(const BatchCtx& c, int img) {
@@ -508,6 +538,16 @@
     *local = k % bpi;
     return *img < n_img;
 }
+static inline __host__ dim3 xcd_grid3(int n_img, int bpi) {
+    const int groups = (n_img + 7) / 8;
+    return bpi <= 65535 && groups <= 65535 ? dim3(8, bpi, groups) : dim3(xcd_grid(n_img, bpi));
+}
+__device__ __forceinline__ bool xcd_image_block3(int n_img, int bpi, int* img, int* local) {
+    if ((int)gridDim.y != bpi) return xcd_image_block(blockIdx.x, n_img, bpi, img, local);
+    *img = blockIdx.z * 8 + blockIdx.x;
+    *local = blockIdx.y;
+    return *img < n_img;
+}
 
 __device__ __forceinline__ double pose_used(const BatchCtx& c, int st, int f0, int i) {
     return (st == 0 || (st == 2 && c.g0 + f0 + i == 0)) ? 1.0 : 0.0;
diff --git a/thor-slam_amd/csrc/tslam_handle.h b/thor-slam_amd/csrc/tslam_handle.h
--- a/thor-slam_amd/csrc/tslam_handle.h
+++ b/thor-slam_amd/csrc/tslam_handle.h
@@ -33,6 +33,7 @@
     int32_t* d_maps = nullptr;
     uint32_t* d_brief = nullptr;
     int64_t* d_wedges = nullptr;
+    uint32_t* d_dt_tile = nullptr;
     uint8_t* d_gray = nullptr;
     Buffer buf[TSLAM_BUF_COUNT];
     uint32_t* d_cand = nullptr;
diff --git a/thor-slam_amd/csrc/tslam_tables.h b/thor-slam_amd/csrc/tslam_tables.h
--- a/thor-slam_amd/csrc/tslam_tables.h
+++ b/thor-slam_amd/csrc/tslam_tables.h
@@ -964,7 +964,7 @@
     0xf3070302u, 0x0b09fdfdu, 0xff08f3ffu, 0x0b05fbfeu, 0x02fa06f4u, 0x0500fe01u, 0xfdfff901u, 0x00f405fcu,
 };
 
-static const int64_t TSLAM_WEDGES[31 * 2] = {
+static constexpr int64_t TSLAM_WEDGES[31 * 2] = {
     16685309ll, -1753697ll,
     16685309ll, 1753697ll,
     15956081ll, 5184445ll,
```
